# Nazukixv/LiteASR

Measured on AMD Instinct MI355X. Metric: utterances/sec (U2-Conformer+CTC, 80-d fbank T≈1000) at 1/2/4/8 MI355X, higher is better.
Workload: dtype bf16; 1 GPU; U2-Conformer-small hybrid CTC-attention training step (fwd+loss+bwd+allreduce+clip+Noam/Adam); model=U2 enc 12x conformer d256 H4 ff2048, dec 6x, V 4233, global_batch=32, per_gpu_batch=32, seq_len=1000, label_len=40, parallelism=dp1, launch=hipgraph, ranks_seen=1, rank_launcher=env

## Files before the change

### include/liteasr_hip.h

```cpp
#ifndef LITEASR_HIP_H
#define LITEASR_HIP_H

#include <stdint.h>

#ifdef __cplusplus
extern "C" {
#endif

enum { LASR_F32 = 0, LASR_BF16 = 1, LASR_I32 = 2, LASR_I64 = 3, LASR_U8 = 4 };
enum { LASR_OK = 0, LASR_ERR_INVALID = -1, LASR_ERR_LAUNCH = -2 };
enum { LASR_ACT_NONE = 0, LASR_ACT_RELU = 1, LASR_ACT_SWISH = 2,
       LASR_ACT_GATE = 3 ,
       LASR_ACT_TANH = 4  };

const char* lasr_last_error(void);
int lasr_version(void);
int lasr_set_dropout_counter(const uint64_t* dev_counter);
int lasr_counter_add(uint64_t* dev_counter, uint64_t v, void* stream);

typedef struct lasr_gemm_args {
  int M, N, K;
  int batch, batch_div;
  const void* A; int64_t lda_m, lda_k, sa1, sa2;
  const void* B; int64_t ldb_n, ldb_k, sb1, sb2;
  void* C; int64_t ldc, sc1, sc2;
  int in_dtype;
  int c_dtype;
  float alpha; const float* alpha_dev;
  float beta;
  const float* bias;
  int act;
  void* zout;
  const void* aux; int aux_dtype; int64_t ldaux; int aux_act;
  float drop_p; uint64_t drop_seed;
  const void* res; int res_dtype; int64_t ldres; float res_scale;
  int split_k;
  void* workspace; int64_t workspace_bytes;
  float* rowsum;
  int zout_mode;
  int tile_m, tile_n;
  int ksub;
} lasr_gemm_args;
int lasr_gemm(const lasr_gemm_args* args, void* stream);
int lasr_gemm_ln_fwd(const lasr_gemm_args* args, const float* gamma, const float* beta, float eps, void* y,
                     int y_dtype, float* mean, float* rstd, void* stream);
int lasr_gemm_ln_bwd(const lasr_gemm_args* args, const void* x, int x_dtype, const float* gamma, const float* mean,
                     const float* rstd, const void* dres, int dres_dtype, void* dx, int dx_dtype, float* part,
                     int64_t part_floats, void* gb, int gb_dtype, float bscale, float bp, uint64_t bseed,
                     void* stream);
int lasr_gemm_qbias_bwd(const lasr_gemm_args* args, const void* dqu, const void* dqv, int dt, int B, int T, int H,
                        int dk, void* dqkv, int64_t ld, float* ws, int64_t ws_floats, void* stream);
float lasr_dropout_scale(float p);
#define LASR_PLAN_GLDS 1
#define LASR_PLAN_ROWSUM_FUSED 2
#define LASR_PLAN_KSUB2 4
#define LASR_PLAN_WIDE 8
int lasr_gemm_plan(const lasr_gemm_args* args, int* tile_m, int* tile_n, int* split_k, int* flags);

int lasr_gemm_dw_group(const lasr_gemm_args* args, int n, void* stream);
int lasr_gemm_dw_group_order(int longest_first);
int lasr_gemm_narrow_tiles(int on);

typedef struct lasr_reduce_seg {
  const float* part; int64_t N; int P; int accumulate;
  float* out0; float* out1; int64_t split;
} lasr_reduce_seg;
int lasr_reduce_multi(const lasr_reduce_seg* segs, int nseg, void* stream);

int lasr_colsum(const void* X, int dtype, int64_t M, int64_t N, int64_t ldx,
                float* out, int accumulate, float* workspace, int64_t ws_floats, void* stream);

int lasr_layernorm_fwd(const void* x, int x_dtype, int64_t rows, int D, const float* gamma,
                       const float* beta, float eps, void* y, int y_dtype, float* mean,
                       float* rstd, void* y2, int y2_dtype, float p2, uint64_t seed2,
                       void* stream);
int lasr_layernorm2_fwd(const float* x, int64_t rows, int D, const float* g1, const float* b1,
                        const float* g2, const float* b2, float eps, float* y, float* mean1,
                        float* rstd1, void* z, float* mean2, float* rstd2, void* stream);
int lasr_layernorm_bwd(const void* x, int x_dtype, const void* dy, int dy_dtype, int64_t rows,
                       int D, const float* gamma, const float* mean, const float* rstd,
                       const void* dres, int dres_dtype, void* dx, int dx_dtype,
                       float* dgamma, float* dbeta, float* workspace, int64_t ws_floats,
                       void* gb, int gb_dtype, float bscale, float bp, uint64_t bseed,
                       void* stream);
int lasr_layernorm2_bwd(const float* x1, const void* dy1, int dy1_dtype, const float* dres1, int64_t rows, int D,
                        const float* g1, const float* mean1, const float* rstd1, float* part1, const float* x2,
                        const float* g2, const float* mean2, const float* rstd2, float* dx2, float* part2, void* gb2,
                        int gb2_dtype, float bscale, float bp, uint64_t bseed, void* stream);
typedef struct lasr_row_ln_args {
  int M, D, K;
  const void* A; int64_t lda;
  const void* W; int64_t ldw;
  const float* gamma1; const float* beta1; float eps;
  float* mean1; float* rstd1;
  const float* bias; const float* res; float res_scale; float drop_p; uint64_t drop_seed;
  float* out; void* y1; int y1_dtype;
  const float* gamma2; const float* beta2; void* y2; float* mean2; float* rstd2;
  const float* x; const float* dres; float* dx; void* gb; float bscale; float bp; uint64_t bseed;
  float* part; float* dgamma; float* dbeta;
} lasr_row_ln_args;
int lasr_linear_res_ln(const lasr_row_ln_args* args, void* stream);
int lasr_linear_dx_ln_bwd(const lasr_row_ln_args* args, void* stream);

int lasr_branch_grad(const void* dx, int dx_dtype, int64_t n, void* gb, int gb_dtype,
                     float scale, float p, uint64_t seed, void* stream);

int lasr_ctc_fwd(const void* logits, int ldt, int B, int T, int V, int64_t ld, const int32_t* targets,
                 int Lmax, const int32_t* ilen, const int32_t* tlen, float* lse, float* lp,
                 float* alpha, float* beta, float* nll, void* stream);
int lasr_ctc_lattice(int B, int T, int Lmax, const int32_t* targets, const int32_t* ilen, const int32_t* tlen,
                     const float* lp, float* alpha, float* beta, float* nll, void* stream);
int lasr_ctc_bwd(const void* logits, int ldt, int B, int T, int V, int64_t ld, const int32_t* targets,
                 int Lmax, const int32_t* ilen, const int32_t* tlen, const float* lse,
                 const float* lp, const float* alpha, const float* nll, float* beta,
                 int beta_ready, void* grad, int gdt, float gscale, const float* gdev, void* stream);

int lasr_lsm_kl_fwd(const void* logits, int ldt, int R, int V, int64_t ld, const int32_t* target,
                    int ignore, float smoothing, float* lse, float* loss_rows, void* stream);
int lasr_lsm_kl_bwd(const void* logits, int ldt, int R, int V, int64_t ld, const int32_t* target,
                    int ignore, float smoothing, const float* lse, void* grad, int gdt,
                    float gscale, const float* gdev, void* stream);
int lasr_loss_combine(const float* a, int na, float wa, const float* b, int nb, float wb,
                      float* out, void* stream);

int lasr_qbias_fwd(const void* qkv, int dt, int B, int T, int H, int dk, int64_t ld_qkv,
                   const float* bias_u, const float* bias_v, void* qu, void* qv, void* stream);
int lasr_qbias_bwd(const void* dqu, const void* dqv, int dt, int B, int T, int H, int dk,
                   void* dqkv, int64_t ld_dqkv, float* dbias_u, float* dbias_v,
                   float* workspace, int64_t ws_floats, void* stream);
int lasr_attn_softmax_fwd(const float* s_ac, const float* s_bd, int relpos, int B, int H,
                          int Tq, int Tk, int ldS, const uint8_t* mask, int64_t mask_sb,
                          int64_t mask_sq, void* P, int pdt, float drop_p, uint64_t seed,
                          void* Praw, void* stream);
int lasr_attn_softmax_bwd(const void* P, int pdt, const float* dPd, int B, int H, int Tq, int Tk,
                          int ldS, const uint8_t* mask, int64_t mask_sb, int64_t mask_sq,
                          float drop_p, uint64_t seed, void* dS, int dsdt, void* stream);
int lasr_relshift_bwd(const void* dS, int dt, int Z, int T, int ldS, void* dBD, void* stream);
int lasr_relattn_fwd(const void* qu, const void* qv, int64_t ldq, const void* k, const void* v,
                     int64_t ldkv, const void* pos, int64_t ldp, int B, int H, int T, int dk,
                     const uint8_t* mask, int64_t mask_sb, int64_t mask_sq, float scale,
                     float* stats, void* ctx, int64_t ldc, void* stream);
int lasr_relattn_fwd_qb(const void* q, int64_t ldqin, const float* bu, const float* bv, void* qu, void* qv,
                        int64_t ldq, const void* k, const void* v, int64_t ldkv, const void* pos, int64_t ldp,
                        int B, int H, int T, int dk, const uint8_t* mask, int64_t mask_sb, int64_t mask_sq,
                        float scale, float* stats, void* ctx, int64_t ldc, void* stream);
int lasr_relattn_bwd(const void* qu, const void* qv, int64_t ldq, const void* k, const void* v,
                     int64_t ldkv, const void* pos, int64_t ldp, int B, int H, int T, int dk,
                     const uint8_t* mask, int64_t mask_sb, int64_t mask_sq, float scale,
                     const float* stats, const void* ctx, const void* dctx, int64_t ldc,
                     float* Dbuf, void* dqu, void* dbd, int ldS, int dbd_head_major, void* dk_out,
                     void* dv_out, int64_t lddkv, void* stream);
int lasr_attn_fwd(const void* q, int64_t ldq, const void* k, const void* v, int64_t ldkv, int B, int H,
// ... 36 lines not shown
  const void* w2p;
  const float* bias;
  const void* dy2; int64_t dy2_rows;
  void* out;
  float* rowsum;
  void* workspace; int64_t workspace_bytes;
  const float* x; int T, F;
  float* dw1; float* db1;
} lasr_conv2_args;
int lasr_conv2_gemm(const lasr_conv2_args* args, void* stream);
int64_t lasr_conv2_dx_w1_workspace(int B, int T1, int F1, int C);
typedef struct lasr_cif_args {
  int B, T, D, U;
  const float* z; const int* plen; const int* ylen; const float* h;
  float* alpha; float* acc; uint8_t* fired; int* row; float* sum_alpha; float* mae; float* out;
  const float* gout; const float* gsum; float* dz; float* dh;
} lasr_cif_args;
int lasr_cif_fwd(const lasr_cif_args* args, void* stream);
int lasr_cif_bwd(const lasr_cif_args* args, void* stream);
typedef struct lasr_cif_infer_args {
  int B, T, D;
  const float* z; const int* plen; const float* h;
  float* alpha; float* acc; uint8_t* fired; int* row; float* sum_alpha; int* ulen; int* count; float* out;
} lasr_cif_infer_args;
int lasr_cif_infer(const lasr_cif_infer_args* args, void* stream);
int lasr_glancing_mix(int64_t rows, int D, const uint8_t* replace, const float* a, const float* b,
                      float* out, float* out2, int backward, void* stream);
int lasr_permute_last2(const void* src, int sdt, int64_t N, int64_t A, int64_t Bd, void* dst,
                       int ddt, int reverse, int accumulate, void* stream);

int lasr_glu_dwconv_fwd(const void* z1, int dt, int B, int T, int C, int K, const float* w,
                        const float* bias, void* y, int ydt, float* stats_ws, void* stream);
int lasr_dwconv_nparts(int B, int T);
int lasr_bn_finalize(const float* stats_ws, int nparts, int C, float eps, float momentum,
                     const float* gamma, const float* beta, float* running_mean,
                     float* running_var, int64_t* num_batches, float* mean, float* rstd,
                     float* scale, float* shift, int mode, void* stream);
int lasr_bn_act_fwd(const void* y, int ydt, int64_t rows, int C, const float* scale,
                    const float* shift, void* h, int hdt, int act, void* stream);
int lasr_bn_act_bwd(const void* y, int ydt, const void* dh, int hdt, int64_t rows, int C,
                    const float* scale, const float* shift, const float* mean,
                    const float* rstd, const float* gamma, float* dgamma, float* dbeta,
                    void* dy, int dydt, float* ws, int64_t ws_floats, int batch_stats, int act,
                    void* stream);
int lasr_glu_dwconv_bwd(const void* z1, int dt, const void* dy, int dydt, int B, int T, int C,
                        int K, const float* w, void* dz1, float* dw, float* db, float* ws,
                        int64_t ws_floats, void* stream);
int lasr_bn_act_glu_dwconv_bwd(const void* y, int ydt, const void* dh, int hdt, int B, int T, int C,
                               const float* scale, const float* shift, const float* mean, const float* rstd,
                               const float* gamma, float* dgamma, float* dbeta, float* bn_ws,
                               int64_t bn_ws_floats, int batch_stats, int act, const void* z1, int dt, int K,
                               const float* w, void* dz1, float* dw, float* db, float* ws, int64_t ws_floats,
                               void* stream);

int lasr_cast(const void* src, int sdt, void* dst, int ddt, int64_t n, void* stream);
int lasr_scale_add(const void* a, int adt, const void* b, int bdt, float sa, float sb,
                   void* out, int odt, int64_t n, void* stream);
int lasr_embed_pe_fwd(const int32_t* ids, int R, int L, int D, const float* E,
                      const float* pe, float xscale, float p, uint64_t seed, void* y, int ydt,
                      void* stream);
int lasr_embed_bwd(const int32_t* ids, int R, int D, const void* dy, int dydt, float xscale,
                   float p, uint64_t seed, float* dE, void* stream);
int lasr_pe_fwd(const void* x, int xdt, int64_t rows, int T, int D, const float* pe,
                float xscale, float p, uint64_t seed, void* y, int ydt, void* stream);

int lasr_rnnt_fwd(const void* logits, int ldt, int B, int T, int U1, int V, int64_t ld, const int32_t* targets,
                  int Lmax, const int32_t* ilen, const int32_t* tlen, int blank, float* lse, float* lp,
                  float* alpha, float* beta, float* nll, void* stream);
int lasr_rnnt_bwd(const void* logits, int ldt, int B, int T, int U1, int V, int64_t ld, const int32_t* targets,
                  int Lmax, const int32_t* ilen, const int32_t* tlen, int blank, const float* lse, const float* lp,
                  const float* alpha, const float* beta, const float* nll, void* grad, int gdt, float gscale,
                  const float* gdev, void* stream);
int lasr_joint_fwd(const float* e, const float* d, int B, int T, int U1, int J, void* z, int zdt, void* stream);
int lasr_joint_reduce(const void* dz, int dzdt, int B, int T, int U1, int J, void* de, void* dd, int odt,
                      void* stream);
int lasr_lstm_cell_fwd(const float* gates, int64_t ldg, const float* bias, const float* c_prev, int B, int H,
                       float* c_out, void* h_out, int hdt, int64_t ldh, void* stream);
int lasr_lstm_cell_bwd(const float* gates, int64_t ldg, const float* bias, const float* c, const float* c_prev,
                       const void* dh_out, int dhdt, int64_t lddh, const float* dh_rec, const float* dc_next, int B,
                       int H, void* dgates, int gdt, int64_t lddg, float* dc_prev, void* stream);

int lasr_u2_prep(const int64_t* xlens, const int64_t* ys, const int64_t* ylens, int B, int Tx,
                 int L, int Tsub, int sos, int eos, int chunk, int32_t* ys_in, int32_t* tgt,
                 int32_t* tgt_ctc, uint8_t* dec_mask, uint8_t* enc_mask, int32_t* pred_len,
                 int32_t* ylen32, void* stream);
int lasr_u2_prep_ld(const int64_t* xlens, const int64_t* ys, const int64_t* ylens, int B, int Tx,
                    int L, int Tsub, int sos, int eos, int chunk, int32_t* ys_in, int32_t* tgt,
                    int32_t* tgt_ctc, uint8_t* dec_mask, int dec_ld, uint8_t* enc_mask, int enc_ld,
                    int32_t* pred_len, int32_t* ylen32, void* stream);
int lasr_u2_prep_chunk(const int64_t* xlens, const int64_t* ys, const int64_t* ylens, int B, int L,
                       int Tsub, int sos, int eos, int chunk_mode, int chunk, int32_t* chunk_dev,
                       const uint64_t* ctr, uint64_t chunk_seed, int chunk_max, int32_t* ys_in,
                       int32_t* tgt, int32_t* tgt_ctc, uint8_t* dec_mask, int dec_ld, uint8_t* key_mask,
                       uint8_t* chunk_mask, int chunk_ld, int32_t* pred_len, int32_t* ylen32,
                       void* stream);

int64_t lasr_spec_augment_ws_bytes(int B, int Tmax);
int lasr_spec_augment(const float* x, float* out, const int64_t* xlens, const int32_t* plan,
                      int plan_stride, int B, int Tmax, int F, int replace_with_zero, void* ws,
                      int64_t ws_bytes, void* stream);

int lasr_sumsq_nparts(int64_t n);
int lasr_sumsq_partial(const float* g, int64_t n, float* ws, int64_t ws_floats, void* stream);
int lasr_adam_step(float* param, void* param_lp, int lp_dtype, const float* grad, float* m,
                   float* v, int64_t n, const float* ws, int nparts, float* state,
                   float max_norm, int lr_mode, float lr, float factor, float model_dim,
// ... 81 lines not shown
```

### liteasr_amd/_native.py

```python

from __future__ import annotations

import ctypes as C
import os

_HERE = os.path.dirname(os.path.abspath(__file__))
LIB_PATH = os.path.join(_HERE, "lib", "libliteasr_hip.so")

F32, BF16, I32, I64, U8 = 0, 1, 2, 3, 4
ACT_NONE, ACT_RELU, ACT_SWISH, ACT_GATE, ACT_TANH = 0, 1, 2, 3, 4

_p = C.c_void_p
_i = C.c_int
_l = C.c_int64
_f = C.c_float
_u = C.c_uint64


class GemmArgs(C.Structure):

    _fields_ = [
        ("M", _i), ("N", _i), ("K", _i),
        ("batch", _i), ("batch_div", _i),
        ("A", _p), ("lda_m", _l), ("lda_k", _l), ("sa1", _l), ("sa2", _l),
        ("B", _p), ("ldb_n", _l), ("ldb_k", _l), ("sb1", _l), ("sb2", _l),
        ("C", _p), ("ldc", _l), ("sc1", _l), ("sc2", _l),
        ("in_dtype", _i), ("c_dtype", _i),
        ("alpha", _f), ("alpha_dev", _p),
        ("beta", _f),
        ("bias", _p),
        ("act", _i),
        ("zout", _p),
        ("aux", _p), ("aux_dtype", _i), ("ldaux", _l), ("aux_act", _i),
        ("drop_p", _f), ("drop_seed", _u),
        ("res", _p), ("res_dtype", _i), ("ldres", _l), ("res_scale", _f),
        ("split_k", _i), ("workspace", _p), ("workspace_bytes", _l),
        ("rowsum", _p),
        ("zout_mode", _i),
        ("tile_m", _i), ("tile_n", _i), ("ksub", _i),
    ]


class Conv2Args(C.Structure):

    _fields_ = [
        ("mode", _i),
        ("B", _i), ("T1", _i), ("F1", _i), ("C", _i),
        ("y1", _p), ("w2p", _p), ("bias", _p),
        ("dy2", _p), ("dy2_rows", _l),
        ("out", _p), ("rowsum", _p),
        ("workspace", _p), ("workspace_bytes", _l),
        ("x", _p), ("T", _i), ("F", _i),
        ("dw1", _p), ("db1", _p),
    ]


CONV2_FWD, CONV2_DW, CONV2_DX, CONV2_DX_W1 = 0, 1, 2, 3


class CifArgs(C.Structure):

    _fields_ = [
        ("B", _i), ("T", _i), ("D", _i), ("U", _i),
        ("z", _p), ("plen", _p), ("ylen", _p), ("h", _p),
        ("alpha", _p), ("acc", _p), ("fired", _p), ("row", _p), ("sum_alpha", _p), ("mae", _p), ("out", _p),
        ("gout", _p), ("gsum", _p), ("dz", _p), ("dh", _p),
    ]


class CifInferArgs(C.Structure):

    _fields_ = [
        ("B", _i), ("T", _i), ("D", _i),
        ("z", _p), ("plen", _p), ("h", _p),
        ("alpha", _p), ("acc", _p), ("fired", _p), ("row", _p), ("sum_alpha", _p), ("ulen", _p), ("count", _p),
        ("out", _p),
    ]


class RowLnArgs(C.Structure):

    _fields_ = [
        ("M", _i), ("D", _i), ("K", _i),
        ("A", _p), ("lda", _l), ("W", _p), ("ldw", _l),
        ("gamma1", _p), ("beta1", _p), ("eps", _f), ("mean1", _p), ("rstd1", _p),
        ("bias", _p), ("res", _p), ("res_scale", _f), ("drop_p", _f), ("drop_seed", _u),
        ("out", _p), ("y1", _p), ("y1_dtype", _i),
        ("gamma2", _p), ("beta2", _p), ("y2", _p), ("mean2", _p), ("rstd2", _p),
        ("x", _p), ("dres", _p), ("dx", _p), ("gb", _p), ("bscale", _f), ("bp", _f), ("bseed", _u),
        ("part", _p), ("dgamma", _p), ("dbeta", _p),
    ]


class ReduceSeg(C.Structure):

    _fields_ = [("part", _p), ("N", _l), ("P", _i), ("accumulate", _i), ("out0", _p), ("out1", _p),
                ("split", _l)]


RNNT_SEARCH_MAX_LAYERS = 8


class RnntSearchArgs(C.Structure):

    _fields_ = [
        ("Tcap", _i), ("layers", _i), ("dec_dim", _i), ("H", _i), ("J", _i), ("V", _i),
        ("node_cap", _i), ("slot_cap", _i),
        ("w_dtype", _i),
        ("arena", _p), ("arena_bytes", _l),
        ("embed", _p),
        ("Wih", _p * RNNT_SEARCH_MAX_LAYERS), ("Whh", _p * RNNT_SEARCH_MAX_LAYERS),
        ("bih", _p * RNNT_SEARCH_MAX_LAYERS), ("bhh", _p * RNNT_SEARCH_MAX_LAYERS),
        ("Wd", _p), ("Wj", _p), ("bj", _p), ("enc_proj", _p),
    ]


SIGNATURES = {
    "lasr_version": [],
    "lasr_last_error": [],
    "lasr_set_dropout_counter": [_p],
    "lasr_counter_add": [_p, _u, _p],
    "lasr_gemm": [C.POINTER(GemmArgs), _p],
    "lasr_gemm_plan": [C.POINTER(GemmArgs), _p, _p, _p, _p],
    "lasr_gemm_dw_group": [C.POINTER(GemmArgs), _i, _p],
    "lasr_gemm_dw_group_order": [_i],
    "lasr_gemm_narrow_tiles": [_i],
    "lasr_relattn_fwd": [_p, _p, _l, _p, _p, _l, _p, _l, _i, _i, _i, _i, _p, _l, _l, _f, _p, _p, _l, _p],
    "lasr_relattn_fwd_qb": [_p, _l, _p, _p, _p, _p, _l, _p, _p, _l, _p, _l, _i, _i, _i, _i, _p, _l, _l, _f, _p, _p,
                            _l, _p],
    "lasr_attn_fwd": [_p, _l, _p, _p, _l, _i, _i, _i, _i, _i, _p, _l, _l, _f, _p, _p, _l, _p],
    "lasr_attn_bwd": [_p, _l, _p, _p, _l, _i, _i, _i, _i, _i, _p, _l, _l, _f, _p, _p, _p, _l, _p, _p, _p, _p,
                      _l, _p],
    "lasr_attn_fwd_split": [_p, _l, _p, _p, _l, _i, _i, _i, _i, _i, _p, _l, _l, _f, _p, _p, _l, _i, _p, _l, _p],
    "lasr_attn_bwd_split": [_p, _l, _p, _p, _l, _i, _i, _i, _i, _i, _p, _l, _l, _f, _p, _p, _p, _l, _p, _p, _p,
                            _p, _l, _i, _p, _l, _p],
    "lasr_attn_split_work": [_i, _i, _i, _i, _i],
    "lasr_attn_split_count": [_i, _i, _i, _i],
    "lasr_relattn_bwd": [_p, _p, _l, _p, _p, _l, _p, _l, _i, _i, _i, _i, _p, _l, _l, _f, _p, _p, _p, _l,
                         _p, _p, _p, _i, _i, _p, _p, _l, _p],
    "lasr_reduce_multi": [C.POINTER(ReduceSeg), _i, _p],
    "lasr_linear_res_ln": [C.POINTER(RowLnArgs), _p],
    "lasr_linear_dx_ln_bwd": [C.POINTER(RowLnArgs), _p],
    "lasr_dropout_scale": [_f],
    "lasr_colsum": [_p, _i, _l, _l, _l, _p, _i, _p, _l, _p],
    "lasr_layernorm2_fwd": [_p, _l, _i, _p, _p, _p, _p, _f, _p, _p, _p, _p, _p, _p, _p],
    "lasr_layernorm_fwd": [_p, _i, _l, _i, _p, _p, _f, _p, _i, _p, _p, _p, _i, _f, _u, _p],
    "lasr_layernorm_bwd": [_p, _i, _p, _i, _l, _i, _p, _p, _p, _p, _i, _p, _i, _p, _p, _p, _l,
                           _p, _i, _f, _f, _u, _p],
    "lasr_layernorm2_bwd": [_p, _p, _i, _p, _l, _i, _p, _p, _p, _p, _p, _p, _p, _p, _p, _p, _p, _i, _f, _f, _u,
                            _p],
    "lasr_branch_grad": [_p, _i, _l, _p, _i, _f, _f, _u, _p],
    "lasr_ctc_fwd": [_p, _i, _i, _i, _i, _l, _p, _i, _p, _p, _p, _p, _p, _p, _p, _p],
    "lasr_ctc_lattice": [_i, _i, _i, _p, _p, _p, _p, _p, _p, _p, _p],
    "lasr_rnnt_fwd": [_p, _i, _i, _i, _i, _i, _l, _p, _i, _p, _p, _i, _p, _p, _p, _p, _p, _p],
    "lasr_rnnt_bwd": [_p, _i, _i, _i, _i, _i, _l, _p, _i, _p, _p, _i, _p, _p, _p, _p, _p, _p, _i, _f, _p, _p],
    "lasr_joint_fwd": [_p, _p, _i, _i, _i, _i, _p, _i, _p],
    "lasr_joint_reduce": [_p, _i, _i, _i, _i, _i, _p, _p, _i, _p],
    "lasr_lstm_cell_fwd": [_p, _l, _p, _p, _i, _i, _p, _p, _i, _l, _p],
    "lasr_lstm_cell_bwd": [_p, _l, _p, _p, _p, _p, _i, _l, _p, _p, _i, _i, _p, _i, _l, _p, _p],
    "lasr_ctc_bwd": [_p, _i, _i, _i, _i, _l, _p, _i, _p, _p, _p, _p, _p, _p, _p, _i, _p, _i, _f, _p, _p],
    "lasr_lsm_kl_fwd": [_p, _i, _i, _i, _l, _p, _i, _f, _p, _p, _p],
    "lasr_lsm_kl_bwd": [_p, _i, _i, _i, _l, _p, _i, _f, _p, _p, _i, _f, _p, _p],
    "lasr_loss_combine": [_p, _i, _f, _p, _i, _f, _p, _p],
    "lasr_qbias_fwd": [_p, _i, _i, _i, _i, _i, _l, _p, _p, _p, _p, _p],
    "lasr_qbias_bwd": [_p, _p, _i, _i, _i, _i, _i, _p, _l, _p, _p, _p, _l, _p],
    "lasr_attn_softmax_fwd": [_p, _p, _i, _i, _i, _i, _i, _i, _p, _l, _l, _p, _i, _f, _u, _p, _p],
    "lasr_attn_softmax_bwd": [_p, _i, _p, _i, _i, _i, _i, _i, _p, _l, _l, _f, _u, _p, _i, _p],
    "lasr_relshift_bwd": [_p, _i, _i, _i, _i, _p, _p],
    "lasr_reduce_batch": [_p, _i, _i, _i, _i, _p, _i, _p],
    "lasr_conv1_fwd": [_p, _i, _i, _i, _i, _p, _p, _p, _i, _p],
    "lasr_conv1_bwd": [_p, _i, _i, _i, _i, _p, _i, _p, _p, _p, _l, _p],
    "lasr_conv2_gemm": [C.POINTER(Conv2Args), _p],
    "lasr_conv2_dx_w1_workspace": [_i, _i, _i, _i],
    "lasr_cif_fwd": [C.POINTER(CifArgs), _p],
    "lasr_cif_bwd": [C.POINTER(CifArgs), _p],
    "lasr_cif_infer": [C.POINTER(CifInferArgs), _p],
    "lasr_glancing_mix": [_l, _i, _p, _p, _p, _p, _p, _i, _p],
    "lasr_im2col3x3s2": [_p, _i, _i, _i, _i, _i, _p, _p],
    "lasr_col2im3x3s2": [_p, _i, _i, _i, _i, _i, _p, _p, _p],
    "lasr_permute_last2": [_p, _i, _l, _l, _l, _p, _i, _i, _i, _p],
    "lasr_glu_dwconv_fwd": [_p, _i, _i, _i, _i, _i, _p, _p, _p, _i, _p, _p],
    "lasr_dwconv_nparts": [_i, _i],
    "lasr_bn_finalize": [_p, _i, _i, _f, _f, _p, _p, _p, _p, _p, _p, _p, _p, _p, _i, _p],
    "lasr_bn_act_fwd": [_p, _i, _l, _i, _p, _p, _p, _i, _i, _p],
    "lasr_bn_act_bwd": [_p, _i, _p, _i, _l, _i, _p, _p, _p, _p, _p, _p, _p, _p, _i, _p, _l, _i, _i, _p],
    "lasr_glu_dwconv_bwd": [_p, _i, _p, _i, _i, _i, _i, _i, _p, _p, _p, _p, _p, _l, _p],
    "lasr_bn_act_glu_dwconv_bwd": [_p, _i, _p, _i, _i, _i, _i, _p, _p, _p, _p, _p, _p, _p, _p, _l, _i, _i,
                                   _p, _i, _i, _p, _p, _p, _p, _p, _l, _p],
    "lasr_cast": [_p, _i, _p, _i, _l, _p],
    "lasr_scale_add": [_p, _i, _p, _i, _f, _f, _p, _i, _l, _p],
    "lasr_embed_pe_fwd": [_p, _i, _i, _i, _p, _p, _f, _f, _u, _p, _i, _p],
    "lasr_embed_bwd": [_p, _i, _i, _p, _i, _f, _f, _u, _p, _p],
    "lasr_pe_fwd": [_p, _i, _l, _i, _i, _p, _f, _f, _u, _p, _i, _p],
    "lasr_u2_prep": [_p, _p, _p, _i, _i, _i, _i, _i, _i, _i, _p, _p, _p, _p, _p, _p, _p, _p],
    "lasr_u2_prep_ld": [_p, _p, _p, _i, _i, _i, _i, _i, _i, _i, _p, _p, _p, _p, _i, _p, _i, _p, _p, _p],
    "lasr_gemm_qbias_bwd": [C.POINTER(GemmArgs), _p, _p, _i, _i, _i, _i, _i, _p, _l, _p, _l, _p],
    "lasr_gemm_ln_fwd": [C.POINTER(GemmArgs), _p, _p, _f, _p, _i, _p, _p, _p],
    "lasr_gemm_ln_bwd": [C.POINTER(GemmArgs), _p, _i, _p, _p, _p, _p, _i, _p, _i, _p, _l, _p, _i, _f, _f, _u, _p],
    "lasr_u2_prep_chunk": [_p, _p, _p, _i, _i, _i, _i, _i, _i, _i, _p, _p, _u, _i,
                           _p, _p, _p, _p, _i, _p, _p, _i, _p, _p, _p],
    "lasr_sumsq_nparts": [_l],
    "lasr_sumsq_partial": [_p, _l, _p, _l, _p],
    "lasr_adam_step": [_p, _p, _i, _p, _p, _p, _l, _p, _i, _p, _f, _i, _f, _f, _f, _f, _f, _f,
                       _f, _f, _p],
    "lasr_fill": [_p, _i, _l, _f, _p],
    "lasr_spec_augment": [_p, _p, _p, _p, _i, _i, _i, _i, _i, _p, _l, _p],
    "lasr_spec_augment_ws_bytes": [_i, _i],
    "lasr_logsoftmax_topk": [_p, _i, _l, _i, _l, _i, _p, _p, _p, _p, _p],
    "lasr_rnnt_search_workspace": [_i, _i, _i, _i, _i, _i, _i],
    "lasr_rnnt_search_init": [C.POINTER(RnntSearchArgs), _i, _p],
    "lasr_rnnt_search_expand": [C.POINTER(RnntSearchArgs), _i, _p],
    "lasr_rescore_workspace": [_i, _i],
    "lasr_rescore_search": [_p, _l, _i, _i, _i, _i, _i, _p, _p, _p, _p],
    "lasr_rescore_prep": [_p, _l, _i, _i, _i, _i, _p, _p, _i, _p, _p, _p],
    "lasr_rescore_pick": [_p, _l, _i, _i, _p, C.c_double, _p],
    "lasr_w2v_conv0_fwd": [_p, _i, _i, _i, _i, _i, _p, _p, _p, _p],
    "lasr_w2v_conv0_dw_parts": [_i, _i],
    "lasr_w2v_conv0_dw": [_p, _p, _i, _i, _i, _i, _i, _i, _p, _p, _l, _p],
    "lasr_w2v_ln_act_fwd": [_p, _i, _l, _i, _p, _p, _f, _i, _p, _i, _p, _p, _p],
    "lasr_w2v_ln_act_bwd": [_p, _i, _p, _i, _l, _i, _p, _p, _p, _p, _i, _p, _i, _p, _p, _p, _l, _p],
    "lasr_w2v_col2im1d": [_p, _i, _i, _i, _i, _i, _i, _i, _p, _p],
    "lasr_w2v_group_pack": [_p, _i, _i, _i, _i, _i, _i, _p, _i, _p, _p, _i, _p],
    "lasr_w2v_group_unpack": [_p, _i, _p, _i, _p, _i, _i, _i, _i, _p, _p],
    "lasr_w2v_group_colsum": [_p, _i, _i, _l, _i, _p, _p],
    "lasr_w2v_mask_fwd": [_p, _p, _i, _i, _i, _i, _p, _p],
    "lasr_w2v_mask_bwd": [_p, _p, _i, _i, _i, _i, _p, _p],
    "lasr_w2v_gather_rows": [_p, _i, _l, _l, _p, _i, _i, _i, _i, _p, _i, _p],
    "lasr_w2v_scatter_rows": [_p, _i, _p, _i, _i, _i, _i, _p, _l, _l, _i, _p],
    "lasr_w2v_gumbel_fwd": [_p, _i, _p, _u, _f, _i, _l, _i, _i, _p, _i, _p, _i, _p, _p],
    "lasr_w2v_gumbel_bwd": [_p, _i, _p, _u, _f, _i, _l, _i, _i, _p, _i, _p, _i, _p, _p, _i, _p, _p],
    "lasr_w2v_contrast_fwd": [_p, _p, _p, _p, _i, _i, _i, _i, _i, _f, _p, _p, _p, _p, _p],
    "lasr_w2v_contrast_bwd": [_p, _p, _p, _p, _i, _i, _i, _i, _i, _f, _p, _p, _p, _p, _p, _l, _p],
}
_RESTYPES = {"lasr_last_error": C.c_char_p, "lasr_spec_augment_ws_bytes": C.c_int64,
             "lasr_rnnt_search_workspace": C.c_int64, "lasr_rescore_workspace": C.c_int64,
             "lasr_conv2_dx_w1_workspace": C.c_int64, "lasr_attn_split_work": C.c_int64,
             "lasr_dropout_scale": C.c_float}


class NativeError(RuntimeError):
    pass
# ... 39 lines not shown
```

### liteasr_amd/csrc/common.h

```cpp
#pragma once
#include <hip/hip_runtime.h>
#include <stdint.h>

#include "../../include/liteasr_hip.h"

typedef uint16_t bf16_t;

#define LASR_DEV __device__ __forceinline__

LASR_DEV float bf2f(bf16_t h) { return __uint_as_float(((uint32_t)h) << 16); }
LASR_DEV bf16_t f2bf(float f) {
  __bf16 b = (__bf16)f;
  return __builtin_bit_cast(bf16_t, b);
}

typedef float lasr_f2 __attribute__((ext_vector_type(2)));
typedef __bf16 lasr_bf2 __attribute__((ext_vector_type(2)));
LASR_DEV uint32_t pk_bf16(float a, float b) {
  return __builtin_bit_cast(uint32_t, __builtin_convertvector((lasr_f2){a, b}, lasr_bf2));
}

LASR_DEV float to_f(float x) { return x; }
LASR_DEV float to_f(bf16_t x) { return bf2f(x); }
template <typename T> LASR_DEV T from_f(float x);
// ... 180 lines not shown
    if (q + 1 < N) k[q + 1] = (b >> 16) >= d.thr ? 1.f : 0.f;
  }
}
template <int N>
LASR_DEV uint32_t drop_keep_mask(const DropCfg& d, uint32_t key, uint64_t idx0) {
  uint32_t km = 0u;
  if (idx0 & 1) {
#pragma unroll
    for (int q = 0; q < N; ++q) km |= (drop_keep_k(d, key, idx0 + q) != 0.f ? 1u : 0u) << q;
    return km;
  }
#pragma unroll
  for (int q = 0; q < N; q += 2) {
    const uint32_t b = drop_bits(key, (idx0 >> 1) + (q >> 1));
    km |= ((b & 0xFFFFu) >= d.thr ? 1u : 0u) << q;
    if (q + 1 < N) km |= ((b >> 16) >= d.thr ? 1u : 0u) << (q + 1);
  }
  return km;
}
template <int N>
LASR_DEV uint32_t drop_keep_mask_even(const DropCfg& d, uint32_t key, uint64_t idx0) {
  static_assert(N % 2 == 0, "pairs");
  uint32_t km = 0u;
  const uint64_t pair0 = idx0 >> 1;
#pragma unroll
  for (int q = 0; q < N; q += 2) {
    const uint32_t b = drop_bits(key, pair0 + (q >> 1));
    km |= ((b & 0xFFFFu) >= d.thr ? 1u : 0u) << q;
    km |= ((b >> 16) >= d.thr ? 1u : 0u) << (q + 1);
  }
  return km;
}
template <int N>
LASR_DEV void drop_mul_n(const DropCfg& d, uint32_t key, uint64_t idx0, float* m) {
  drop_keep_n<N>(d, key, idx0, m);
#pragma unroll
  for (int q = 0; q < N; ++q) m[q] *= d.scale;
}
LASR_DEV uint32_t drop_key_if(const DropCfg& d) { return d.p > 0.f ? drop_key(d) : 0u; }
LASR_DEV float drop_mul_if(const DropCfg& d, uint32_t key, uint64_t idx) {
  return d.p > 0.f ? drop_mul_k(d, key, idx) : 1.f;
}
LASR_DEV float drop_mul(const DropCfg& d, uint64_t idx) {
  if (d.p <= 0.f) return 1.f;
  return drop_mul_k(d, drop_key(d), idx);
}

LASR_DEV float sigmoidf_(float x) { return __builtin_amdgcn_rcpf(1.f + __expf(-x)); }
LASR_DEV float swishf(float x) { return x * sigmoidf_(x); }
LASR_DEV float swish_grad(float z) {
  const float s = sigmoidf_(z);
  return s * (1.f + z * (1.f - s));
}

void lasr_set_error(const char* fmt, ...);
int lasr_check_launch(const char* what);

#define LASR_CHECK_ARG(cond, ...)          \
  do {                                     \
    if (!(cond)) {                         \
      lasr_set_error(__VA_ARGS__);         \
      return LASR_ERR_INVALID;             \
    }                                      \
  } while (0)

static inline int64_t cdiv(int64_t a, int64_t b) { return (a + b - 1) / b; }

int lasr_reduce_cols(const float* part, int P, int64_t N, float* out0, float* out1, int64_t split,
                     int accumulate, hipStream_t st);
int lasr_scatter_kc(const float* src, int K, int C, int ld, float* dst, float* bias,
                    hipStream_t st);
```

### liteasr_amd/csrc/conv.hip

```cpp
#include "common.h"

template <typename T>
__global__ __launch_bounds__(256) void conv1_fwd_kernel(const float* __restrict__ x, int T_, int F,
                                                        int C, int T1, int F1, const float* w,
                                                        const float* bias, T* y1) {
  extern __shared__ float sh[];
  float* xs = sh;
  float* ws = sh + 3 * F;
  const int bt = blockIdx.x;
  const int b = bt / T1, t1 = bt - b * T1;
  for (int i = threadIdx.x; i < 3 * F; i += blockDim.x) {
    const int kh = i / F, f = i - kh * F;
    xs[i] = x[((int64_t)b * T_ + 2 * t1 + kh) * F + f];
  }
  for (int i = threadIdx.x; i < C * 9; i += blockDim.x) ws[(i / 9) * 10 + (i % 9)] = w[i];
  for (int c = threadIdx.x; c < C; c += blockDim.x) ws[c * 10 + 9] = bias[c];
  __syncthreads();
  T* out = y1 + (int64_t)bt * F1 * C;
  for (int e = threadIdx.x; e < F1 * C; e += blockDim.x) {
    const int f1 = e / C, c = e - f1 * C;
    const float* wc = ws + c * 10;
    float acc = wc[9];
#pragma unroll
    for (int kh = 0; kh < 3; ++kh)
// ... 540 lines not shown
  const int tx = threadIdx.x % BNF_C, ty = threadIdx.x / BNF_C;
  const int c = blockIdx.x * BNF_C + tx;
  if (blockIdx.x == 0 && threadIdx.x == 0 && update == 1 && nbt) nbt[0] += 1;
  if (update == 2) {
    if (ty == 0 && c < C) {
      const float rs = rsqrtf(rvar[c] + eps);
      mean[c] = rmean[c];
      rstd[c] = rs;
      const float sc = __fmul_rn(gamma[c], rs);
      scale[c] = sc;
      shift[c] = fmaf(-rmean[c], sc, beta[c]);
    }
    return;
  }
  double n = 0.0, s = 0.0;
  if (c < C)
    for (int p = ty; p < nparts; p += BNF_G) {
      const float* st = stats + (int64_t)p * 3 * C;
      const double nb = st[c];
      n += nb;
      s += nb * (double)st[C + c];
    }
  sn[ty][tx] = n;
  smu[ty][tx] = s;
  __syncthreads();
  for (int w = BNF_G / 2; w >= 1; w >>= 1) {
    if (ty < w) {
      sn[ty][tx] += sn[ty + w][tx];
      smu[ty][tx] += smu[ty + w][tx];
    }
    __syncthreads();
  }
  n = sn[0][tx];
  s = smu[0][tx];
  const double mu = n > 0.0 ? s / n : 0.0;
  double m2 = 0.0;
  if (c < C)
    for (int p = ty; p < nparts; p += BNF_G) {
      const float* st = stats + (int64_t)p * 3 * C;
      const double nb = st[c], dl = (double)st[C + c] - mu;
      m2 += (double)st[2 * C + c] + nb * dl * dl;
    }
  sm2[ty][tx] = m2;
  __syncthreads();
  for (int w = BNF_G / 2; w >= 1; w >>= 1) {
    if (ty < w) sm2[ty][tx] += sm2[ty + w][tx];
    __syncthreads();
  }
  if (ty != 0 || c >= C) return;
  m2 = sm2[0][tx];
  bn_final_write(c, n, mu, m2, eps, momentum, gamma, beta, rmean, rvar, mean, rstd, scale, shift, update);
}

template <bool RELU>
LASR_DEV float bn_act(float u) {
  if constexpr (RELU) return fmaxf(u, 0.f);
  else return swishf(u);
}
template <bool RELU>
LASR_DEV float bn_act_grad(float u) {
  if constexpr (RELU) return u > 0.f ? 1.f : 0.f;
  else return swish_grad(u);
}

template <bool RELU>
LASR_DEV float bn_dy(float yv, float gv, float sc, float sf, float mu, float rs, float ga, float t1, float t2,
                     float inv_n) {
  const float du = gv * bn_act_grad<RELU>(yv * sc + sf);
  const float xh = (yv - mu) * rs;
  return ga * rs * (du - t1 * inv_n - xh * t2 * inv_n);
}

template <typename TY, typename TH, bool RELU>
struct BnDyWin {
  const TY* y;
  const TH* dh;
  const float *scale, *shift, *mean, *rstd, *gamma, *tot;
  float* dgamma;
  float* dbeta;
  float inv_n;
  int C;
  LASR_DEV float one(float yv, float gv, int c) const {
    return bn_dy<RELU>(yv, gv, scale[c], shift[c], mean[c], rstd[c], gamma[c], tot[c], tot[C + c], inv_n);
  }
  LASR_DEV void load8(const TY* row, int ce, float* v, float* u) const {
    float yv[8], gv[8];
    ldv<8>(row + ce, yv);
    ldv<8>(dh + (row - y) + ce, gv);
#pragma unroll
    for (int k = 0; k < 8; ++k) {
      v[k] = one(yv[k], gv[k], ce + k);
      u[k] = 0.f;
    }
  }
  LASR_DEV void load2(const TY* row, int ce, float* v, float* u) const {
    float yv[2], gv[2];
    ldv<2>(row + ce, yv);
    ldv<2>(dh + (row - y) + ce, gv);
    v[0] = one(yv[0], gv[0], ce);
    v[1] = one(yv[1], gv[1], ce + 1);
    u[0] = u[1] = 0.f;
  }
  LASR_DEV float2 pair(const float* v, const float*) const { return make_float2(v[0], v[1]); }
  LASR_DEV void finish(int) const {
    if (blockIdx.x == 0 && blockIdx.y == 0)
      for (int c = threadIdx.x; c < C; c += blockDim.x) {
        dbeta[c] += tot[c];
        dgamma[c] += tot[C + c];
      }
  }
};

template <typename TY, typename TH, bool RELU>
__global__ void bn_act_fwd_kernel(const TY* y, int64_t rows, int C, const float* scale,
                                  const float* shift, TH* h) {
  const int64_t n8 = rows * C / 8;
// ... 281 lines not shown
  hipStream_t st = (hipStream_t)stream;
  if (act == LASR_ACT_RELU)
    return bn_act_bwd_launch<true>(y, ydt, dh, hdt, rows, C, scale, shift, mean, rstd, gamma, dgamma, dbeta, dy,
                                   dydt, ws, nparts, batch_stats, st);
  return bn_act_bwd_launch<false>(y, ydt, dh, hdt, rows, C, scale, shift, mean, rstd, gamma, dgamma, dbeta, dy,
                                  dydt, ws, nparts, batch_stats, st);
}

extern "C" int lasr_glu_dwconv_bwd(const void* z1, int dt, const void* dy, int dydt, int B, int T,
                                   int C, int K, const float* w, void* dz1, float* dw, float* db,
                                   float* ws, int64_t ws_floats, void* stream) {
  LASR_CHECK_ARG(K == DW_K, "lasr_glu_dwconv_bwd: only kernel size %d is built", DW_K);
  const int nchunk = (int)cdiv(T, DW_TT);
  const int nparts = B * nchunk;
  LASR_CHECK_ARG(ws_floats >= (int64_t)nparts * (DW_K + 1) * C, "lasr_glu_dwconv_bwd: workspace too small");
  LASR_CHECK_ARG(C % 2 == 0, "lasr_glu_dwconv_bwd: C must be even");
  dim3 g((unsigned)nparts, (unsigned)cdiv(C, 2 * DW_CP));
  hipStream_t st = (hipStream_t)stream;
  const int vec = C % 8 == 0 && ((uintptr_t)z1 & 15) == 0 && ((uintptr_t)dy & 15) == 0 && ((uintptr_t)dz1 & 15) == 0;
#define GB(TT, TD) glu_dwconv_bwd_kernel<TT, TD><<<g, DW_NT, 0, st>>>((const TT*)z1, (const TD*)dy, T, C, w, (TT*)dz1, ws, vec)
  if (dt == LASR_F32 && dydt == LASR_F32) GB(float, float);
  else if (dt == LASR_F32) GB(float, bf16_t);
  else if (dydt == LASR_F32) GB(bf16_t, float);
  else GB(bf16_t, bf16_t);
#undef GB
  int rc = lasr_check_launch("glu_dwconv_bwd");
  if (rc || (!dw && !db)) return rc;
  LASR_CHECK_ARG(dw && db, "lasr_glu_dwconv_bwd: dw and db go together");
  return lasr_reduce_cols(ws, nparts, (int64_t)(DW_K + 1) * C, dw, db, (int64_t)DW_K * C, 1, st);
}

template <typename TT, typename TY, typename TH, bool RELU>
static void bn_glu_launch(dim3 g, hipStream_t st, const void* z1, const void* y, const void* dh, int T, int C,
                          const float* w, void* dz1, float* ws, int vec, const BnDyWin<TY, TH, RELU>& f) {
  glu_dwconv_bwd_kernel<TT, TY, BnDyWin<TY, TH, RELU>><<<g, DW_NT, 0, st>>>((const TT*)z1, (const TY*)y, T, C, w,
                                                                          (TT*)dz1, ws, vec, f);
}

template <typename TT, typename TY, typename TH>
static void bn_glu_dispatch(bool relu, dim3 g, hipStream_t st, const void* z1, const void* y, const void* dh, int T,
                            int C, const float* w, void* dz1, float* ws, int vec, const float* scale,
                            const float* shift, const float* mean, const float* rstd, const float* gamma,
                            const float* tot, float* dgamma, float* dbeta, float inv_n) {
  if (relu)
    bn_glu_launch<TT, TY, TH, true>(g, st, z1, y, dh, T, C, w, dz1, ws, vec,
                                    BnDyWin<TY, TH, true>{(const TY*)y, (const TH*)dh, scale, shift, mean, rstd,
                                                          gamma, tot, dgamma, dbeta, inv_n, C});
  else
    bn_glu_launch<TT, TY, TH, false>(g, st, z1, y, dh, T, C, w, dz1, ws, vec,
                                     BnDyWin<TY, TH, false>{(const TY*)y, (const TH*)dh, scale, shift, mean, rstd,
                                                            gamma, tot, dgamma, dbeta, inv_n, C});
}

extern "C" int lasr_bn_act_glu_dwconv_bwd(const void* y, int ydt, const void* dh, int hdt, int B, int T, int C,
                                          const float* scale, const float* shift, const float* mean,
                                          const float* rstd, const float* gamma, float* dgamma, float* dbeta,
                                          float* bn_ws, int64_t bn_ws_floats, int batch_stats, int act,
                                          const void* z1, int dt, int K, const float* w, void* dz1, float* dw,
                                          float* db, float* ws, int64_t ws_floats, void* stream) {
  const int64_t rows = (int64_t)B * T;
  const int64_t nparts_bn = cdiv(rows, BN_ROWS);
  LASR_CHECK_ARG(bn_ws_floats >= (nparts_bn + 1) * 2 * C, "lasr_bn_act_glu_dwconv_bwd: BN workspace too small");
  LASR_CHECK_ARG(nparts_bn <= 65535, "lasr_bn_act_glu_dwconv_bwd: too many rows");
  LASR_CHECK_ARG(act == LASR_ACT_SWISH || act == LASR_ACT_RELU, "lasr_bn_act_glu_dwconv_bwd: act must be SWISH or RELU");
  LASR_CHECK_ARG(K == DW_K, "lasr_bn_act_glu_dwconv_bwd: only kernel size %d is built", DW_K);
  LASR_CHECK_ARG(C % 8 == 0 && rows > 0, "lasr_bn_act_glu_dwconv_bwd: C must be a multiple of 8, rows > 0");
  LASR_CHECK_ARG((ydt == LASR_F32 || ydt == LASR_BF16) && (hdt == LASR_F32 || hdt == LASR_BF16) &&
                     (dt == LASR_F32 || dt == LASR_BF16), "lasr_bn_act_glu_dwconv_bwd: bad dtype");
  const int nchunk = (int)cdiv(T, DW_TT);
  const int nparts = B * nchunk;
  LASR_CHECK_ARG(ws_floats >= (int64_t)nparts * (DW_K + 1) * C, "lasr_bn_act_glu_dwconv_bwd: workspace too small");
  hipStream_t st = (hipStream_t)stream;
  float* tot = bn_ws + nparts_bn * 2 * C;
  {
    dim3 g((unsigned)cdiv(C, 2 * BN_CP), (unsigned)nparts_bn);
#define BR(RL, TY, TH) bn_act_bwd_reduce_kernel<TY, TH, RL><<<g, 256, 0, st>>>((const TY*)y, (const TH*)dh, rows, C, scale, shift, mean, rstd, bn_ws)
    const bool relu = act == LASR_ACT_RELU, yf = ydt == LASR_F32, hf = hdt == LASR_F32;
    if (relu) {
      if (yf && hf) BR(true, float, float); else if (yf) BR(true, float, bf16_t);
      else if (hf) BR(true, bf16_t, float); else BR(true, bf16_t, bf16_t);
    } else {
      if (yf && hf) BR(false, float, float); else if (yf) BR(false, float, bf16_t);
      else if (hf) BR(false, bf16_t, float); else BR(false, bf16_t, bf16_t);
    }
#undef BR
    if (int rc = lasr_check_launch("bn_act_glu_dwconv_bwd/reduce")) return rc;
    if (int rc = lasr_reduce_cols(bn_ws, (int)nparts_bn, 2 * C, tot, nullptr, 2 * C, 0, st)) return rc;
  }
  const float inv_n = batch_stats ? 1.f / (float)rows : 0.f;
  dim3 g((unsigned)nparts, (unsigned)cdiv(C, 2 * DW_CP));
  const int vec = ((uintptr_t)z1 & 15) == 0 && ((uintptr_t)y & 15) == 0 && ((uintptr_t)dh & 15) == 0 &&
                  ((uintptr_t)dz1 & 15) == 0;
  const bool relu = act == LASR_ACT_RELU;
#define BG(TT, TY, TH) bn_glu_dispatch<TT, TY, TH>(relu, g, st, z1, y, dh, T, C, w, dz1, ws, vec, scale, shift, mean, rstd, gamma, tot, dgamma, dbeta, inv_n)
  const bool zf = dt == LASR_F32, yf = ydt == LASR_F32, hf = hdt == LASR_F32;
  if (zf) {
    if (yf && hf) BG(float, float, float); else if (yf) BG(float, float, bf16_t);
    else if (hf) BG(float, bf16_t, float); else BG(float, bf16_t, bf16_t);
  } else {
    if (yf && hf) BG(bf16_t, float, float); else if (yf) BG(bf16_t, float, bf16_t);
    else if (hf) BG(bf16_t, bf16_t, float); else BG(bf16_t, bf16_t, bf16_t);
  }
#undef BG
  int rc = lasr_check_launch("bn_act_glu_dwconv_bwd");
  if (rc || (!dw && !db)) return rc;
  LASR_CHECK_ARG(dw && db, "lasr_bn_act_glu_dwconv_bwd: dw and db go together");
  return lasr_reduce_cols(ws, nparts, (int64_t)(DW_K + 1) * C, dw, db, (int64_t)DW_K * C, 1, st);
}
```

### liteasr_amd/csrc/gemm.hip

```cpp
#include "gemm_kernel.h"
#include <algorithm>


template <bool AKC, bool BKC, typename TC>
void launch_bf16(const GemmP& p, int BM, int BN, int ks, int nw, bool glds, dim3 grid, hipStream_t st);
#define LASR_EXTERN_LAUNCH(ak, bk)                                                                         \
  extern template void launch_bf16<ak, bk, float>(const GemmP&, int, int, int, int, bool, dim3, hipStream_t); \
  extern template void launch_bf16<ak, bk, bf16_t>(const GemmP&, int, int, int, int, bool, dim3, hipStream_t);
LASR_EXTERN_LAUNCH(true, true)
LASR_EXTERN_LAUNCH(true, false)
LASR_EXTERN_LAUNCH(false, true)
LASR_EXTERN_LAUNCH(false, false)
#undef LASR_EXTERN_LAUNCH

template <typename TC>
static void dispatch(const GemmP& p, bool akc, bool bkc, int bf16in, int BM, int BN, int ks, int nw, bool glds,
                     dim3 grid, hipStream_t st) {
  if (bf16in) {
    if (akc && bkc) launch_bf16<true, true, TC>(p, BM, BN, ks, nw, glds, grid, st);
    else if (akc) launch_bf16<true, false, TC>(p, BM, BN, ks, nw, glds, grid, st);
    else if (bkc) launch_bf16<false, true, TC>(p, BM, BN, ks, nw, glds, grid, st);
    else launch_bf16<false, false, TC>(p, BM, BN, ks, nw, glds, grid, st);
  } else {
    if (akc && bkc) gemm_f32_kernel<true, true, TC><<<grid, 256, 0, st>>>(p);
// ... 36 lines not shown
    const int cfg[4][2] = {{128, 128}, {128, 64}, {64, 128}, {64, 64}};
    const int c0 = a->N <= 64 && narrow_n_tiles ? 3 : 0;
    for (int c = c0; c < 4; ++c) {
      const int64_t nb = cdiv(a->M, cfg[c][0]) * cdiv(a->N, cfg[c][1]) * (int64_t)batch;
      BM = cfg[c][0]; BN = cfg[c][1];
      if (nb >= 480) break;
    }
    if (BM == 128 && BN == 128 && a->N >= 256 && a->K >= 1024 && cdiv(a->M, 128) * batch >= 1024) BN = 256;
    if (BM == 128 && BN == 128 && (a->zout || a->aux || (a->act && a->drop_p > 0.f)) && a->N >= 1024) BN = 256;
  }
  if (!bf && autosplit) {
    const int64_t nb = cdiv(a->M, BM) * cdiv(a->N, BN) * (int64_t)batch;
    while (nb * split < 512 && split * 2 <= 32 && kt / (split * 2) >= 4) split *= 2;
  }
  if (bf && a->tile_m) {
    BM = a->tile_m;
    BN = a->tile_n;
    nw = 4;
  }
  if (a->split_k <= -2 && plain && a->workspace) split = -a->split_k;
  const int64_t rs_floats = a->rowsum ? (int64_t)split * a->M : 0;
  if (split > 1 && ((!plain && !autosplit && (a->split_k < 2 || a->zout)) || !a->workspace ||
                    a->workspace_bytes < ((int64_t)split * batch * a->M * a->N + rs_floats) * 4))
    split = 1;
  if (kso) {
    const int64_t kc = split > 1 ? cdiv(a->K, split) : a->K;
    const bool small = BM * BN <= 64 * 128;
    *kso = (bf && BM < 256 && BN < 256 && ((BM == 64 && BN == 64) || kc >= 1024 || (kc >= 512 && small))) ? 2 : 1;
    if (nw == 8) *kso = 2;
    else if (a->ksub) *kso = a->ksub;
  }
  if (nwo) *nwo = nw;
  *BMo = BM;
  *BNo = BN;
  *splito = split;
}

static bool gemm_uses_glds(const lasr_gemm_args* a) {
  if (a->in_dtype != LASR_BF16) return false;
  const bool akc = (a->lda_k == 1), bkc = (a->ldb_k == 1);
  const int64_t s_a = akc ? a->lda_m : a->lda_k;
  const int64_t s_b = bkc ? a->ldb_n : a->ldb_k;
  const bool a_vec = aligned16(a->A) && s_a % 8 == 0 && a->sa1 % 8 == 0 && a->sa2 % 8 == 0;
  const bool b_vec = aligned16(a->B) && s_b % 8 == 0 && a->sb1 % 8 == 0 && a->sb2 % 8 == 0;
  const int64_t M8 = cdiv(a->M, 8) * 8, N8 = cdiv(a->N, 8) * 8;
  return a_vec && b_vec && (akc || a->lda_k >= M8) && (bkc || a->ldb_k >= N8);
}

static bool tile_ok(int tm, int tn) {
  return (tm == 0 && tn == 0) || ((tm == 64 || tm == 128 || tm == 256) && (tn == 64 || tn == 128 || tn == 256) &&
                                  (tm < 256 || tn >= 128) && (tn < 256 || tm >= 128));
}

extern "C" int lasr_gemm_plan(const lasr_gemm_args* a, int* tile_m, int* tile_n, int* split_k, int* flags) {
  LASR_CHECK_ARG(a && tile_m && tile_n && split_k, "lasr_gemm_plan: null argument");
  int ks = 1, nw = 4;
  gemm_plan(a, tile_m, tile_n, split_k, &ks, &nw);
  const bool glds = gemm_uses_glds(a);
  if (!glds) {
    *tile_m = std::min(*tile_m, 128);
    *tile_n = std::min(*tile_n, 128);
    nw = 4;
  }
  if (flags) {
    *flags = (glds ? LASR_PLAN_GLDS : 0) | (a->rowsum && glds && a->lda_k != 1 ? LASR_PLAN_ROWSUM_FUSED : 0) |
             (glds && ks == 2 && (*tile_m < 256 || nw == 8) ? LASR_PLAN_KSUB2 : 0) |
             (glds && nw == 8 ? LASR_PLAN_WIDE : 0);
  }
  return LASR_OK;
}

extern "C" int lasr_gemm(const lasr_gemm_args* a, void* stream) { return gemm_run(a, stream, nullptr); }

int gemm_run(const lasr_gemm_args* a, void* stream, GemmRowPost* post) {
  LASR_CHECK_ARG(a != nullptr, "lasr_gemm: null args");
  LASR_CHECK_ARG(a->M >= 0 && a->N >= 0 && a->K >= 0, "lasr_gemm: negative size");
  LASR_CHECK_ARG(a->in_dtype == LASR_F32 || a->in_dtype == LASR_BF16, "lasr_gemm: bad in_dtype");
  LASR_CHECK_ARG(a->c_dtype == LASR_F32 || a->c_dtype == LASR_BF16, "lasr_gemm: bad c_dtype");
  LASR_CHECK_ARG(a->lda_m == 1 || a->lda_k == 1, "lasr_gemm: A needs a unit stride");
  LASR_CHECK_ARG(a->ldb_n == 1 || a->ldb_k == 1, "lasr_gemm: B needs a unit stride");
  LASR_CHECK_ARG(a->A && a->B && a->C, "lasr_gemm: null operand");
  LASR_CHECK_ARG(a->zout_mode == 0 || a->zout_mode == 1, "lasr_gemm: zout_mode must be 0 or 1");
  LASR_CHECK_ARG(a->act != LASR_ACT_GATE && (!a->aux || a->aux_act != LASR_ACT_NONE),
                 "lasr_gemm: act GATE is only an aux_act; aux needs an aux_act");
  LASR_CHECK_ARG(tile_ok(a->tile_m, a->tile_n) && a->ksub >= 0 && a->ksub <= 2,
                 "lasr_gemm: tile override must be 64/128/256 x 64/128/256 (256 only beside >= 128) or 0 x 0, "
                 "ksub 0, 1 or 2");
  if (a->M == 0 || a->N == 0 || a->batch == 0) return LASR_OK;
  const int batch = a->batch > 0 ? a->batch : 1;
  const int bdiv = a->batch_div > 0 ? a->batch_div : 1;
  LASR_CHECK_ARG(batch == 1 || (!a->aux && !a->res && !a->zout && !a->rowsum),
                 "lasr_gemm: aux/res/zout/rowsum only supported for batch == 1");
  LASR_CHECK_ARG(!a->rowsum || a->lda_m == 1, "lasr_gemm: rowsum needs an M-contiguous A");

  GemmP p;
  p.M = a->M; p.N = a->N; p.K = a->K; p.batch = batch; p.batch_div = bdiv;
  p.A = a->A; p.lda_m = a->lda_m; p.lda_k = a->lda_k; p.sa1 = a->sa1; p.sa2 = a->sa2;
  p.B = a->B; p.ldb_n = a->ldb_n; p.ldb_k = a->ldb_k; p.sb1 = a->sb1; p.sb2 = a->sb2;
  p.C = a->C; p.ldc = a->ldc; p.sc1 = a->sc1; p.sc2 = a->sc2;
  p.alpha = a->alpha; p.alpha_dev = a->alpha_dev; p.beta = a->beta;
  p.bias = a->bias; p.act = a->act; p.zout = a->zout; p.zout_mode = a->zout_mode;
  p.aux = a->aux; p.aux_dtype = a->aux_dtype; p.ldaux = a->ldaux; p.aux_act = a->aux_act;
  p.drop = mkdrop(a->drop_p, a->drop_seed);
  p.res = a->res; p.res_dtype = a->res_dtype; p.ldres = a->ldres; p.res_scale = a->res_scale;

  const bool akc = (a->lda_k == 1);
  const bool bkc = (a->ldb_k == 1);
  const bool bf = a->in_dtype == LASR_BF16;
  {
    const int64_t s_a = akc ? a->lda_m : a->lda_k;
    const int64_t s_b = bkc ? a->ldb_n : a->ldb_k;
    p.a_vec = bf && aligned16(a->A) && s_a % 8 == 0 && a->sa1 % 8 == 0 && a->sa2 % 8 == 0;
    p.b_vec = bf && aligned16(a->B) && s_b % 8 == 0 && a->sb1 % 8 == 0 && a->sb2 % 8 == 0;
  }
  p.c_vec = aligned16(a->C) && a->ldc % 8 == 0 && a->sc1 % 8 == 0 && a->sc2 % 8 == 0 &&
            (!a->zout || aligned16(a->zout));
  p.aux_vec = a->aux && aligned16(a->aux) && a->ldaux % 8 == 0;
  p.res_vec = a->res && aligned16(a->res) && a->ldres % 8 == 0;
  p.ws_vec = a->N % 8 == 0;
  p.bias_vec = a->bias && aligned16(a->bias);
  {
    auto al4 = [](const void* q, int dtp) {
      return ((uintptr_t)q & (dtp == LASR_F32 ? 15 : 7)) == 0;
    };
    const int cdt = a->c_dtype;
    p.v4 = a->N % 4 == 0 && a->ldc % 4 == 0 && a->sc1 % 4 == 0 && a->sc2 % 4 == 0 && al4(a->C, cdt) &&
           (!a->zout || al4(a->zout, cdt)) && (!a->bias || aligned16(a->bias)) &&
           (!a->aux || (a->ldaux % 4 == 0 && al4(a->aux, a->aux_dtype))) &&
           (!a->res || (a->ldres % 4 == 0 && al4(a->res, a->res_dtype))) &&
           (!a->workspace || aligned16(a->workspace));
  }
  {
    const int nsrc = (a->aux ? 1 : 0) + (a->res ? 1 : 0);
    const bool base_ok = p.c_vec && a->beta == 0.f;
    const bool src_ok = nsrc == 1 && a->N % 8 == 0 && (a->aux ? p.aux_vec : p.res_vec);
    p.epi_mode = !base_ok ? 2 : nsrc == 0 ? 0 : src_ok ? 1 : 2;
  }

  int BM, BN, split, ks, nw;
  gemm_plan(a, &BM, &BN, &split, &ks, &nw);
  p.split_k = split;
  const int kstep = bf ? 32 : 16;
  p.kchunk = split > 1 ? (int)(cdiv(cdiv(a->K, split), kstep) * kstep) : a->K;
  p.ws = (float*)a->workspace;
  p.rowsum = nullptr;
  p.rs_ws = nullptr;

  hipStream_t st = (hipStream_t)stream;
  const bool glds = gemm_uses_glds(a);
  if (!glds) {
    BM = std::min(BM, 128);
    BN = std::min(BN, 128);
    nw = 4;
  }
  dim3 grid((unsigned)cdiv(a->N, BN), (unsigned)cdiv(a->M, BM), (unsigned)(batch * split));
  LASR_CHECK_ARG(grid.y <= 65535 && grid.z <= 65535, "lasr_gemm: grid too large");
  const bool rs_fused = a->rowsum && glds && !akc;
  if (rs_fused) {
    p.rowsum = a->rowsum;
    if (split > 1) p.rs_ws = p.ws + (int64_t)split * batch * a->M * a->N;
  }
  if (a->c_dtype == LASR_F32) dispatch<float>(p, akc, bkc, bf, BM, BN, ks, nw, glds, grid, st);
  else dispatch<bf16_t>(p, akc, bkc, bf, BM, BN, ks, nw, glds, grid, st);
  int rc = lasr_check_launch("lasr_gemm");
  if (!rc && split > 1 && a->split_k >= 0 && post) {
    const int r = post->launch(p, post->ctx, st);
    if (r < 0) return r;
    post->done = r;
    if (r) {
      rc = lasr_check_launch("lasr_gemm/splitk_reduce_post");
      if (rc || !a->rowsum || rs_fused) return rc;
    }
  }
  if (!rc && split > 1 && a->split_k >= 0 && !(post && post->done)) {
    const int64_t total = (int64_t)a->M * a->N * batch;
    const int nblk = (int)std::min<int64_t>(cdiv(p.v4 ? total / 4 : total, 256), 4096);
    if (a->c_dtype == LASR_F32) splitk_reduce_kernel<float><<<nblk, 256, 0, st>>>(p);
    else splitk_reduce_kernel<bf16_t><<<nblk, 256, 0, st>>>(p);
    rc = lasr_check_launch("lasr_gemm/splitk_reduce");
  }
  if (rc || !a->rowsum || rs_fused) return rc;
  const int64_t used = split > 1 ? (int64_t)split * batch * a->M * a->N : 0;
  LASR_CHECK_ARG(a->workspace && a->workspace_bytes / 4 > used, "lasr_gemm: no workspace left for the rowsum");
  return lasr_colsum(a->A, a->in_dtype, a->K, a->M, a->lda_k, a->rowsum, 1, (float*)a->workspace + used,
                     a->workspace_bytes / 4 - used, stream);
}


int launch_dw_group(const DwGroupP& g, int BM, int BN, int blocks, bool serial, hipStream_t st);
static int dw_group_lpt = 1;
extern "C" int lasr_gemm_dw_group_order(int longest_first) {
  dw_group_lpt = longest_first != 0;
  return LASR_OK;
}

extern "C" int lasr_gemm_dw_group(const lasr_gemm_args* args, int n, void* stream) {
  LASR_CHECK_ARG(args && n >= 1 && n <= LASR_DW_GROUP_MAX, "lasr_gemm_dw_group: 1..%d problems", LASR_DW_GROUP_MAX);
  DwGroupP g = {};
  g.n = n;
  int ord[LASR_DW_GROUP_MAX];
  int64_t work[LASR_DW_GROUP_MAX];
  auto planned = [](const lasr_gemm_args* a) {
    lasr_gemm_args b = *a;
    if (b.split_k <= -2 && !b.workspace) {
      b.workspace = (void*)(uintptr_t)16;
      b.workspace_bytes = INT64_MAX;
    }
    return b;
  };
// ... 72 lines not shown
```

### liteasr_amd/csrc/gemm_kernel.h

```cpp
#pragma once
#include "common.h"
#include "tile.h"

#include <cstring>
#include <type_traits>

#ifndef LASR_EXP
#define LASR_EXP 0
#endif


struct ConvG {
  int B, T1, F1, T2, F2, C;
  int M2;
  int cls;
  int q32, r32;
  const bf16_t* zero;
  const float* x;
  int T0, F0;
  float* w1part;
  int w1rb;
};
typedef ConvG ConvGeom;
enum { G_LIN = 0, G_FWD = 1, G_DW = 2, G_DX = 3 };

struct GemmP {
  int M, N, K, batch, batch_div;
  const void* A;
  int64_t lda_m, lda_k, sa1, sa2;
  const void* B;
  int64_t ldb_n, ldb_k, sb1, sb2;
  void* C;
  int64_t ldc, sc1, sc2;
  float alpha;
  const float* alpha_dev;
  float beta;
  const float* bias;
  int act;
  void* zout;
  const void* aux;
  int aux_dtype;
  int64_t ldaux;
  int aux_act;
  DropCfg drop;
  const void* res;
  int res_dtype;
  int64_t ldres;
  float res_scale;
  int split_k;
  int kchunk;
  float* ws;
  int a_vec, b_vec;
  int c_vec, aux_vec, res_vec, ws_vec;
  int epi_mode;
  int bias_vec;
  float* rowsum;
  float* rs_ws;
  int v4;
  int zout_mode;
  ConvGeom cv;
};

struct GemmRowPost {
  int (*launch)(const GemmP& p, const void* ctx, hipStream_t st);
  const void* ctx;
  int done;
};
struct lasr_gemm_args;
int gemm_run(const lasr_gemm_args* a, void* stream, GemmRowPost* post);

LASR_DEV float load_any(const void* p, int dt, int64_t i) {
  return dt == LASR_F32 ? ((const float*)p)[i] : bf2f(((const bf16_t*)p)[i]);
}

enum {
  EPI_RT = 0, EPI_SWISH_GATE_DROP = 1, EPI_AUX_GATE = 2, EPI_PLAIN = 3, EPI_RES_DROP = 4, EPI_RELU_GATE_DROP = 5,
  EPI_RELU = 6, EPI_AUX_RELU = 7,
  EPI_AUX_RELU_W1 = 8
};

template <int N, int EPI = EPI_RT, typename ZST>
LASR_DEV void epi_core(const GemmP& p, uint32_t dkey, uint64_t dbase, float (&v)[N], const float (&auxv)[N],
                       bool has_aux, const float (&resv)[N], bool has_res, ZST zst) {
  if constexpr (EPI == EPI_SWISH_GATE_DROP) {
    const uint32_t km = (LASR_EXP & 8) ? 0xffffffffu : drop_keep_mask_even<N>(p.drop, dkey, dbase);
    float g[N];
#pragma unroll
    for (int q = 0; q < N; ++q) {
      if constexpr ((LASR_EXP & 16) != 0) {
        g[q] = v[q];
      } else {
        const float s = sigmoidf_(v[q]);
        g[q] = s * (1.f + v[q] * (1.f - s));
        v[q] *= s;
      }
    }
#pragma unroll
    for (int q = 0; q < N; ++q) g[q] *= (km >> q) & 1u ? 1.f : 0.f;
    zst(g);
#pragma unroll
    for (int q = 0; q < N; ++q) v[q] *= (km >> q) & 1u ? p.drop.scale : 0.f;
    return;
  } else if constexpr (EPI == EPI_AUX_GATE) {
#pragma unroll
    for (int q = 0; q < N; ++q) v[q] *= auxv[q];
    return;
  } else if constexpr (EPI == EPI_RELU_GATE_DROP) {
    const uint32_t km = drop_keep_mask_even<N>(p.drop, dkey, dbase);
    float g[N];
#pragma unroll
    for (int q = 0; q < N; ++q) g[q] = v[q] > 0.f ? 1.f : 0.f;
#pragma unroll
    for (int q = 0; q < N; ++q) g[q] *= (km >> q) & 1u ? 1.f : 0.f;
    zst(g);
#pragma unroll
    for (int q = 0; q < N; ++q) v[q] = fmaxf(v[q], 0.f);
#pragma unroll
    for (int q = 0; q < N; ++q) v[q] *= (km >> q) & 1u ? p.drop.scale : 0.f;
    return;
  } else if constexpr (EPI == EPI_RELU) {
#pragma unroll
    for (int q = 0; q < N; ++q) v[q] = fmaxf(v[q], 0.f);
    return;
  } else if constexpr (EPI == EPI_AUX_RELU || EPI == EPI_AUX_RELU_W1) {
#pragma unroll
    for (int q = 0; q < N; ++q) v[q] *= auxv[q] > 0.f ? 1.f : 0.f;
    return;
  } else if constexpr (EPI == EPI_PLAIN) {
    return;
  } else if constexpr (EPI == EPI_RES_DROP) {
    const uint32_t km = drop_keep_mask_even<N>(p.drop, dkey, dbase);
#pragma unroll
    for (int q = 0; q < N; ++q) v[q] *= (km >> q) & 1u ? p.drop.scale : 0.f;
#pragma unroll
    for (int q = 0; q < N; ++q) v[q] = resv[q] + p.res_scale * v[q];
    return;
  }
  const bool drop = p.drop.p > 0.f;
  const uint32_t km = drop ? drop_keep_mask<N>(p.drop, dkey, dbase) : 0u;
  bool acted = false;
  if (p.zout) {
    if (p.zout_mode == 1) {
      float g[N];
      if (p.act == LASR_ACT_SWISH) {
#pragma unroll
        for (int q = 0; q < N; ++q) {
          const float s = sigmoidf_(v[q]);
          g[q] = s * (1.f + v[q] * (1.f - s));
          v[q] *= s;
        }
        acted = true;
      } else if (p.act == LASR_ACT_RELU) {
#pragma unroll
        for (int q = 0; q < N; ++q) g[q] = v[q] > 0.f ? 1.f : 0.f;
      } else if (p.act == LASR_ACT_TANH) {
#pragma unroll
        for (int q = 0; q < N; ++q) {
          v[q] = tanhf(v[q]);
          g[q] = 1.f - v[q] * v[q];
        }
        acted = true;
      } else {
#pragma unroll
        for (int q = 0; q < N; ++q) g[q] = 1.f;
      }
      if (drop) {
#pragma unroll
        for (int q = 0; q < N; ++q) g[q] *= (km >> q) & 1u ? 1.f : 0.f;
      }
      zst(g);
    } else {
      zst(v);
    }
  }
  if (acted) {
  } else if (p.act == LASR_ACT_SWISH) {
#pragma unroll
    for (int q = 0; q < N; ++q) v[q] = swishf(v[q]);
  } else if (p.act == LASR_ACT_RELU) {
#pragma unroll
    for (int q = 0; q < N; ++q) v[q] = fmaxf(v[q], 0.f);
// ... 62 lines not shown
#pragma unroll
    for (int q = 0; q < 8; ++q)
      if (q < cnt) dst[q] = from_f<T>(v[q]);
  }
}

template <typename TC>
LASR_DEV void epi_store8(const GemmP& p, uint32_t dkey, int z1, int z2, int z, int m, int n, const float* acc,
                         float alpha_eff) {
  const int cnt = min(8, p.N - n);
  float v[8], t[8];
#pragma unroll
  for (int q = 0; q < 8; ++q) v[q] = acc[q] * alpha_eff;
  if (p.bias) {
#pragma unroll
    for (int q = 0; q < 8; ++q) v[q] += q < cnt ? p.bias[n + q] : 0.f;
  }
  const int64_t cidx = (int64_t)z1 * p.sc1 + (int64_t)z2 * p.sc2 + (int64_t)m * p.ldc + n;
  float r[8];
  if (p.aux) ld_any8(p.aux, p.aux_dtype, (int64_t)m * p.ldaux + n, p.aux_vec, cnt, t);
  if (p.res) ld_any8(p.res, p.res_dtype, (int64_t)m * p.ldres + n, p.res_vec, cnt, r);
  epi_core<8>(p, dkey, ((uint64_t)z * p.M + m) * (uint64_t)p.N + n, v, t, p.aux != nullptr, r, p.res != nullptr,
              [&](const float (&zv)[8]) { st_8((TC*)p.zout + cidx, zv, p.c_vec, cnt); });
  TC* C = (TC*)p.C + cidx;
  if (p.beta != 0.f) {
    ld_any8(C, sizeof(TC) == 4 ? LASR_F32 : LASR_BF16, 0, p.c_vec, cnt, t);
#pragma unroll
    for (int q = 0; q < 8; ++q) v[q] += p.beta * t[q];
  }
  st_8(C, v, p.c_vec, cnt);
}

template <typename TC, int EPI = EPI_RT>
LASR_DEV void epi_fast8(const GemmP& p, uint32_t dkey, int64_t cidx, int z, int m, int n, int cnt,
                        const float* acc, float alpha_eff, const float* bv, const float (&sv)[8]) {
  float v[8];
#pragma unroll
  for (int q = 0; q < 8; ++q) v[q] = acc[q] * alpha_eff + bv[q];
  epi_core<8, EPI>(p, dkey, ((uint64_t)z * p.M + m) * (uint64_t)p.N + n, v, sv, p.aux != nullptr, sv, p.res != nullptr,
              [&](const float (&zv)[8]) { st_8((TC*)p.zout + cidx, zv, true, cnt); });
  st_8((TC*)p.C + cidx, v, true, cnt);
}

LASR_DEV float alpha_of(const GemmP& p) {
  return p.alpha_dev ? p.alpha * p.alpha_dev[0] : p.alpha;
}


LASR_DEV int64_t dx_row(const ConvG& g, int m) {
  const int pt = g.cls >> 1, pf = g.cls & 1;
  const int nI = (g.T1 - pt + 1) >> 1, nJ = (g.F1 - pf + 1) >> 1;
  const int j = m % nJ, t = m / nJ, i = t % nI, b = t / nI;
  return ((int64_t)(b * g.T1 + 2 * i + pt) * g.F1 + 2 * j + pf) * g.C;
}

template <int BM, int BN, typename TC, bool TRANS = false, int G = G_LIN, int NW = 4, int EPI = EPI_RT>
LASR_DEV void gemm_epilogue(const GemmP& p, f32x4 (&acc)[BM / 32][BN / (8 * NW)], char* smem_epi, int m0,
                            int n0, int s, int z, int z1, int z2, const int64_t* dxrow = nullptr) {
  auto crow = [&](int m) -> int64_t {
    if constexpr (G == G_DX) return dxrow[m - m0];
    else return (int64_t)z1 * p.sc1 + (int64_t)z2 * p.sc2 + (int64_t)m * p.ldc;
  };
  constexpr int NT = NW * 64, WCOLS = NW / 2;
  constexpr int WM = BM / 2, WN = BN / WCOLS, FM = WM / 16, FN = WN / 16;
  const int tid = threadIdx.x, lane = tid & 63, wid = tid >> 6;
  const int wr = wid / WCOLS, wc = wid % WCOLS;
  constexpr int LDC = BN + 4;
  float* cs = reinterpret_cast<float*>(smem_epi);
  const int rq = (lane >> 4) * 4, cl = lane & 15;
  const float al = alpha_of(p);
  const uint32_t dkey = epi_key(p);
  const bool split = p.split_k > 1;
  float* wsp = split ? p.ws + ((int64_t)s * p.batch + z) * (int64_t)p.M * p.N : nullptr;
  constexpr int CPR = BN / 8, RPI = NT / CPR, ITERS = WM / RPI;
  static_assert(WM % RPI == 0, "epilogue tiling");
  const int ec8 = (tid % CPR) * 8, er0 = tid / CPR;
  const int en = n0 + ec8;
  const bool fast = G != G_LIN || (!split && p.epi_mode < 2);
  float bv[8];
#pragma unroll
  for (int q = 0; q < 8; ++q) bv[q] = 0.f;
  if (fast && p.bias && en < p.N) {
    if (p.bias_vec && en + 8 <= p.N) ld8(p.bias + en, bv);
    else
#pragma unroll
      for (int q = 0; q < 8; ++q) bv[q] = en + q < p.N ? p.bias[en + q] : 0.f;
  }
  const void* src = p.aux ? p.aux : p.res;
  const int src_dt = p.aux ? p.aux_dtype : p.res_dtype;
  const int64_t src_ld = p.aux ? p.ldaux : p.ldres;
#pragma unroll
  for (int h = 0; h < 2; ++h) {
    constexpr int PF = ITERS < 2 ? ITERS : 2;
    float sv[PF][8];
    auto prefetch = [&](int b) {
      if (!(fast && p.epi_mode == 1)) return;
      const int mlast = p.M - 1, nc = min(en, p.N - 8);
      if (src_dt == LASR_F32) {
#pragma unroll
        for (int it = 0; it < PF; ++it) {
          const int m = min(m0 + h * WM + er0 + (b + it) * RPI, mlast);
          const int64_t ro = G == G_DX ? dxrow[m - m0] : (int64_t)m * src_ld;
          ld8((const float*)src + ro + nc, sv[it]);
        }
      } else {
#pragma unroll
        for (int it = 0; it < PF; ++it) {
          const int m = min(m0 + h * WM + er0 + (b + it) * RPI, mlast);
          const int64_t ro = G == G_DX ? dxrow[m - m0] : (int64_t)m * src_ld;
          ld8((const bf16_t*)src + ro + nc, sv[it]);
        }
      }
    };
    prefetch(0);
    if (wr == h) {
      if constexpr (TRANS) {
#pragma unroll
        for (int i = 0; i < FM; ++i)
#pragma unroll
          for (int j = 0; j < FN; ++j)
            *(f32x4*)(cs + (i * 16 + cl) * LDC + wc * WN + j * 16 + rq) = acc[i][j];
      } else {
#pragma unroll
        for (int i = 0; i < FM; ++i)
#pragma unroll
          for (int j = 0; j < FN; ++j)
#pragma unroll
            for (int e = 0; e < 4; ++e) cs[(i * 16 + rq + e) * LDC + wc * WN + j * 16 + cl] = acc[i][j][e];
      }
    }
    __syncthreads();
    if (fast) {
#pragma unroll
      for (int b = 0; b < ITERS; b += PF) {
        if (b > 0) prefetch(b);
#pragma unroll
        for (int it = 0; it < PF; ++it) {
          const int r = er0 + (b + it) * RPI;
          const int m = m0 + h * WM + r;
          if (m < p.M && en < p.N) {
            float a8[8];
#pragma unroll
            for (int q = 0; q < 8; ++q) a8[q] = cs[r * LDC + ec8 + q];
            epi_fast8<TC, EPI>(p, dkey, crow(m) + en, z, m, en, min(8, p.N - en), a8, al, bv, sv[it]);
          }
        }
      }
      __syncthreads();
      continue;
    }
    constexpr int NV = WM * BN / 8;
    for (int v = tid; v < NV; v += NT) {
      const int r = v / (BN / 8), c8 = (v % (BN / 8)) * 8;
      const int m = m0 + h * WM + r, n = n0 + c8;
      if (m < p.M && n < p.N) {
        float a8[8];
#pragma unroll
        for (int q = 0; q < 8; ++q) a8[q] = cs[r * LDC + c8 + q];
        if (split) {
          float* dst = wsp + (int64_t)m * p.N + n;
          if (p.ws_vec && n + 8 <= p.N) st8(dst, a8);
          else
            for (int q = 0; q < 8 && n + q < p.N; ++q) dst[q] = a8[q];
        } else {
          epi_store8<TC>(p, dkey, z1, z2, z, m, n, a8, al);
        }
      }
    }
    __syncthreads();
  }
}

template <int BM, int BN, bool AKC, bool BKC, typename TC>
__global__ __launch_bounds__(256) void gemm_bf16_kernel(GemmP p) {
  constexpr int BK = 32;
  constexpr int WM = BM / 2, WN = BN / 2, FM = WM / 16, FN = WN / 16;
  constexpr int MAIN_BYTES = 2 * (BM + BN) * BK * 2;
  constexpr int EPI_BYTES = WM * (BN + 4) * 4;
  __shared__ __attribute__((aligned(16))) char smem_epi[MAIN_BYTES > EPI_BYTES ? MAIN_BYTES : EPI_BYTES];
  bf16_t* smem = reinterpret_cast<bf16_t*>(smem_epi);
  const int tid = threadIdx.x, lane = tid & 63, wid = tid >> 6;
  const int wr = wid >> 1, wc = wid & 1;

  const int zz = blockIdx.z;
  const int s = zz % p.split_k, z = zz / p.split_k;
  const int z1 = z / p.batch_div, z2 = z % p.batch_div;
  const bf16_t* A = (const bf16_t*)p.A + z1 * p.sa1 + z2 * p.sa2;
  const bf16_t* B = (const bf16_t*)p.B + z1 * p.sb1 + z2 * p.sb2;
  const int m0 = blockIdx.y * BM, n0 = blockIdx.x * BN;
  const int kbeg = s * p.kchunk;
  const int kend = min(p.K, kbeg + p.kchunk);
  const int nk = kend > kbeg ? (kend - kbeg + BK - 1) / BK : 0;

  f32x4 acc[FM][FN];
#pragma unroll
  for (int i = 0; i < FM; ++i)
#pragma unroll
    for (int j = 0; j < FN; ++j) acc[i][j] = (f32x4){0.f, 0.f, 0.f, 0.f};

  TileLoader<BM, AKC> la;
  TileLoader<BN, BKC> lb;
  const int64_t a_ldr = AKC ? p.lda_m : 0, a_ldk = AKC ? 0 : p.lda_k;
  const int64_t b_ldr = BKC ? p.ldb_n : 0, b_ldk = BKC ? 0 : p.ldb_k;

  if (nk > 0) {
    la.load(A, a_ldr, a_ldk, m0, p.M, kbeg, kend, p.a_vec, tid);
    lb.load(B, b_ldr, b_ldk, n0, p.N, kbeg, kend, p.b_vec, tid);
    la.store(smem, tid);
    lb.store(smem + BM * BK, tid);
  }
  __syncthreads();

  for (int kt = 0; kt < nk; ++kt) {
    bf16_t* cur = smem + (kt & 1) * (BM + BN) * BK;
    bf16_t* nxt = smem + ((kt + 1) & 1) * (BM + BN) * BK;
    const bool more = kt + 1 < nk;
    if (more) {
      const int k0 = kbeg + (kt + 1) * BK;
      la.load(A, a_ldr, a_ldk, m0, p.M, k0, kend, p.a_vec, tid);
      lb.load(B, b_ldr, b_ldk, n0, p.N, k0, kend, p.b_vec, tid);
    }
    bf16x8 af[FM], bfr[FN];
// ... 288 lines not shown
    const int tap = n0 / g.C, kh = tap / 3, kw = tap - 3 * kh;
    const int tbase = (kh * g.F1 + kw) * g.C - tap * g.C;
#pragma unroll
    for (int i = 0; i < PER; ++i) {
      const int P = i * NT + tid, k = P / CPR, ps = P % CPR;
      const int ls = ((((ps >> 1) ^ htr<R_TILE>(k))) << 1) | (ps & 1);
      const int gc = min(n0 + ls * 8, ((N + 7) & ~7) - 8);
      noff[i] = tbase + gc;
      const int m = kbeg + k;
      f2[i] = m % g.F2;
      const int t = m / g.F2;
      t2[i] = t % g.T2;
      b[i] = t / g.T2;
    }
  }
  LASR_DEV void issue(const ConvG& g, const bf16_t* base, bf16_t* dst, int tid) {
    const int wid = tid >> 6;
    const int last = ((g.B * g.T1 - g.T1 + 2 * (g.T2 - 1)) * g.F1 + 2 * (g.F2 - 1)) * g.C;
#pragma unroll
    for (int i = 0; i < PER; ++i) {
      const int rb = b[i] < g.B ? ((b[i] * g.T1 + 2 * t2[i]) * g.F1 + 2 * f2[i]) * g.C : last;
      __builtin_amdgcn_global_load_lds((gptr_t)(base + rb + noff[i]), (lptr_t)(dst + (i * NT + wid * 64) * 8),
                                       16, 0, 0);
      f2[i] += g.r32;
      t2[i] += g.q32;
      if (f2[i] >= g.F2) { f2[i] -= g.F2; t2[i] += 1; }
      while (t2[i] >= g.T2) { t2[i] -= g.T2; b[i] += 1; }
    }
  }
};

LASR_DEV int xcd_remap(int orig, int nwg) {
  const int xcd = orig & 7, q8 = nwg >> 3, r8 = nwg & 7;
  return (xcd < r8 ? xcd * (q8 + 1) : r8 * (q8 + 1) + (xcd - r8) * q8) + (orig >> 3);
}

template <int BM, int BN, bool AKC, bool BKC, typename TC, int S, int G, int KS, int NW = 4, int EPI = EPI_RT,
          bool SERIAL = false>
LASR_DEV void gemm_glds_tile(const GemmP& p, const int tx, const int ty, const int zz) {
  static_assert(G == G_LIN || (G == G_DW ? (!AKC && !BKC) : (AKC && (G == G_FWD) == BKC)),
                "gather instance operand orientation");
  static_assert(!SERIAL || (G == G_LIN && !AKC && !BKC && std::is_same<TC, float>::value && EPI == EPI_RT),
                "serial slices: fp32 weight gradients only");
  static_assert(KS == 1 || KS == 2, "k sub-tiles per ring stage");
  static_assert(NW == 4 || NW == 8, "4 waves (2 x 2) or 8 waves (2 x 4)");
  constexpr int BK = 32;
  constexpr int NT = NW * 64, WCOLS = NW / 2;
  constexpr int WM = BM / 2, WN = BN / WCOLS, FM = WM / 16, FN = WN / 16;
  constexpr int TILE = (BM + BN) * BK;
  constexpr int STAGE = KS * TILE;
  constexpr int MAIN_BYTES = S * STAGE * 2;
  constexpr int EPI_BYTES = WM * (BN + 4) * 4;
  constexpr int GL = (BM + BN) * 4 / NT;
  __shared__ __attribute__((aligned(16))) char smem_epi[MAIN_BYTES > EPI_BYTES ? MAIN_BYTES : EPI_BYTES];
  bf16_t* smem = reinterpret_cast<bf16_t*>(smem_epi);
  const int tid = threadIdx.x, lane = tid & 63, wid = tid >> 6;
  const int wr = wid / WCOLS, wc = wid % WCOLS;

  int s = SERIAL ? 0 : zz % p.split_k;
  const int z = SERIAL ? 0 : zz / p.split_k;
  const int z1 = z / p.batch_div, z2 = z % p.batch_div;
  const bf16_t* A = (const bf16_t*)p.A + z1 * p.sa1 + z2 * p.sa2;
  const bf16_t* B = (const bf16_t*)p.B + z1 * p.sb1 + z2 * p.sb2;
  const int m0 = ty * BM, n0 = tx * BN;
  int kbeg = s * p.kchunk;
  int kend = min(p.K, kbeg + p.kchunk);
  int nk = kend > kbeg ? (kend - kbeg + BK - 1) / BK : 0;
  const int64_t lda = AKC ? p.lda_m : p.lda_k, ldb = BKC ? p.ldb_n : p.ldb_k;

  f32x4 acc[FM][FN];
#pragma unroll
  for (int i = 0; i < FM; ++i)
#pragma unroll
    for (int j = 0; j < FN; ++j) acc[i][j] = (f32x4){0.f, 0.f, 0.f, 0.f};

  int nfull = (kend - kbeg) > 0 ? (kend - kbeg) / BK : 0;
  [[maybe_unused]] ConvRowsKC<BM, NT> ga;
  [[maybe_unused]] ConvRowsDW<BN, NT> gb;
  if constexpr (G == G_FWD) ga.init_fwd(p.cv, m0, p.M, tid);
  if constexpr (G == G_DX) ga.init_dx(p.cv, m0, p.M, tid);
  [[maybe_unused]] __shared__ int64_t dxrow[G == G_DX ? BM : 1];
  if constexpr (G == G_DX)
    for (int r = tid; r < BM; r += NT) dxrow[r] = dx_row(p.cv, min(m0 + r, p.M - 1));
  constexpr bool W1 = G == G_DX && EPI == EPI_AUX_RELU_W1;
  constexpr int XN = W1 ? (9 * BM + NT - 1) / NT : 1;
  [[maybe_unused]] float xr[XN];
  if constexpr (W1) {
    const ConvG& g = p.cv;
    const int pt = g.cls >> 1, pf = g.cls & 1;
    const int nI = (g.T1 - pt + 1) >> 1, nJ = (g.F1 - pf + 1) >> 1;
#pragma unroll
    for (int i = 0; i < XN; ++i) {
      const int e = i * NT + tid, r = e / 9, k = e - 9 * r;
      xr[i] = 0.f;
      if (e < 9 * BM) {
        const int m = min(m0 + r, p.M - 1);
        const int j = m % nJ, t = m / nJ, ii = t % nI, b = t / nI;
        const int kh = k / 3, kw = k - 3 * kh;
        xr[i] = g.x[((int64_t)b * g.T0 + 2 * (2 * ii + pt) + kh) * g.F0 + 2 * (2 * j + pf) + kw];
      }
    }
  }
  if constexpr (G == G_DW) gb.init(p.cv, n0, p.N, kbeg, tid);
  auto issue_sub = [&](const int k0, bf16_t* dst) {
    if (LASR_EXP & 4) return;
    if constexpr (G == G_LIN) {
// ... 337 lines not shown
  const int64_t total = MN * p.batch;
  const float al = alpha_of(p);
  const uint32_t dkey = epi_key(p);
  if (p.v4) {
    const int64_t sstride = (int64_t)p.batch * MN;
    for (int64_t i4 = (int64_t)bx * 256 + threadIdx.x; i4 < total / 4; i4 += (int64_t)nbx * 256) {
      const int64_t i = i4 * 4;
      const int z = (int)(i / MN);
      const int64_t r = i - (int64_t)z * MN;
      const float* src = p.ws + (int64_t)z * MN + r;
      float acc[4] = {0.f, 0.f, 0.f, 0.f};
      int sl = 0;
      for (; sl + 4 <= p.split_k; sl += 4) {
        f32x4 v[4];
#pragma unroll
        for (int u = 0; u < 4; ++u) v[u] = *(const f32x4*)(src + (int64_t)(sl + u) * sstride);
#pragma unroll
        for (int u = 0; u < 4; ++u)
#pragma unroll
          for (int e = 0; e < 4; ++e) acc[e] += v[u][e];
      }
      for (; sl < p.split_k; ++sl) {
        const f32x4 v = *(const f32x4*)(src + (int64_t)sl * sstride);
#pragma unroll
        for (int e = 0; e < 4; ++e) acc[e] += v[e];
      }
      const int m = (int)(r / p.N), n = (int)(r - (int64_t)m * p.N);
      epi_store4<TC, true>(p, dkey, z / p.batch_div, z % p.batch_div, z, m, n, 4, acc, al);
    }
  } else {
    for (int64_t i = (int64_t)bx * 256 + threadIdx.x; i < total; i += (int64_t)nbx * 256) {
      const int z = (int)(i / MN);
      const int64_t r = i - (int64_t)z * MN;
      float acc = 0.f;
      for (int s = 0; s < p.split_k; ++s) acc += p.ws[((int64_t)s * p.batch + z) * MN + r];
      const int m = (int)(r / p.N), n = (int)(r - (int64_t)m * p.N);
      epi_store<TC>(p, dkey, z / p.batch_div, z % p.batch_div, z, m, n, acc, al);
    }
  }
  if (p.rs_ws) {
    for (int64_t m = (int64_t)bx * 256 + threadIdx.x; m < p.M; m += (int64_t)nbx * 256) {
      float acc = 0.f;
      for (int s = 0; s < p.split_k; ++s) acc += p.rs_ws[(int64_t)s * p.M + m];
      p.rowsum[m] += acc;
    }
  }
}
template <typename TC>
__global__ __launch_bounds__(256) void splitk_reduce_kernel(GemmP p) {
  splitk_reduce_body<TC>(p, blockIdx.x, gridDim.x);
}


static inline int epi_code(const GemmP& p) {
  static const int on = [] { const char* e = getenv("LASR_EPI_SPEC"); return e && e[0] ? atoi(e) : 1; }();
  if (!on || p.split_k > 1 || p.beta != 0.f || p.alpha_dev || p.N % 8 != 0) return EPI_RT;
  if (p.res) {
    return !p.zout && p.act == LASR_ACT_NONE && !p.aux && p.drop.p > 0.f && p.epi_mode == 1 ? EPI_RES_DROP : EPI_RT;
  }
  if (!p.zout && p.act == LASR_ACT_NONE && !p.aux && p.drop.p <= 0.f && p.epi_mode == 0) return EPI_PLAIN;
  if (!p.zout && p.act == LASR_ACT_RELU && !p.aux && p.drop.p <= 0.f && p.epi_mode == 0) return EPI_RELU;
  if (!p.zout && p.act == LASR_ACT_NONE && p.aux && p.aux_act == LASR_ACT_RELU && p.drop.p <= 0.f && p.epi_mode == 1)
    return EPI_AUX_RELU;
  if (p.zout && p.zout_mode == 1 && p.act == LASR_ACT_SWISH && p.drop.p > 0.f && !p.aux && p.epi_mode == 0)
    return EPI_SWISH_GATE_DROP;
  if (p.zout && p.zout_mode == 1 && p.act == LASR_ACT_RELU && p.drop.p > 0.f && !p.aux && p.epi_mode == 0)
    return EPI_RELU_GATE_DROP;
  if (!p.zout && p.act == LASR_ACT_NONE && p.aux && p.aux_act == LASR_ACT_GATE && p.drop.p <= 0.f && p.epi_mode == 1)
    return EPI_AUX_GATE;
  return EPI_RT;
}

static inline bool aligned16(const void* ptr) { return ((uintptr_t)ptr & 15) == 0; }
```

### liteasr_amd/csrc/gemm_launch.h

```cpp
#pragma once
#include "gemm_kernel.h"

template <bool AKC, bool BKC, typename TC>
void launch_bf16(const GemmP& p, int BM, int BN, int ks, int nw, bool glds, dim3 grid, hipStream_t st) {
  (void)nw;
  if (glds && ks == 2 && BM < 256) {
    if (BN == 256) gemm_bf16_glds_kernel<128, 256, AKC, BKC, TC, 2, 1, G_LIN, 2><<<grid, 256, 0, st>>>(p);
    else if (BM == 128 && BN == 128) gemm_bf16_glds_kernel<128, 128, AKC, BKC, TC, 2, 2, G_LIN, 2><<<grid, 256, 0, st>>>(p);
    else if (BM == 128) gemm_bf16_glds_kernel<128, 64, AKC, BKC, TC, 3, 2, G_LIN, 2><<<grid, 256, 0, st>>>(p);
    else if (BN == 128) gemm_bf16_glds_kernel<64, 128, AKC, BKC, TC, 3, 2, G_LIN, 2><<<grid, 256, 0, st>>>(p);
    else {
      const int e = epi_code(p);
#define L64(E) gemm_bf16_glds_kernel<64, 64, AKC, BKC, TC, 3, 3, G_LIN, 2, 4, E><<<grid, 256, 0, st>>>(p)
      if constexpr (AKC && std::is_same<TC, bf16_t>::value) {
        if (e == EPI_PLAIN) { L64(EPI_PLAIN); return; }
      }
      if constexpr (AKC && !BKC && std::is_same<TC, bf16_t>::value) {
        if (e == EPI_AUX_GATE) { L64(EPI_AUX_GATE); return; }
      }
      if constexpr (AKC && BKC && std::is_same<TC, bf16_t>::value) {
        if (e == EPI_RELU_GATE_DROP) { L64(EPI_RELU_GATE_DROP); return; }
      }
#undef L64
      if constexpr (AKC && BKC && std::is_same<TC, float>::value) {
        if (e == EPI_RES_DROP) {
          gemm_bf16_glds_kernel<64, 64, AKC, BKC, TC, 3, 3, G_LIN, 2, 4, EPI_RES_DROP><<<grid, 256, 0, st>>>(p);
          return;
        }
      }
      gemm_bf16_glds_kernel<64, 64, AKC, BKC, TC, 3, 3, G_LIN, 2><<<grid, 256, 0, st>>>(p);
    }
    return;
  }
  if (glds) {
    if (BM == 256 && BN == 256) gemm_bf16_glds_kernel<256, 256, AKC, BKC, TC, 3, 1><<<grid, 256, 0, st>>>(p);
    else if (BM == 256) gemm_bf16_glds_kernel<256, 128, AKC, BKC, TC, 3, 2><<<grid, 256, 0, st>>>(p);
    else if (BN == 256) {
      const int e = epi_code(p);
      if constexpr (AKC && BKC && std::is_same<TC, bf16_t>::value) {
        if (e == EPI_SWISH_GATE_DROP) {
          gemm_bf16_glds_kernel<128, 256, AKC, BKC, TC, 3, 2, G_LIN, 1, 4, EPI_SWISH_GATE_DROP><<<grid, 256, 0, st>>>(p);
          return;
        }
      }
      if constexpr (AKC && !BKC && std::is_same<TC, bf16_t>::value) {
        if (e == EPI_AUX_GATE) {
          gemm_bf16_glds_kernel<128, 256, AKC, BKC, TC, 3, 2, G_LIN, 1, 4, EPI_AUX_GATE><<<grid, 256, 0, st>>>(p);
          return;
        }
        if (e == EPI_AUX_RELU) {
          gemm_bf16_glds_kernel<128, 256, AKC, BKC, TC, 3, 2, G_LIN, 1, 4, EPI_AUX_RELU><<<grid, 256, 0, st>>>(p);
          return;
        }
      }
      gemm_bf16_glds_kernel<128, 256, AKC, BKC, TC, 3, 2><<<grid, 256, 0, st>>>(p);
    }
    else if (BM == 128 && BN == 128) {
      if constexpr (AKC && BKC && std::is_same<TC, bf16_t>::value) {
        if (epi_code(p) == EPI_PLAIN) {
          gemm_bf16_glds_kernel<128, 128, AKC, BKC, TC, 3, 3, G_LIN, 1, 4, EPI_PLAIN><<<grid, 256, 0, st>>>(p);
          return;
        }
      }
      gemm_bf16_glds_kernel<128, 128, AKC, BKC, TC, 3><<<grid, 256, 0, st>>>(p);
    }
    else if (BM == 128) {
      if constexpr (AKC && BKC && std::is_same<TC, bf16_t>::value) {
        if (epi_code(p) == EPI_PLAIN) {
          gemm_bf16_glds_kernel<128, 64, AKC, BKC, TC, 4, 3, G_LIN, 1, 4, EPI_PLAIN><<<grid, 256, 0, st>>>(p);
          return;
        }
// ... 22 lines not shown
```

### liteasr_amd/csrc/gemm_row.hip

```cpp
#include "gemm_kernel.h"
#include "ln_math.h"

namespace {

constexpr int RB = 32;
constexpr int BK = 32;
constexpr int KS = 2;

template <int D>
struct RowCfg {
  static constexpr int NT = 512;
  static constexpr int WN = D / 4;
  static constexpr int FN = WN / 16;
  static constexpr int NPL = D / 64;
  static constexpr int RW = RB / 8;
  static constexpr int TILE = (RB + D) * BK;
  static constexpr int STAGE = KS * TILE;
  static constexpr int S = D == 256 ? 4 : 2;
  static constexpr int GLB = KS * D * 4 / NT;
  static constexpr int GLA = GLB + 1;
  static constexpr int LDC = D + 4;
  static constexpr int RPW = NPL <= 8 ? 1 : 2;
  static constexpr int SMEM = S * STAGE * 2;
  static_assert(SMEM >= (RB * LDC + RB * D) * 4, "epilogue staging must fit the ring");
};

struct RowP {
  int M, K;
  const bf16_t* A;
  int64_t lda;
  const bf16_t* W;
  int64_t ldw;
  const float* g1;
  const float* b1;
  float eps;
  float* mean1;
  float* rstd1;
  const float* bias;
  const float* res;
  float res_scale;
  DropCfg drop;
  float* out;
  void* y1;
  const float* g2;
  const float* b2;
  bf16_t* y2;
  float* mean2;
  float* rstd2;
  const float* x;
  const float* dres;
  float* dx;
  bf16_t* gb;
  float bscale;
  DropCfg bd;
  float* part;
};

template <int D>
LASR_DEV void issue_a(const RowP& p, int m0, int k0, bf16_t* stage, int tid) {
  const int u = tid >> 7, P = tid & 127, r = P >> 2, c = (P & 3) ^ swz(r);
  const int gr = min(m0 + r, p.M - 1);
  const bf16_t* src = p.A + (int64_t)gr * p.lda + k0 + u * BK + c * 8;
  __builtin_amdgcn_global_load_lds((gptr_t)src, (lptr_t)(stage + u * RowCfg<D>::TILE + (P & ~63) * 8), 16, 0,
                                   0);
}

template <int R_TILE, bool KC>
LASR_DEV void glds_tile512(const bf16_t* base, int64_t ld, int R, int k0, bf16_t* dst, int tid) {
  constexpr int PER = R_TILE * 4 / 512;
  const int wid = tid >> 6;
#pragma unroll
  for (int i = 0; i < PER; ++i) {
    const int P = i * 512 + tid;
    const bf16_t* src;
    if (KC) {
      const int r = P >> 2, c = (P & 3) ^ swz(r);
      src = base + (int64_t)min(r, R - 1) * ld + k0 + c * 8;
    } else {
      constexpr int CPR = R_TILE / 8;
      const int k = P / CPR, ps = P % CPR;
      const int ls = ((((ps >> 1) ^ htr<R_TILE>(k))) << 1) | (ps & 1);
      src = base + (int64_t)(k0 + k) * ld + min(ls * 8, ((R + 7) & ~7) - 8);
    }
    __builtin_amdgcn_global_load_lds((gptr_t)src, (lptr_t)(dst + (i * 512 + wid * 64) * 8), 16, 0, 0);
  }
}

template <int D, bool BKC>
LASR_DEV void row_mainloop(const RowP& p, int m0, bf16_t* smem) {
  using Cf = RowCfg<D>;
  constexpr int FN = Cf::FN, S = Cf::S;
  const int tid = threadIdx.x, lane = tid & 63, wid = tid >> 6;
  const int wr = wid >> 2, wc = wid & 3;
  f32x4 acc[FN];
#pragma unroll
  for (int j = 0; j < FN; ++j) acc[j] = (f32x4){0.f, 0.f, 0.f, 0.f};

  auto issue = [&](int t) {
    bf16_t* dst = smem + (t % S) * Cf::STAGE;
    const int k0 = t * (KS * BK);
    if (wid < 4) issue_a<D>(p, m0, k0, dst, tid);
#pragma unroll
    for (int u = 0; u < KS; ++u) glds_tile512<D, BKC>(p.W, p.ldw, D, k0 + u * BK, dst + u * Cf::TILE + RB * BK, tid);
  };
  auto compute = [&](const bf16_t* cur) {
    bf16x8 bfr[FN];
    v2i rb[2 * FN];
    const bf16x8 af = frag<RB, true>(cur, wr * 16, lane);
#pragma unroll
    for (int j = 0; j < FN; ++j) {
      if constexpr (BKC) bfr[j] = frag<D, true>(cur + RB * BK, wc * Cf::WN + j * 16, lane);
      else frag_tr_raw<D>(cur + RB * BK, wc * Cf::WN + j * 16, lane, rb + 2 * j);
    }
    if constexpr (!BKC) {
      tie_lgkm<2 * FN>(rb);
#pragma unroll
      for (int j = 0; j < FN; ++j) bfr[j] = frag_from_raw(rb + 2 * j);
    }
#pragma unroll
    for (int j = 0; j < FN; ++j) acc[j] = __builtin_amdgcn_mfma_f32_16x16x32_bf16(bfr[j], af, acc[j], 0, 0, 0);
  };

  const int nst = p.K / (KS * BK);
#pragma unroll
  for (int t = 0; t < S - 1; ++t)
    if (t < nst) issue(t);
  for (int kt = 0; kt < nst; ++kt) {
    const int after = min(S - 2, nst - 1 - kt);
    if (wid < 4) wait_ring<S, Cf::GLA>(after);
    else wait_ring<S, Cf::GLB>(after);
    lds_barrier();
    if (kt + S - 1 < nst) issue(kt + S - 1);
#pragma unroll
    for (int u = 0; u < KS; ++u) compute(smem + (kt % S) * Cf::STAGE + u * Cf::TILE);
  }
  __syncthreads();
  float* cs = reinterpret_cast<float*>(smem);
  const int cl = lane & 15, rq = (lane >> 4) * 4;
#pragma unroll
  for (int j = 0; j < FN; ++j) *(f32x4*)(cs + (wr * 16 + cl) * Cf::LDC + wc * Cf::WN + j * 16 + rq) = acc[j];
  __syncthreads();
}

template <int D, typename TY1>
__global__ __launch_bounds__(512, 1) void row_res_ln_kernel(RowP p) {
  using Cf = RowCfg<D>;
  constexpr int NPL = Cf::NPL, RW = Cf::RW;
  __shared__ __attribute__((aligned(16))) char smem_raw[Cf::SMEM];
  bf16_t* smem = reinterpret_cast<bf16_t*>(smem_raw);
  const int m0 = blockIdx.x * RB;
  const int lane = threadIdx.x & 63, wid = threadIdx.x >> 6, c0 = lane * NPL;
  float rv[RW][NPL];
#pragma unroll
  for (int it = 0; it < RW; ++it) ldv<NPL>(p.res + (int64_t)min(m0 + it * 8 + wid, p.M - 1) * D + c0, rv[it]);
  float bv[NPL], g1[NPL], b1[NPL], g2[NPL], b2[NPL];
  if (p.bias) ldv<NPL>(p.bias + c0, bv);
  else
#pragma unroll
    for (int q = 0; q < NPL; ++q) bv[q] = 0.f;
  ldv<NPL>(p.g1 + c0, g1);
  ldv<NPL>(p.b1 + c0, b1);
  if (p.g2) {
    ldv<NPL>(p.g2 + c0, g2);
    ldv<NPL>(p.b2 + c0, b2);
  }
  row_mainloop<D, true>(p, m0, smem);

  const float* cs = reinterpret_cast<const float*>(smem_raw);
  const bool drop = p.drop.p > 0.f;
  const uint32_t key = drop ? drop_key(p.drop) : 0u;
#pragma unroll
  for (int it = 0; it < RW; ++it) {
    const int r = it * 8 + wid, m = m0 + r;
    if (m < p.M) {
      float v[NPL];
#pragma unroll
      for (int q = 0; q < NPL; ++q) v[q] = cs[r * Cf::LDC + c0 + q] * 1.f + bv[q];
      if (drop) {
        const uint32_t km = drop_keep_mask<NPL>(p.drop, key, (uint64_t)m * D + c0);
#pragma unroll
        for (int q = 0; q < NPL; ++q) v[q] *= (km >> q) & 1u ? p.drop.scale : 0.f;
      }
#pragma unroll
      for (int q = 0; q < NPL; ++q) v[q] = rv[it][q] + p.res_scale * v[q];
      stv<NPL>(p.out + (int64_t)m * D + c0, v);
      float o[NPL], mu, rs;
      ln_fwd_row<D, NPL>(v, g1, b1, p.eps, o, mu, rs);
      if (lane == 0) { p.mean1[m] = mu; p.rstd1[m] = rs; }
      stv<NPL>((TY1*)p.y1 + (int64_t)m * D + c0, o);
      if (p.g2) {
        float z[NPL];
        ln_fwd_row<D, NPL>(o, g2, b2, p.eps, z, mu, rs);
        if (lane == 0) { p.mean2[m] = mu; p.rstd2[m] = rs; }
        stv<NPL>(p.y2 + (int64_t)m * D + c0, z);
      }
    }
  }
}

template <int D>
__global__ __launch_bounds__(512, 1) void row_dx_ln_bwd_kernel(RowP p) {
  using Cf = RowCfg<D>;
  constexpr int NPL = Cf::NPL, RPW = Cf::RPW, LDC = Cf::LDC, NG = Cf::RW;
  static_assert(RPW == 1, "row groups of more than one row: D > 512 is not instantiated");
  __shared__ __attribute__((aligned(16))) char smem_raw[Cf::SMEM];
  bf16_t* smem = reinterpret_cast<bf16_t*>(smem_raw);
  const int m0 = blockIdx.x * RB;
  const int lane = threadIdx.x & 63, wid = threadIdx.x >> 6, c0 = lane * NPL;
  float xv[NG][NPL], rv[NG][NPL], mu[NG], rs[NG];
#pragma unroll
  for (int it = 0; it < NG; ++it) {
    const int m = min(m0 + it * 8 + wid, p.M - 1);
    ldv<NPL>(p.x + (int64_t)m * D + c0, xv[it]);
    if (p.dres) ldv<NPL>(p.dres + (int64_t)m * D + c0, rv[it]);
    mu[it] = p.mean1[m];
    rs[it] = p.rstd1[m];
  }
  float gm[NPL];
  ldv<NPL>(p.g1 + c0, gm);
// ... 31 lines not shown
    }
  }
  __syncthreads();
#pragma unroll
  for (int hh = 0; hh < RB / 16 * D / Cf::NT; ++hh) {
    const int h = D == 256 ? (int)(threadIdx.x >> 8) : hh, c = threadIdx.x % D;
    if (m0 + h * 16 >= p.M) continue;
    float* dst = p.part + (int64_t)(m0 / 16 + h) * 2 * D;
    {
      float a = 0.f, b = 0.f;
#pragma unroll
      for (int k = 0; k < 16; ++k) {
        a += cs[(h * 16 + k) * LDC + c];
        b += pb[(h * 16 + k) * D + c];
      }
      dst[c] = a;
      dst[D + c] = b;
    }
  }
}

bool al16(const void* q) { return ((uintptr_t)q & 15) == 0; }

}

static int row_common(const lasr_row_ln_args* a, RowP& p, const char* who) {
  LASR_CHECK_ARG(a != nullptr, "%s: null args", who);
  LASR_CHECK_ARG(a->D == 256 || a->D == 512, "%s: D=%d (256 or 512)", who, a->D);
  LASR_CHECK_ARG(a->M >= 0 && a->K > 0 && a->K % 64 == 0, "%s: K=%d must be a positive multiple of 64", who, a->K);
  LASR_CHECK_ARG(a->A && a->W && al16(a->A) && al16(a->W) && a->lda % 8 == 0 && a->ldw % 8 == 0 &&
                     a->lda >= a->K,
                 "%s: A / W must be 16-B aligned with row strides a multiple of 8", who);
  LASR_CHECK_ARG(a->gamma1 && a->mean1 && a->rstd1 && al16(a->gamma1), "%s: gamma1 / mean1 / rstd1 required", who);
  p = RowP{};
  p.M = a->M; p.K = a->K;
  p.A = (const bf16_t*)a->A; p.lda = a->lda;
  p.W = (const bf16_t*)a->W; p.ldw = a->ldw;
  p.g1 = a->gamma1; p.b1 = a->beta1; p.eps = a->eps; p.mean1 = a->mean1; p.rstd1 = a->rstd1;
  return LASR_OK;
}

extern "C" int lasr_linear_res_ln(const lasr_row_ln_args* a, void* stream) {
  RowP p;
  int rc = row_common(a, p, "lasr_linear_res_ln");
  if (rc) return rc;
  LASR_CHECK_ARG(a->ldw >= a->K, "lasr_linear_res_ln: W is [D, K] (ldw >= K)");
  LASR_CHECK_ARG(a->res && a->out && a->y1 && a->beta1 && al16(a->res) && al16(a->out) && al16(a->y1) &&
                     al16(a->beta1) && (!a->bias || al16(a->bias)),
                 "lasr_linear_res_ln: res / out / y1 / beta1 required, 16-B aligned");
  LASR_CHECK_ARG(a->y1_dtype == LASR_BF16 || a->y1_dtype == LASR_F32, "lasr_linear_res_ln: y1 bf16 or fp32");
  LASR_CHECK_ARG(!a->gamma2 || (a->y1_dtype == LASR_F32 && a->beta2 && a->y2 && a->mean2 && a->rstd2 &&
                                al16(a->gamma2) && al16(a->beta2) && al16(a->y2)),
                 "lasr_linear_res_ln: the chained norm needs an fp32 y1 and gamma2 / beta2 / y2 / mean2 / rstd2");
  if (a->M == 0) return LASR_OK;
  p.bias = a->bias; p.res = a->res; p.res_scale = a->res_scale;
  p.drop = mkdrop(a->drop_p, a->drop_seed);
  p.out = a->out; p.y1 = a->y1;
  p.g2 = a->gamma2; p.b2 = a->beta2; p.y2 = (bf16_t*)a->y2; p.mean2 = a->mean2; p.rstd2 = a->rstd2;
  const dim3 grid((unsigned)cdiv(a->M, RB));
  hipStream_t st = (hipStream_t)stream;
  if (a->D == 256) {
    if (a->y1_dtype == LASR_F32) row_res_ln_kernel<256, float><<<grid, 512, 0, st>>>(p);
    else row_res_ln_kernel<256, bf16_t><<<grid, 512, 0, st>>>(p);
  } else {
    if (a->y1_dtype == LASR_F32) row_res_ln_kernel<512, float><<<grid, 512, 0, st>>>(p);
    else row_res_ln_kernel<512, bf16_t><<<grid, 512, 0, st>>>(p);
  }
  return lasr_check_launch("lasr_linear_res_ln");
}

extern "C" int lasr_linear_dx_ln_bwd(const lasr_row_ln_args* a, void* stream) {
  RowP p;
  int rc = row_common(a, p, "lasr_linear_dx_ln_bwd");
  if (rc) return rc;
  LASR_CHECK_ARG(a->ldw >= a->D, "lasr_linear_dx_ln_bwd: W is [K, D] (ldw >= D)");
  LASR_CHECK_ARG(!a->dgamma == !a->dbeta, "lasr_linear_dx_ln_bwd: dgamma and dbeta together (or neither)");
  LASR_CHECK_ARG(a->x && a->dx && a->part && al16(a->x) && al16(a->dx) && al16(a->part) &&
                     (!a->dres || al16(a->dres)) && (!a->gb || al16(a->gb)),
                 "lasr_linear_dx_ln_bwd: x / dx / part required, 16-B aligned");
  if (a->M == 0) return LASR_OK;
  p.x = a->x; p.dres = a->dres; p.dx = a->dx; p.gb = (bf16_t*)a->gb; p.bscale = a->bscale;
  p.bd = mkdrop(a->bp, a->bseed);
  p.part = a->part;
  const dim3 grid((unsigned)cdiv(a->M, RB));
  hipStream_t st = (hipStream_t)stream;
  if (a->D == 256) row_dx_ln_bwd_kernel<256><<<grid, 512, 0, st>>>(p);
  else row_dx_ln_bwd_kernel<512><<<grid, 512, 0, st>>>(p);
  rc = lasr_check_launch("lasr_linear_dx_ln_bwd");
  if (rc || !a->dgamma) return rc;
  return lasr_reduce_cols(a->part, (int)cdiv(a->M, 16), 2 * a->D, a->dgamma, a->dbeta, a->D, 1, st);
}
```

### liteasr_amd/kernels.py

```python

from __future__ import annotations

import contextlib
import os
import ctypes as C
import math
from types import SimpleNamespace
from typing import Optional

import torch

from . import _native as N

_DT = {torch.float32: N.F32, torch.bfloat16: N.BF16}


def dt(t: torch.Tensor) -> int:
    try:
        return _DT[t.dtype]
    except KeyError:
        raise TypeError(f"unsupported dtype {t.dtype}") from None


def ptr(t: Optional[torch.Tensor]):
# ... 186 lines not shown
    segs = _DEFER.held + _DEFER.segs
    _DEFER.held, _DEFER.segs = [], []
    done, _DEFER.done = _DEFER.done, []
    if segs or _DEFER.gemms:
        _flush_node_end(segs)
    for fn in done:
        fn()



GEMM_NARROW_TILES = True
_narrow_set = [None]


def _split(t: torch.Tensor):
    nb = t.dim() - 2
    assert 0 <= nb <= 2, "gemm operands take at most 2 batch dims"
    st = t.stride()
    sh = t.shape
    if nb == 0:
        return (0, 0), (1, 1), st[0], st[1]
    if nb == 1:
        return (st[0], 0), (sh[0], 1), st[1], st[2]
    return (st[0], st[1]), (sh[0], sh[1]), st[2], st[3]


def gemm(
    a: torch.Tensor,
    b: torch.Tensor,
    c: torch.Tensor,
    *,
    alpha: float = 1.0,
    alpha_dev: Optional[torch.Tensor] = None,
    beta: float = 0.0,
    bias: Optional[torch.Tensor] = None,
    act: int = N.ACT_NONE,
    zout: Optional[torch.Tensor] = None,
    aux: Optional[torch.Tensor] = None,
    aux_act: int = N.ACT_NONE,
    drop_p: float = 0.0,
    drop_seed: int = 0,
    res: Optional[torch.Tensor] = None,
    res_scale: float = 1.0,
    split_k: int = 1,
    rowsum: Optional[torch.Tensor] = None,
    plan_only: bool = False,
    zout_mode: int = 0,
    group: bool = False,
    tile: Optional[tuple] = None,
    ksub: int = 0,
    ln_fwd: Optional[tuple] = None,
    ln_bwd: Optional[object] = None,
    qbias: Optional[tuple] = None,
):
    if _narrow_set[0] != GEMM_NARROW_TILES:
        N.call("lasr_gemm_narrow_tiles", int(GEMM_NARROW_TILES))
        _narrow_set[0] = GEMM_NARROW_TILES
    M, K = a.shape[-2], a.shape[-1]
    K2, Nn = b.shape[-2], b.shape[-1]
    assert K == K2 and c.shape[-2] == M and c.shape[-1] == Nn, (a.shape, b.shape, c.shape)
    assert a.dtype == b.dtype
    (sa1, sa2), (za1, za2), a_m, a_k = _split(a)
    (sb1, sb2), (zb1, zb2), b_k, b_n = _split(b)
    (sc1, sc2), (zc1, zc2), c_m, c_n = _split(c)
    assert c_n == 1, "C must be row-contiguous"
    z1, z2 = zc1, zc2
    assert (za1, za2) == (z1, z2) and (zb1, zb2) == (z1, z2), "batch shapes differ"
    if a_k != 1 and a_m != 1:
        raise ValueError("A needs a unit stride")
    if b_k != 1 and b_n != 1:
        raise ValueError("B needs a unit stride")
    args = N.GemmArgs()
    args.M, args.N, args.K = M, Nn, K
    args.batch, args.batch_div = z1 * z2, z2
    args.A, args.lda_m, args.lda_k, args.sa1, args.sa2 = ptr(a), a_m, a_k, sa1, sa2
    args.B, args.ldb_n, args.ldb_k, args.sb1, args.sb2 = ptr(b), b_n, b_k, sb1, sb2
    args.C, args.ldc, args.sc1, args.sc2 = ptr(c), c_m, sc1, sc2
    if a_k == 1 and a_m == 1:
        args.lda_k = 1
    if b_k == 1 and b_n == 1:
        args.ldb_k = 1
    args.in_dtype, args.c_dtype = dt(a), dt(c)
    args.alpha, args.alpha_dev, args.beta = alpha, ptr(alpha_dev), beta
    args.bias = ptr(bias)
    args.act = act
    args.zout = ptr(zout)
    args.zout_mode = zout_mode
    if aux is not None:
        args.aux, args.aux_dtype, args.ldaux, args.aux_act = ptr(aux), dt(aux), aux.stride(0), aux_act
    args.drop_p, args.drop_seed = drop_p, drop_seed
    if tile is not None:
        args.tile_m, args.tile_n = int(tile[0]), int(tile[1])
    args.ksub = int(ksub)
    if res is not None:
        args.res, args.res_dtype, args.ldres, args.res_scale = ptr(res), dt(res), res.stride(0), res_scale
    auto_split = (split_k == 1 and SMALL_GRID_SPLIT and rowsum is None and zout is None and not group
                  and a.dtype == torch.bfloat16 and z1 * z2 == 1 and K >= 1024
                  and ((M + 63) // 64) * ((Nn + 63) // 64) < SMALL_GRID_TILES)
    if auto_split:
        split_k = 0
    args.split_k = split_k
    if rowsum is not None:
        assert rowsum.dtype == torch.float32 and rowsum.is_contiguous() and rowsum.numel() == M
        assert z1 * z2 == 1 and a_m == 1, "rowsum needs batch 1 and an M-contiguous A"
        args.rowsum = ptr(rowsum)
    if split_k != 1 or rowsum is not None:
# ... 36 lines not shown
            return c
        if sp > 1:
            nrs = (sp + 128) * M if rowsum is not None else 0
            part = torch.empty(sp * M * Nn + nrs, dtype=torch.float32, device=c.device)
            args.split_k = -sp
            args.workspace, args.workspace_bytes = ptr(part), part.numel() * 4
            if grouped:
                key = _GROUP_TILES[(tm.value, tn.value)]
                _DEFER.gemms.append((key, N.GemmArgs.from_buffer_copy(args), (a, b)))
            else:
                N.call("lasr_gemm", C.byref(args), stream())
            _defer(part, sp, M * Nn, c, accumulate=beta == 1.0)
            if rowsum is not None and fl.value & 2:
                _defer(part[sp * M * Nn:], sp, M, rowsum)
            return c
    if ln_fwd is not None:
        g_, b_, eps, y, mean, rstd = ln_fwd
        assert c.dtype == torch.float32 and c.is_contiguous() and z1 * z2 == 1 and rowsum is None
        N.call("lasr_gemm_ln_fwd", C.byref(args), ptr(g_), ptr(b_), float(eps), ptr(y), dt(y), ptr(mean), ptr(rstd),
               stream())
        return c
    if qbias is not None:
        dqu, dqv, B_, T_, H_, dk_, dqkv, du, dv = qbias
        assert c.dtype == dqu.dtype == dqv.dtype == dqkv.dtype
        D_ = H_ * dk_
        nchunk = (B_ * T_ + 63) // 64
        part = torch.empty(nchunk * 2 * D_, dtype=torch.float32, device=c.device)
        N.call("lasr_gemm_qbias_bwd", C.byref(args), ptr(dqu), ptr(dqv), dt(dqu), B_, T_, H_, dk_, ptr(dqkv),
               dqkv.stride(0), ptr(part), part.numel(), stream())
        if _DEFER.depth:
            _defer(part, nchunk, 2 * D_, du, dv, split=D_)
        else:
            arr = (N.ReduceSeg * 1)()
            arr[0] = N.ReduceSeg(ptr(part), 2 * D_, nchunk, 1, ptr(du), ptr(dv), D_)
            N.call("lasr_reduce_multi", arr, 1, stream())
        return c
    if ln_bwd is not None:
        q = ln_bwd
        assert c.is_contiguous() and z1 * z2 == 1 and rowsum is None
        nblk = (M + 15) // 16
        defer = _DEFER.depth and q.dgamma is not None and q.dbeta is not None
        part = torch.empty(nblk * 2 * Nn, dtype=torch.float32, device=c.device)
        N.call("lasr_gemm_ln_bwd", C.byref(args), ptr(q.x), dt(q.x), ptr(q.g), ptr(q.mean), ptr(q.rstd),
               ptr(q.dres), dt(q.dres) if q.dres is not None else 0, ptr(q.dx), dt(q.dx), ptr(part), part.numel(),
               ptr(q.gb), dt(q.gb) if q.gb is not None else 0, float(q.bscale), float(q.bp), int(q.bseed), stream())
        if defer:
            _defer(part, nblk, 2 * Nn, q.dgamma, q.dbeta, split=Nn)
        elif q.dgamma is not None or q.dbeta is not None:
            assert q.dgamma is not None and q.dbeta is not None
            arr = (N.ReduceSeg * 1)()
            arr[0] = N.ReduceSeg(ptr(part), 2 * Nn, nblk, 1, ptr(q.dgamma), ptr(q.dbeta), Nn)
            N.call("lasr_reduce_multi", arr, 1, stream())
        return c
    N.call("lasr_gemm", C.byref(args), stream())
    return c


def gemm_plan(a, b, c, flags=False, **kw):
    return gemm(a, b, c, plan_only="flags" if flags else True, **kw)


def linear(x, w, out, bias=None, **kw):
    return gemm(x, w.t(), out, bias=bias, **kw)


def dropout_scale(p: float) -> float:
    return float(N.load().lasr_dropout_scale(float(p))) if p > 0 else 1.0


def colsum(x2d: torch.Tensor, out: torch.Tensor, accumulate=True):
    M, Nn = x2d.shape
    nchunk = max(1, min((M + 63) // 64, 128))
    ws = WS.get(nchunk * Nn, x2d.device)
    N.call("lasr_colsum", ptr(x2d), dt(x2d), M, Nn, x2d.stride(0), ptr(out), int(accumulate),
           ptr(ws), ws.numel(), stream())


def layernorm_fwd(x, gamma, beta, eps, y, mean, rstd, y2=None, p2=0.0, seed2=0):
    rows, D = x.shape
    N.call("lasr_layernorm_fwd", ptr(x), dt(x), rows, D, ptr(gamma), ptr(beta), eps, ptr(y),
           dt(y), ptr(mean), ptr(rstd), ptr(y2), dt(y2) if y2 is not None else 0, p2, seed2,
           stream())


def layernorm2_fwd(x, g1, b1, g2, b2, eps, y, mean1, rstd1, z, mean2, rstd2):
    rows, D = x.shape
    N.call("lasr_layernorm2_fwd", ptr(x), rows, D, ptr(g1), ptr(b1), ptr(g2), ptr(b2), eps, ptr(y), ptr(mean1),
           ptr(rstd1), ptr(z), ptr(mean2), ptr(rstd2), stream())


def layernorm_bwd(x, dy, gamma, mean, rstd, dx, dgamma, dbeta, dres=None, gb=None,
                  bscale=1.0, bp=0.0, bseed=0):
    rows, D = x.shape
    nblk = (rows + 15) // 16
    defer = _DEFER.depth and dgamma is not None and dbeta is not None
    if defer:
        ws = torch.empty(nblk * 2 * D, dtype=torch.float32, device=x.device)
        og, ob = None, None
    else:
        ws = WS.get(nblk * 2 * D, x.device)
        og, ob = dgamma, dbeta
    N.call("lasr_layernorm_bwd", ptr(x), dt(x), ptr(dy), dt(dy), rows, D, ptr(gamma), ptr(mean),
           ptr(rstd), ptr(dres), dt(dres) if dres is not None else 0, ptr(dx), dt(dx),
           ptr(og), ptr(ob), ptr(ws), ws.numel(), ptr(gb),
           dt(gb) if gb is not None else 0, bscale, bp, bseed, stream())
    if defer:
        _defer(ws, nblk, 2 * D, dgamma, dbeta, split=D)


def layernorm2_bwd(x1, dy1, dres1, g1, mean1, rstd1, dgamma1, dbeta1, x2, g2, mean2, rstd2, dx2, dgamma2, dbeta2,
                   gb2=None, bscale=1.0, bp=0.0, bseed=0):
    rows, D = x1.shape
    assert x1.dtype == x2.dtype == dres1.dtype == dx2.dtype == torch.float32
    assert dy1.shape == x1.shape == x2.shape == dres1.shape == dx2.shape
    nblk = (rows + 15) // 16
    part1 = torch.empty(nblk * 2 * D, dtype=torch.float32, device=x1.device)
    part2 = torch.empty(nblk * 2 * D, dtype=torch.float32, device=x1.device)
    N.call("lasr_layernorm2_bwd", ptr(x1), ptr(dy1), dt(dy1), ptr(dres1), rows, D, ptr(g1), ptr(mean1), ptr(rstd1),
           ptr(part1), ptr(x2), ptr(g2), ptr(mean2), ptr(rstd2), ptr(dx2), ptr(part2), ptr(gb2),
           dt(gb2) if gb2 is not None else 0, bscale, bp, bseed, stream())
    if _DEFER.depth:
        _defer(part1, nblk, 2 * D, dgamma1, dbeta1, split=D)
        _defer(part2, nblk, 2 * D, dgamma2, dbeta2, split=D)
        return
    arr = (N.ReduceSeg * 2)()
    arr[0] = N.ReduceSeg(ptr(part1), 2 * D, nblk, 1, ptr(dgamma1), ptr(dbeta1), D)
    arr[1] = N.ReduceSeg(ptr(part2), 2 * D, nblk, 1, ptr(dgamma2), ptr(dbeta2), D)
    N.call("lasr_reduce_multi", arr, 2, stream())


def _al16(t):
    return t is None or t.data_ptr() % 16 == 0


ROW_LN_MAX_K = 1024
ROW_LN_MAX_D = 256


def row_ln_ok(a, w, D, max_k=None, max_d=None):
    Kd = a.shape[-1]
    return (a.dtype == torch.bfloat16 and w.dtype == torch.bfloat16 and D in (256, 512)
            and D <= (ROW_LN_MAX_D if max_d is None else max_d) and a.dim() == 2
            and Kd % 64 == 0 and Kd <= (ROW_LN_MAX_K if max_k is None else max_k) and a.stride(1) == 1
            and a.stride(0) % 8 == 0 and w.is_contiguous() and _al16(a) and _al16(w))


def linear_res_ln(x, w, out, y1, mean1, rstd1, g1, b1, eps, *, bias=None, res, res_scale=1.0, drop_p=0.0,
                  drop_seed=0, g2=None, b2=None, y2=None, mean2=None, rstd2=None):
    M, Kd = x.shape
    D = w.shape[0]
    a = N.RowLnArgs()
    a.M, a.D, a.K = M, D, Kd
    a.A, a.lda, a.W, a.ldw = ptr(x), x.stride(0), ptr(w), w.stride(0)
    a.gamma1, a.beta1, a.eps, a.mean1, a.rstd1 = ptr(g1), ptr(b1), eps, ptr(mean1), ptr(rstd1)
    a.bias, a.res, a.res_scale, a.drop_p, a.drop_seed = ptr(bias), ptr(res), res_scale, drop_p, drop_seed
    a.out, a.y1, a.y1_dtype = ptr(out), ptr(y1), dt(y1)
    if g2 is not None:
        a.gamma2, a.beta2, a.y2, a.mean2, a.rstd2 = ptr(g2), ptr(b2), ptr(y2), ptr(mean2), ptr(rstd2)
    N.call("lasr_linear_res_ln", C.byref(a), stream())


def linear_dx_ln_bwd(dy, w, x, gamma, mean, rstd, dx, dgamma, dbeta, dres=None, gb=None, bscale=1.0, bp=0.0,
                     bseed=0):
    M, Kd = dy.shape
    D = w.shape[1]
    nblk = (M + 15) // 16
    defer = _DEFER.depth and dgamma is not None and dbeta is not None
    part = torch.empty(nblk * 2 * D, dtype=torch.float32, device=dy.device) if defer else \
        WS.get(nblk * 2 * D, dy.device)
    a = N.RowLnArgs()
    a.M, a.D, a.K = M, D, Kd
    a.A, a.lda, a.W, a.ldw = ptr(dy), dy.stride(0), ptr(w), w.stride(0)
    a.gamma1, a.mean1, a.rstd1 = ptr(gamma), ptr(mean), ptr(rstd)
    a.x, a.dres, a.dx, a.gb, a.bscale, a.bp, a.bseed = ptr(x), ptr(dres), ptr(dx), ptr(gb), bscale, bp, bseed
    a.part = ptr(part)
    if not defer:
        a.dgamma, a.dbeta = ptr(dgamma), ptr(dbeta)
    N.call("lasr_linear_dx_ln_bwd", C.byref(a), stream())
    if defer:
        _defer(part, nblk, 2 * D, dgamma, dbeta, split=D)


def branch_grad(dx, gb, scale, p=0.0, seed=0):
    N.call("lasr_branch_grad", ptr(dx), dt(dx), dx.numel(), ptr(gb), dt(gb), scale, p, seed,
           stream())


def _rows_ld(x, lead):
    ld = x.stride(-2)
    assert x.stride(-1) == 1 and ld >= x.shape[-1], "logits rows must be unit-stride"
    for d in range(lead):
        assert x.stride(d) == ld * math.prod(x.shape[d + 1:-1]), "logits rows must be evenly spaced"
    return ld


def ctc_fwd(logits, targets, ilen, tlen, lse, lp, alpha, nll, beta=None):
    B, T, V = logits.shape
    Lmax = targets.shape[1]
    N.call("lasr_ctc_fwd", ptr(logits), dt(logits), B, T, V, _rows_ld(logits, 1), ptr(targets), Lmax,
           ptr(ilen), ptr(tlen), ptr(lse), ptr(lp), ptr(alpha), ptr(beta), ptr(nll), stream())


def ctc_bwd(logits, targets, ilen, tlen, lse, lp, alpha, nll, beta, grad, gscale, gdev=None,
            beta_ready=False):
    B, T, V = logits.shape
    Lmax = targets.shape[1]
    ld = _rows_ld(logits, 1)
    assert grad.shape == logits.shape and _rows_ld(grad, 1) == ld
    N.call("lasr_ctc_bwd", ptr(logits), dt(logits), B, T, V, ld, ptr(targets), Lmax, ptr(ilen),
           ptr(tlen), ptr(lse), ptr(lp), ptr(alpha), ptr(nll), ptr(beta), int(beta_ready), ptr(grad),
           dt(grad), gscale, ptr(gdev), stream())
# ... 225 lines not shown

def conv2_dx_w1(dy2, w2p, y1, x, dw1, db1):
    _conv2(N.CONV2_DX_W1, y1, None, w2p=w2p, dy2=dy2, x=x, dw1=dw1, db1=db1)


def permute_last2(src, Nn, A, Bd, dst, reverse=False, accumulate=False):
    N.call("lasr_permute_last2", ptr(src), dt(src), Nn, A, Bd, ptr(dst), dt(dst), int(reverse),
           int(accumulate), stream())


def dwconv_nparts(B, T):
    return N.load().lasr_dwconv_nparts(B, T)


def glu_dwconv_fwd(z1, B, T, Cc, K, w, bias, y, stats):
    N.call("lasr_glu_dwconv_fwd", ptr(z1), dt(z1), B, T, Cc, K, ptr(w), ptr(bias), ptr(y), dt(y),
           ptr(stats), stream())


def bn_finalize(stats, nparts, Cc, eps, momentum, gamma, beta, rmean, rvar, nbt, mean, rstd,
                scale, shift, update):
    N.call("lasr_bn_finalize", ptr(stats), nparts, Cc, eps, momentum, ptr(gamma), ptr(beta),
           ptr(rmean), ptr(rvar), ptr(nbt), ptr(mean), ptr(rstd), ptr(scale), ptr(shift),
           int(update), stream())


def bn_act_fwd(y, scale, shift, h, act=N.ACT_SWISH):
    rows, Cc = y.shape
    N.call("lasr_bn_act_fwd", ptr(y), dt(y), rows, Cc, ptr(scale), ptr(shift), ptr(h), dt(h), act, stream())


def bn_act_bwd(y, dh, scale, shift, mean, rstd, gamma, dgamma, dbeta, dy, batch_stats=True, act=N.ACT_SWISH):
    rows, Cc = y.shape
    ws = WS.get(((rows + 63) // 64 + 1) * 2 * Cc, y.device)
    N.call("lasr_bn_act_bwd", ptr(y), dt(y), ptr(dh), dt(dh), rows, Cc, ptr(scale), ptr(shift),
           ptr(mean), ptr(rstd), ptr(gamma), ptr(dgamma), ptr(dbeta), ptr(dy), dt(dy), ptr(ws),
           ws.numel(), int(bool(batch_stats)), act, stream())


def glu_dwconv_bwd(z1, dy, B, T, Cc, K, w, dz1, dw, db):
    nparts = dwconv_nparts(B, T)
    if _DEFER.depth:
        ws = torch.empty(nparts * (K + 1) * Cc, dtype=torch.float32, device=z1.device)
        N.call("lasr_glu_dwconv_bwd", ptr(z1), dt(z1), ptr(dy), dt(dy), B, T, Cc, K, ptr(w), ptr(dz1),
               None, None, ptr(ws), ws.numel(), stream())
        _defer(ws, nparts, (K + 1) * Cc, dw, db, split=K * Cc)
        return
    ws = WS.get((nparts + 1) * (K + 1) * Cc, z1.device)
    N.call("lasr_glu_dwconv_bwd", ptr(z1), dt(z1), ptr(dy), dt(dy), B, T, Cc, K, ptr(w), ptr(dz1),
           ptr(dw), ptr(db), ptr(ws), ws.numel(), stream())


def bn_act_glu_dwconv_bwd(y, dh, scale, shift, mean, rstd, gamma, dgamma, dbeta, z1, B, T, Cc, K, w, dz1, dw, db,
                          batch_stats=True, act=N.ACT_SWISH):
    rows = y.shape[0]
    assert rows == B * T and y.shape[1] == Cc and dh.shape == y.shape and z1.shape == (rows, 2 * Cc)
    bn_ws = torch.empty(((rows + 63) // 64 + 1) * 2 * Cc, dtype=torch.float32, device=y.device)
    nparts = dwconv_nparts(B, T)
    head = (ptr(y), dt(y), ptr(dh), dt(dh), B, T, Cc, ptr(scale), ptr(shift), ptr(mean), ptr(rstd), ptr(gamma),
            ptr(dgamma), ptr(dbeta), ptr(bn_ws), bn_ws.numel(), int(bool(batch_stats)), act, ptr(z1), dt(z1), K,
            ptr(w), ptr(dz1))
    if _DEFER.depth:
        ws = torch.empty(nparts * (K + 1) * Cc, dtype=torch.float32, device=z1.device)
        N.call("lasr_bn_act_glu_dwconv_bwd", *head, None, None, ptr(ws), ws.numel(), stream())
        _defer(ws, nparts, (K + 1) * Cc, dw, db, split=K * Cc)
        return
    ws = WS.get((nparts + 1) * (K + 1) * Cc, z1.device)
    N.call("lasr_bn_act_glu_dwconv_bwd", *head, ptr(dw), ptr(db), ptr(ws), ws.numel(), stream())


def cast(src, dst):
    N.call("lasr_cast", ptr(src), dt(src), ptr(dst), dt(dst), src.numel(), stream())


def scale_add(a, b, sa, sb, out):
    N.call("lasr_scale_add", ptr(a), dt(a), ptr(b), dt(b) if b is not None else 0, sa, sb,
           ptr(out), dt(out), out.numel(), stream())


def pe_fwd(x, rows, T, D, pe, xscale, y, p=0.0, seed=0):
    N.call("lasr_pe_fwd", ptr(x), dt(x) if x is not None else 0, rows, T, D, ptr(pe), xscale, p,
           seed, ptr(y), dt(y), stream())


def embed_pe_fwd(ids, L, E, pe, xscale, y, p=0.0, seed=0):
    R = ids.numel()
    D = E.shape[1]
    N.call("lasr_embed_pe_fwd", ptr(ids), R, L, D, ptr(E), ptr(pe), xscale, p, seed, ptr(y),
           dt(y), stream())


def embed_bwd(ids, dy, xscale, dE, p=0.0, seed=0):
    R = ids.numel()
    D = dE.shape[1]
    N.call("lasr_embed_bwd", ptr(ids), R, D, ptr(dy), dt(dy), xscale, p, seed, ptr(dE), stream())


def fill(t, value):
    N.call("lasr_fill", ptr(t), dt(t), t.numel(), float(value), stream())


CHUNK_NONE, CHUNK_FIXED, CHUNK_DEVICE, CHUNK_SAMPLE = 0, 1, 2, 3


def u2_prep(xlens, ys, ylens, Tx, Tsub, sos, eos, chunk, out, chunk_mode=None, chunk_dev=None, ctr=None,
            chunk_seed=0, chunk_max=25):
    B, L = ys.shape
    if chunk_mode is None:
        chunk_mode = CHUNK_FIXED if chunk > 0 else CHUNK_NONE
    dm, em = out["dec_mask"], out["enc_mask"]
    assert dm.is_contiguous() and dm.dim() == 3 and tuple(dm.shape[:2]) == (B, L + 1) and dm.shape[-1] >= L + 1
    assert em.is_contiguous() and em.dtype == torch.uint8 and em.numel() == B * Tsub
    cm, cld = None, 0
    if chunk_mode != CHUNK_NONE:
        cm = out["chunk_mask"]
        assert cm.is_contiguous() and cm.dim() == 3 and tuple(cm.shape[:2]) == (B, Tsub) and cm.shape[-1] >= Tsub
        cld = cm.shape[-1]
    if chunk_mode in (CHUNK_DEVICE, CHUNK_SAMPLE):
        assert chunk_dev is not None and chunk_dev.dtype == torch.int32 and chunk_dev.is_cuda
    if chunk_mode == CHUNK_SAMPLE:
        assert ctr is not None and ctr.dtype == torch.int64 and ctr.is_cuda
# ... 344 lines not shown
```

### liteasr_amd/nets/functional.py

```python

from __future__ import annotations

import math
from types import SimpleNamespace

import torch

from .. import kernels as K
from .._native import ACT_GATE, ACT_NONE, ACT_RELU, ACT_SWISH, ACT_TANH
from ..utils.markers import ranged
from .links import LayerLink

F32 = torch.float32
LN_EPS = 1e-12


def _e(shape, dtype, dev):
    return torch.empty(shape, dtype=dtype, device=dev)


def ld_scores(T):
    return (T + 7) // 8 * 8


def _seed(base, k):
    return (base * 0x100000001B3 + k * 0x9E3779B1 + 1) & 0xFFFFFFFFFFFFFFFF


def ln_forward(x, g, b, adt, y2=False, p2=0.0, seed2=0):
    rows, D = x.shape
    dev = x.device
    y = _e((rows, D), adt, dev)
    mean = _e(rows, F32, dev)
    rstd = _e(rows, F32, dev)
    yd = _e((rows, D), adt, dev) if y2 else None
    K.layernorm_fwd(x, g, b, LN_EPS, y, mean, rstd, yd, p2, seed2)
    return y, yd, mean, rstd


ROW_LN = True
DEC_ROW_LN = True
SPLITK_LN = True
QBIAS_IN_REDUCE = True
LN2_BWD_CHAIN = True
BN_GLU_FUSED = True
LAYER_RED_HOLD = True


def _link(env, layer):
    return env.links[layer] if env.links is not None else None


def _hold(link):
    return LAYER_RED_HOLD and link is not None and not link.floor


class PostLN:

    __slots__ = ("g", "b", "f32", "nxt", "y1", "m1", "r1", "y2", "m2", "r2")

    def __init__(self, ln, f32=False, nxt=None):
        self.g, self.b, self.f32, self.nxt = ln.g, ln.b, f32, nxt
        self.y1 = self.m1 = self.r1 = self.y2 = self.m2 = self.r2 = None


def norm_of(x, ln, adt, post=None):
    if post is not None and post.y1 is not None:
        return post.y1, post.m1, post.r1
    y, _, m, r = ln_forward(x, ln.g, ln.b, adt)
    return y, m, r


def res_proj(x, W, bias, res, res_scale, p_res, s_res, post=None):
    M, D = x.shape[0], W.shape[0]
    dev = x.device
    out = _e((M, D), F32, dev)
    if post is not None:
        post.y1 = None
    if post is None or not ROW_LN or not K.row_ln_ok(x, W, D):
        if post is not None and SPLITK_LN and post.nxt is None and x.dtype == torch.bfloat16 and W.shape[1] >= 1024:
            post.y1 = _e((M, D), F32 if post.f32 else x.dtype, dev)
            post.m1, post.r1 = _e(M, F32, dev), _e(M, F32, dev)
            K.linear(x, W, out, bias=bias, res=res, res_scale=res_scale, drop_p=p_res, drop_seed=s_res,
                     ln_fwd=(post.g, post.b, LN_EPS, post.y1, post.m1, post.r1))
            return out
        K.linear(x, W, out, bias=bias, res=res, res_scale=res_scale, drop_p=p_res, drop_seed=s_res)
        return out
    post.y1 = _e((M, D), F32 if post.f32 else x.dtype, dev)
    post.m1, post.r1 = _e(M, F32, dev), _e(M, F32, dev)
    kw = {}
    if post.nxt is not None:
        post.y2 = _e((M, D), x.dtype, dev)
        post.m2, post.r2 = _e(M, F32, dev), _e(M, F32, dev)
        kw = dict(g2=post.nxt[0], b2=post.nxt[1], y2=post.y2, mean2=post.m2, rstd2=post.r2)
    K.linear_res_ln(x, W, out, post.y1, post.m1, post.r1, post.g, post.b, LN_EPS, bias=bias, res=res,
                    res_scale=res_scale, drop_p=p_res, drop_seed=s_res, **kw)
    return out


class LnBwd:

    __slots__ = ("x", "g", "mean", "rstd", "dx", "dgamma", "dbeta", "dres", "gb", "bscale", "bp", "bseed", "chain")

    def __init__(self, x, g, mean, rstd, dx, dgamma, dbeta, dres=None, gb=None, bscale=1.0, bp=0.0, bseed=0,
                 chain=None):
        self.x, self.g, self.mean, self.rstd, self.dx, self.dgamma, self.dbeta = x, g, mean, rstd, dx, dgamma, dbeta
        self.dres, self.gb, self.bscale, self.bp, self.bseed, self.chain = dres, gb, bscale, bp, bseed, chain


def dx_ln(dy, W, lnb):
    M, D = dy.shape[0], W.shape[1]
    ch = lnb.chain if lnb is not None else None
    if lnb is not None and ROW_LN and K.row_ln_ok(dy, W, D) and lnb.x.dtype == F32 and lnb.dx.dtype == F32:
        K.linear_dx_ln_bwd(dy, W, lnb.x, lnb.g, lnb.mean, lnb.rstd, lnb.dx, lnb.dgamma, lnb.dbeta,
                           dres=lnb.dres, gb=lnb.gb, bscale=lnb.bscale, bp=lnb.bp, bseed=lnb.bseed)
        if ch is not None:
            ln_bwd_of(lnb.dx, ch)
        return None
    dln = _e((M, D), dy.dtype, dy.device)
    if ch is not None:
        assert lnb.gb is None and lnb.dres is not None and ch.dres is None and lnb.x.dtype == F32
        K.gemm(dy, W, dln)
        K.layernorm2_bwd(lnb.x, dln, lnb.dres, lnb.g, lnb.mean, lnb.rstd, lnb.dgamma, lnb.dbeta, ch.x, ch.g,
                         ch.mean, ch.rstd, ch.dx, ch.dgamma, ch.dbeta, gb2=ch.gb, bscale=ch.bscale, bp=ch.bp,
                         bseed=ch.bseed)
        return None
    if lnb is not None and SPLITK_LN and dy.dtype == torch.bfloat16 and W.shape[0] >= 1024:
        K.gemm(dy, W, dln, ln_bwd=lnb)
        return None
    K.gemm(dy, W, dln)
    if lnb is None:
        return dln
    ln_bwd_of(dln, lnb)
    return None


def ln_bwd_of(dln, lnb):
    K.layernorm_bwd(lnb.x, dln, lnb.g, lnb.mean, lnb.rstd, lnb.dx, lnb.dgamma, lnb.dbeta, dres=lnb.dres,
                    gb=lnb.gb, bscale=lnb.bscale, bp=lnb.bp, bseed=lnb.bseed)


def ffn_forward(ln, W1, b1, W2, b2, act, p_ff, s_ff, res, res_scale, p_res, s_res, post=None):
    M = ln.shape[0]
    dev, adt = ln.device, ln.dtype
    h = _e((M, W1.shape[0]), adt, dev)
    g = _e((M, W1.shape[0]), adt, dev)
    K.linear(ln, W1, h, bias=b1, act=act, zout=g, zout_mode=1, drop_p=p_ff, drop_seed=s_ff)
    out = res_proj(h, W2, b2, res, res_scale, p_res, s_res, post)
    return out, g, h
# ... 238 lines not shown
        if own_kv:
            K.gemm(dkv.t(), mem, g.Wkv, beta=1.0, split_k=0, rowsum=g.bkv, group=True)
            K.gemm(dkv, w.Wkv, dmem, beta=1.0)
        return dx_ln(dq, w.Wq, lnb)
    dctx4 = _heads(dctx, B, Tq, H, dk)
    if mem is None:
        q4 = _slot(sv.qkv, B, Tq, 3, 0, H, dk)
        k4 = _slot(sv.qkv, B, Tk, 3, 1, H, dk)
        v4 = _slot(sv.qkv, B, Tk, 3, 2, H, dk)
        dqkv = _e((R, 3 * d), adt, dev)
        dq4, dk4, dv4 = (_slot(dqkv, B, Tq, 3, i, H, dk) for i in range(3))
    else:
        q4 = _heads(sv.q, B, Tq, H, dk)
        k4 = _slot(sv.kv, B, Tk, 2, 0, H, dk)
        v4 = _slot(sv.kv, B, Tk, 2, 1, H, dk)
        dq = _e((R, d), adt, dev)
        if own_kv:
            dkv = _e((B * Tk, 2 * d), adt, dev)
        dq4 = _heads(dq, B, Tq, H, dk)
        dk4 = _slot(dkv, B, Tk, 2, 0, H, dk)
        dv4 = _slot(dkv, B, Tk, 2, 1, H, dk)
    dPd = _e((B, H, Tq, ldS), F32, dev)
    K.gemm(dctx4, v4.transpose(-1, -2), dPd[..., :Tk])
    K.gemm(sv.P[..., :Tk].transpose(-1, -2), dctx4, dv4)
    dS = _e((B, H, Tq, ldS), adt, dev)
    K.attn_softmax_bwd(sv.Praw if sv.Praw is not None else sv.P, dPd, B, H, Tq, Tk, ldS, mask, msb,
                       msq, dS, p_att, s_att)
    K.gemm(dS[..., :Tk], k4, dq4, alpha=scale)
    K.gemm(dS[..., :Tk].transpose(-1, -2), q4, dk4, alpha=scale)
    if mem is None:
        K.gemm(dqkv.t(), ln, g.Wqkv, beta=1.0, split_k=0, rowsum=g.bqkv, group=True)
        return dx_ln(dqkv, w.Wqkv, lnb)
    K.gemm(dq.t(), ln, g.Wq, beta=1.0, split_k=0, rowsum=g.bq, group=True)
    if own_kv:
        K.gemm(dkv.t(), mem, g.Wkv, beta=1.0, split_k=0, rowsum=g.bkv, group=True)
        K.gemm(dkv, w.Wkv, dmem, beta=1.0)
    return dx_ln(dq, w.Wq, lnb)


def conv_forward(ln, w, env, x_in, p_res, s_res, training, post=None):
    B, T = env.B, env.T
    M, d = ln.shape
    dev, adt = ln.device, ln.dtype
    z1 = _e((M, 2 * d), adt, dev)
    K.linear(ln, w.Wpw1, z1, bias=w.bpw1)
    y = _e((M, d), adt, dev)
    nparts = K.dwconv_nparts(B, T)
    stats = _e(nparts * 3 * d, F32, dev)
    K.glu_dwconv_fwd(z1, B, T, d, w.kernel, w.wdw, w.bdw, y, stats)
    mean, rstd, scale, shift = (_e(d, F32, dev) for _ in range(4))
    K.bn_finalize(stats, nparts, d, 1e-5, 0.1, w.gamma, w.beta, w.rmean, w.rvar, w.nbt, mean, rstd,
                  scale, shift, 1 if training else 2)
    h3 = _e((M, d), adt, dev)
    K.bn_act_fwd(y, scale, shift, h3, act=getattr(w, "act", ACT_SWISH))
    out = res_proj(h3, w.Wpw2, w.bpw2, x_in, 1.0, p_res, s_res, post)
    return out, SimpleNamespace(z1=z1, y=y, mean=mean, rstd=rstd, scale=scale, shift=shift, h3=h3,
                                training=training)


def conv_backward(gb, ln, sv, w, g, env, lnb=None):
    B, T = env.B, env.T
    M, d = ln.shape
    dev, adt = ln.device, ln.dtype
    K.gemm(gb.t(), sv.h3, g.Wpw2, beta=1.0, split_k=0, rowsum=g.bpw2, group=True)
    dh3 = _e((M, d), adt, dev)
    K.gemm(gb, w.Wpw2, dh3)
    dz1 = _e((M, 2 * d), adt, dev)
    if BN_GLU_FUSED and d % 8 == 0:
        K.bn_act_glu_dwconv_bwd(sv.y, dh3, sv.scale, sv.shift, sv.mean, sv.rstd, w.gamma, g.gamma, g.beta, sv.z1,
                                B, T, d, w.kernel, w.wdw, dz1, g.wdw, g.bdw, batch_stats=sv.training,
                                act=getattr(w, "act", ACT_SWISH))
    else:
        dy = _e((M, d), F32, dev)
        K.bn_act_bwd(sv.y, dh3, sv.scale, sv.shift, sv.mean, sv.rstd, w.gamma, g.gamma, g.beta, dy,
                     batch_stats=sv.training, act=getattr(w, "act", ACT_SWISH))
        K.glu_dwconv_bwd(sv.z1, dy, B, T, d, w.kernel, w.wdw, dz1, g.wdw, g.bdw)
    K.gemm(dz1.t(), ln, g.Wpw1, beta=1.0, split_k=0, rowsum=g.bpw1, group=True)
    return dx_ln(dz1, w.Wpw1, lnb)


def _conv2_implicit(adt, C):
    return adt == torch.bfloat16 and C % 128 == 0


@ranged
class EmbedConvFn(torch.autograd.Function):

    @staticmethod
    def forward(ctx, xs, anchor, mod, env):
        B, Tx, Fd = xs.shape
        w = mod.weights()
        C = w.C
        adt, dev = env.adt, xs.device
        T1, F1 = (Tx - 3) // 2 + 1, (Fd - 3) // 2 + 1
        T2, F2 = (T1 - 3) // 2 + 1, (F1 - 3) // 2 + 1
        M2 = B * T2 * F2
        xs = xs.contiguous()
        y1 = _e((B, T1, F1, C), adt, dev)
        K.conv1_fwd(xs, w.W1, w.b1, y1)
        y2_full = _e((K.conv2_dy2_rows(M2), C), adt, dev)
        y2_full[M2:].zero_()
        y2 = y2_full[:M2]
        implicit = _conv2_implicit(adt, C)
        if implicit:
            col = None
            K.conv2_fwd(y1, w.W2p, w.b2, y2)
        else:
            col = _e((M2, 9 * C), adt, dev)
            K.im2col(y1, col)
            K.linear(col, w.W2p, y2, bias=w.b2, act=ACT_RELU)
        ctx.sv = SimpleNamespace(xs=xs, y1=y1, col=col, dims=(B, T1, F1, T2, F2, C), implicit=implicit)
        ctx.mod, ctx.env = mod, env
        return y2_full

    @staticmethod
    def backward(ctx, dy2_full):
        sv, mod = ctx.sv, ctx.mod
        B, T1, F1, T2, F2, C = sv.dims
        w, g = mod.weights(), mod.grads()
        M2 = B * T2 * F2
        dev = dy2_full.device
        dW2 = _e((C, 9 * C), F32, dev)
        if sv.implicit and K.conv2_dx_w1_ok(C):
            K.conv2_dw(dy2_full, sv.y1, dW2, rowsum=g.b2)
# ... 925 lines not shown
```

Measured before the change: 3495 utterances/sec.

## Fuse BatchNorm-activation into pw2 row kernel and BN-grad sums into dx GEMM epilogue

```diff
diff --git a/include/liteasr_hip.h b/include/liteasr_hip.h
--- a/include/liteasr_hip.h
+++ b/include/liteasr_hip.h
@@ -40,6 +40,10 @@
   int zout_mode;
   int tile_m, tile_n;
   int ksub;
+  const void* bn_y;
+  const float* bn_scale; const float* bn_shift; const float* bn_mean; const float* bn_rstd;
+  float* bn_part;
+  int bn_act;
 } lasr_gemm_args;
 int lasr_gemm(const lasr_gemm_args* args, void* stream);
 int lasr_gemm_ln_fwd(const lasr_gemm_args* args, const float* gamma, const float* beta, float eps, void* y,
@@ -55,6 +59,7 @@
 #define LASR_PLAN_ROWSUM_FUSED 2
 #define LASR_PLAN_KSUB2 4
 #define LASR_PLAN_WIDE 8
+#define LASR_PLAN_BN_SUMS 16
 int lasr_gemm_plan(const lasr_gemm_args* args, int* tile_m, int* tile_n, int* split_k, int* flags);
 
 int lasr_gemm_dw_group(const lasr_gemm_args* args, int n, void* stream);
@@ -98,6 +103,7 @@
   const float* gamma2; const float* beta2; void* y2; float* mean2; float* rstd2;
   const float* x; const float* dres; float* dx; void* gb; float bscale; float bp; uint64_t bseed;
   float* part; float* dgamma; float* dbeta;
+  const float* a_scale; const float* a_shift; int a_act; void* a_out;
 } lasr_row_ln_args;
 int lasr_linear_res_ln(const lasr_row_ln_args* args, void* stream);
 int lasr_linear_dx_ln_bwd(const lasr_row_ln_args* args, void* stream);
@@ -240,6 +246,12 @@
                                int64_t bn_ws_floats, int batch_stats, int act, const void* z1, int dt, int K,
                                const float* w, void* dz1, float* dw, float* db, float* ws, int64_t ws_floats,
                                void* stream);
+int lasr_bn_sums_glu_dwconv_bwd(const void* y, int ydt, const void* dh, int hdt, int B, int T, int C,
+                                const float* scale, const float* shift, const float* mean, const float* rstd,
+                                const float* gamma, float* dgamma, float* dbeta, float* bn_ws,
+                                int64_t bn_ws_floats, int batch_stats, int act, const void* z1, int dt, int K,
+                                const float* w, void* dz1, float* dw, float* db, float* ws, int64_t ws_floats,
+                                void* stream);
 
 int lasr_cast(const void* src, int sdt, void* dst, int ddt, int64_t n, void* stream);
 int lasr_scale_add(const void* a, int adt, const void* b, int bdt, float sa, float sb,
diff --git a/liteasr_amd/_native.py b/liteasr_amd/_native.py
--- a/liteasr_amd/_native.py
+++ b/liteasr_amd/_native.py
@@ -9,6 +9,7 @@
 
 F32, BF16, I32, I64, U8 = 0, 1, 2, 3, 4
 ACT_NONE, ACT_RELU, ACT_SWISH, ACT_GATE, ACT_TANH = 0, 1, 2, 3, 4
+PLAN_BN_SUMS = 16
 
 _p = C.c_void_p
 _i = C.c_int
@@ -38,6 +39,8 @@
         ("rowsum", _p),
         ("zout_mode", _i),
         ("tile_m", _i), ("tile_n", _i), ("ksub", _i),
+        ("bn_y", _p), ("bn_scale", _p), ("bn_shift", _p), ("bn_mean", _p), ("bn_rstd", _p), ("bn_part", _p),
+        ("bn_act", _i),
     ]
 
 
@@ -89,6 +92,7 @@
         ("gamma2", _p), ("beta2", _p), ("y2", _p), ("mean2", _p), ("rstd2", _p),
         ("x", _p), ("dres", _p), ("dx", _p), ("gb", _p), ("bscale", _f), ("bp", _f), ("bseed", _u),
         ("part", _p), ("dgamma", _p), ("dbeta", _p),
+        ("a_scale", _p), ("a_shift", _p), ("a_act", _i), ("a_out", _p),
     ]
 
 
@@ -187,6 +191,8 @@
     "lasr_glu_dwconv_bwd": [_p, _i, _p, _i, _i, _i, _i, _i, _p, _p, _p, _p, _p, _l, _p],
     "lasr_bn_act_glu_dwconv_bwd": [_p, _i, _p, _i, _i, _i, _i, _p, _p, _p, _p, _p, _p, _p, _p, _l, _i, _i,
                                    _p, _i, _i, _p, _p, _p, _p, _p, _l, _p],
+    "lasr_bn_sums_glu_dwconv_bwd": [_p, _i, _p, _i, _i, _i, _i, _p, _p, _p, _p, _p, _p, _p, _p, _l, _i, _i,
+                                    _p, _i, _i, _p, _p, _p, _p, _p, _l, _p],
     "lasr_cast": [_p, _i, _p, _i, _l, _p],
     "lasr_scale_add": [_p, _i, _p, _i, _f, _f, _p, _i, _l, _p],
     "lasr_embed_pe_fwd": [_p, _i, _i, _i, _p, _p, _f, _f, _u, _p, _i, _p],
diff --git a/liteasr_amd/csrc/common.h b/liteasr_amd/csrc/common.h
--- a/liteasr_amd/csrc/common.h
+++ b/liteasr_amd/csrc/common.h
@@ -256,6 +256,16 @@
   const float s = sigmoidf_(z);
   return s * (1.f + z * (1.f - s));
 }
+template <bool RELU>
+LASR_DEV float bn_act(float u) {
+  if constexpr (RELU) return fmaxf(u, 0.f);
+  else return swishf(u);
+}
+template <bool RELU>
+LASR_DEV float bn_act_grad(float u) {
+  if constexpr (RELU) return u > 0.f ? 1.f : 0.f;
+  else return swish_grad(u);
+}
 
 void lasr_set_error(const char* fmt, ...);
 int lasr_check_launch(const char* what);
diff --git a/liteasr_amd/csrc/conv.hip b/liteasr_amd/csrc/conv.hip
--- a/liteasr_amd/csrc/conv.hip
+++ b/liteasr_amd/csrc/conv.hip
@@ -616,16 +616,6 @@
   bn_final_write(c, n, mu, m2, eps, momentum, gamma, beta, rmean, rvar, mean, rstd, scale, shift, update);
 }
 
-template <bool RELU>
-LASR_DEV float bn_act(float u) {
-  if constexpr (RELU) return fmaxf(u, 0.f);
-  else return swishf(u);
-}
-template <bool RELU>
-LASR_DEV float bn_act_grad(float u) {
-  if constexpr (RELU) return u > 0.f ? 1.f : 0.f;
-  else return swish_grad(u);
-}
 
 template <bool RELU>
 LASR_DEV float bn_dy(float yv, float gv, float sc, float sf, float mu, float rs, float ga, float t1, float t2,
@@ -1013,12 +1003,12 @@
                                                             gamma, tot, dgamma, dbeta, inv_n, C});
 }
 
-extern "C" int lasr_bn_act_glu_dwconv_bwd(const void* y, int ydt, const void* dh, int hdt, int B, int T, int C,
-                                          const float* scale, const float* shift, const float* mean,
-                                          const float* rstd, const float* gamma, float* dgamma, float* dbeta,
-                                          float* bn_ws, int64_t bn_ws_floats, int batch_stats, int act,
-                                          const void* z1, int dt, int K, const float* w, void* dz1, float* dw,
-                                          float* db, float* ws, int64_t ws_floats, void* stream) {
+static int bn_act_glu_dwconv_bwd_run(bool parts_ready, const void* y, int ydt, const void* dh, int hdt, int B, int T,
+                                     int C, const float* scale, const float* shift, const float* mean,
+                                     const float* rstd, const float* gamma, float* dgamma, float* dbeta,
+                                     float* bn_ws, int64_t bn_ws_floats, int batch_stats, int act,
+                                     const void* z1, int dt, int K, const float* w, void* dz1, float* dw,
+                                     float* db, float* ws, int64_t ws_floats, void* stream) {
   const int64_t rows = (int64_t)B * T;
   const int64_t nparts_bn = cdiv(rows, BN_ROWS);
   LASR_CHECK_ARG(bn_ws_floats >= (nparts_bn + 1) * 2 * C, "lasr_bn_act_glu_dwconv_bwd: BN workspace too small");
@@ -1033,7 +1023,7 @@
   LASR_CHECK_ARG(ws_floats >= (int64_t)nparts * (DW_K + 1) * C, "lasr_bn_act_glu_dwconv_bwd: workspace too small");
   hipStream_t st = (hipStream_t)stream;
   float* tot = bn_ws + nparts_bn * 2 * C;
-  {
+  if (!parts_ready) {
     dim3 g((unsigned)cdiv(C, 2 * BN_CP), (unsigned)nparts_bn);
 #define BR(RL, TY, TH) bn_act_bwd_reduce_kernel<TY, TH, RL><<<g, 256, 0, st>>>((const TY*)y, (const TH*)dh, rows, C, scale, shift, mean, rstd, bn_ws)
     const bool relu = act == LASR_ACT_RELU, yf = ydt == LASR_F32, hf = hdt == LASR_F32;
@@ -1046,8 +1036,8 @@
     }
 #undef BR
     if (int rc = lasr_check_launch("bn_act_glu_dwconv_bwd/reduce")) return rc;
-    if (int rc = lasr_reduce_cols(bn_ws, (int)nparts_bn, 2 * C, tot, nullptr, 2 * C, 0, st)) return rc;
-  }
+  }
+  if (int rc = lasr_reduce_cols(bn_ws, (int)nparts_bn, 2 * C, tot, nullptr, 2 * C, 0, st)) return rc;
   const float inv_n = batch_stats ? 1.f / (float)rows : 0.f;
   dim3 g((unsigned)nparts, (unsigned)cdiv(C, 2 * DW_CP));
   const int vec = ((uintptr_t)z1 & 15) == 0 && ((uintptr_t)y & 15) == 0 && ((uintptr_t)dh & 15) == 0 &&
@@ -1068,3 +1058,25 @@
   LASR_CHECK_ARG(dw && db, "lasr_bn_act_glu_dwconv_bwd: dw and db go together");
   return lasr_reduce_cols(ws, nparts, (int64_t)(DW_K + 1) * C, dw, db, (int64_t)DW_K * C, 1, st);
 }
+
+extern "C" int lasr_bn_act_glu_dwconv_bwd(const void* y, int ydt, const void* dh, int hdt, int B, int T, int C,
+                                          const float* scale, const float* shift, const float* mean,
+                                          const float* rstd, const float* gamma, float* dgamma, float* dbeta,
+                                          float* bn_ws, int64_t bn_ws_floats, int batch_stats, int act,
+                                          const void* z1, int dt, int K, const float* w, void* dz1, float* dw,
+                                          float* db, float* ws, int64_t ws_floats, void* stream) {
+  return bn_act_glu_dwconv_bwd_run(false, y, ydt, dh, hdt, B, T, C, scale, shift, mean, rstd, gamma, dgamma, dbeta,
+                                   bn_ws, bn_ws_floats, batch_stats, act, z1, dt, K, w, dz1, dw, db, ws, ws_floats,
+                                   stream);
+}
+
+extern "C" int lasr_bn_sums_glu_dwconv_bwd(const void* y, int ydt, const void* dh, int hdt, int B, int T, int C,
+                                           const float* scale, const float* shift, const float* mean,
+                                           const float* rstd, const float* gamma, float* dgamma, float* dbeta,
+                                           float* bn_ws, int64_t bn_ws_floats, int batch_stats, int act,
+                                           const void* z1, int dt, int K, const float* w, void* dz1, float* dw,
+                                           float* db, float* ws, int64_t ws_floats, void* stream) {
+  return bn_act_glu_dwconv_bwd_run(true, y, ydt, dh, hdt, B, T, C, scale, shift, mean, rstd, gamma, dgamma, dbeta,
+                                   bn_ws, bn_ws_floats, batch_stats, act, z1, dt, K, w, dz1, dw, db, ws, ws_floats,
+                                   stream);
+}
diff --git a/liteasr_amd/csrc/gemm.hip b/liteasr_amd/csrc/gemm.hip
--- a/liteasr_amd/csrc/gemm.hip
+++ b/liteasr_amd/csrc/gemm.hip
@@ -112,6 +112,14 @@
                                   (tm < 256 || tn >= 128) && (tn < 256 || tm >= 128));
 }
 
+static bool bn_sums_ok(const lasr_gemm_args* a, int BM, int BN, int split, int ks, bool glds) {
+  const int batch = a->batch > 0 ? a->batch : 1;
+  return glds && BM == 64 && BN == 64 && split == 1 && ks == 2 && batch == 1 && a->N % 64 == 0 && a->lda_k == 1 &&
+         a->ldb_k != 1 && a->c_dtype == LASR_BF16 && !a->zout && a->act == LASR_ACT_NONE && !a->aux && !a->res &&
+         a->drop_p <= 0.f && a->beta == 0.f && !a->alpha_dev && !a->rowsum && aligned16(a->C) && a->ldc % 8 == 0 &&
+         epi_spec_on();
+}
+
 extern "C" int lasr_gemm_plan(const lasr_gemm_args* a, int* tile_m, int* tile_n, int* split_k, int* flags) {
   LASR_CHECK_ARG(a && tile_m && tile_n && split_k, "lasr_gemm_plan: null argument");
   int ks = 1, nw = 4;
@@ -125,7 +133,8 @@
   if (flags) {
     *flags = (glds ? LASR_PLAN_GLDS : 0) | (a->rowsum && glds && a->lda_k != 1 ? LASR_PLAN_ROWSUM_FUSED : 0) |
              (glds && ks == 2 && (*tile_m < 256 || nw == 8) ? LASR_PLAN_KSUB2 : 0) |
-             (glds && nw == 8 ? LASR_PLAN_WIDE : 0);
+             (glds && nw == 8 ? LASR_PLAN_WIDE : 0) |
+             (bn_sums_ok(a, *tile_m, *tile_n, *split_k, ks, glds) ? LASR_PLAN_BN_SUMS : 0);
   }
   return LASR_OK;
 }
@@ -146,6 +155,18 @@
   LASR_CHECK_ARG(tile_ok(a->tile_m, a->tile_n) && a->ksub >= 0 && a->ksub <= 2,
                  "lasr_gemm: tile override must be 64/128/256 x 64/128/256 (256 only beside >= 128) or 0 x 0, "
                  "ksub 0, 1 or 2");
+  const bool bn_sums = a->bn_y || a->bn_scale || a->bn_shift || a->bn_mean || a->bn_rstd || a->bn_part || a->bn_act;
+  if (bn_sums) {
+    LASR_CHECK_ARG(a->bn_y && a->bn_scale && a->bn_shift && a->bn_mean && a->bn_rstd && a->bn_part,
+                   "lasr_gemm: bn_y, bn_scale, bn_shift, bn_mean, bn_rstd and bn_part go together");
+    LASR_CHECK_ARG(a->bn_act == LASR_ACT_SWISH || a->bn_act == LASR_ACT_RELU,
+                   "lasr_gemm: bn_act must be SWISH or RELU");
+    LASR_CHECK_ARG(a->c_dtype == LASR_BF16 && a->in_dtype == LASR_BF16,
+                   "lasr_gemm: the bn_* column sums need bf16 operands and a bf16 C");
+    LASR_CHECK_ARG(aligned16(a->bn_y) && aligned16(a->bn_scale) && aligned16(a->bn_shift) && aligned16(a->bn_mean) &&
+                       aligned16(a->bn_rstd) && aligned16(a->bn_part),
+                   "lasr_gemm: bn_y / bn_scale / bn_shift / bn_mean / bn_rstd / bn_part must be 16-B aligned");
+  }
   if (a->M == 0 || a->N == 0 || a->batch == 0) return LASR_OK;
   const int batch = a->batch > 0 ? a->batch : 1;
   const int bdiv = a->batch_div > 0 ? a->batch_div : 1;
@@ -215,6 +236,16 @@
   }
   dim3 grid((unsigned)cdiv(a->N, BN), (unsigned)cdiv(a->M, BM), (unsigned)(batch * split));
   LASR_CHECK_ARG(grid.y <= 65535 && grid.z <= 65535, "lasr_gemm: grid too large");
+  if (bn_sums) {
+    LASR_CHECK_ARG(bn_sums_ok(a, BM, BN, split, ks, glds),
+                   "lasr_gemm: the bn_* column sums ride only the plain bf16-out 64 x 64 LDS-DMA plan without a "
+                   "K split, N %% 64 == 0 (lasr_gemm_plan: LASR_PLAN_BN_SUMS); planned %d x %d, split %d",
+                   BM, BN, split);
+    p.aux = a->bn_y; p.aux_dtype = LASR_BF16; p.ldaux = a->N; p.aux_act = LASR_ACT_NONE; p.aux_vec = 1;
+    p.epi_mode = 1;
+    p.bn_scale = a->bn_scale; p.bn_shift = a->bn_shift; p.bn_mean = a->bn_mean; p.bn_rstd = a->bn_rstd;
+    p.bn_part = a->bn_part; p.bn_relu = a->bn_act == LASR_ACT_RELU;
+  }
   const bool rs_fused = a->rowsum && glds && !akc;
   if (rs_fused) {
     p.rowsum = a->rowsum;
diff --git a/liteasr_amd/csrc/gemm_kernel.h b/liteasr_amd/csrc/gemm_kernel.h
--- a/liteasr_amd/csrc/gemm_kernel.h
+++ b/liteasr_amd/csrc/gemm_kernel.h
@@ -59,6 +59,12 @@
   int v4;
   int zout_mode;
   ConvGeom cv;
+  const float* bn_scale = nullptr;
+  const float* bn_shift = nullptr;
+  const float* bn_mean = nullptr;
+  const float* bn_rstd = nullptr;
+  float* bn_part = nullptr;
+  int bn_relu = 0;
 };
 
 struct GemmRowPost {
@@ -76,7 +82,8 @@
 enum {
   EPI_RT = 0, EPI_SWISH_GATE_DROP = 1, EPI_AUX_GATE = 2, EPI_PLAIN = 3, EPI_RES_DROP = 4, EPI_RELU_GATE_DROP = 5,
   EPI_RELU = 6, EPI_AUX_RELU = 7,
-  EPI_AUX_RELU_W1 = 8
+  EPI_AUX_RELU_W1 = 8,
+  EPI_BN_SUMS = 9
 };
 
 template <int N, int EPI = EPI_RT, typename ZST>
@@ -126,7 +133,7 @@
 #pragma unroll
     for (int q = 0; q < N; ++q) v[q] *= auxv[q] > 0.f ? 1.f : 0.f;
     return;
-  } else if constexpr (EPI == EPI_PLAIN) {
+  } else if constexpr (EPI == EPI_PLAIN || EPI == EPI_BN_SUMS) {
     return;
   } else if constexpr (EPI == EPI_RES_DROP) {
     const uint32_t km = drop_keep_mask_even<N>(p.drop, dkey, dbase);
@@ -295,6 +302,50 @@
   const int nI = (g.T1 - pt + 1) >> 1, nJ = (g.F1 - pf + 1) >> 1;
   const int j = m % nJ, t = m / nJ, i = t % nI, b = t / nI;
   return ((int64_t)(b * g.T1 + 2 * i + pt) * g.F1 + 2 * j + pf) * g.C;
+}
+
+struct BnSumsLds {
+  static constexpr int T = 64;
+  static constexpr int G = 8;
+  static constexpr int DH = (T / 2) * (T + 4) * 4;
+  static constexpr int Y = DH + T * T * 2;
+  static constexpr int SP = Y + T * T * 2;
+  static constexpr int END = SP + G * 2 * T * 4;
+};
+
+template <bool RELU>
+LASR_DEV void bn_sums_tile(const GemmP& p, char* smem_epi, int m0, int n0, const float* sc, const float* sf,
+                           const float* mu, const float* rs) {
+  using L = BnSumsLds;
+  const bf16_t* dhs = reinterpret_cast<const bf16_t*>(smem_epi + L::DH);
+  const bf16_t* ys = reinterpret_cast<const bf16_t*>(smem_epi + L::Y);
+  float (*sp)[2][L::T] = reinterpret_cast<float (*)[2][L::T]>(smem_epi + L::SP);
+  const int cp = threadIdx.x % 32, grp = threadIdx.x / 32;
+  float s1[2] = {0.f, 0.f}, s2[2] = {0.f, 0.f};
+  const int r1 = min(L::T, p.M - m0);
+  for (int r = grp; r < r1; r += L::G) {
+    float yv[2], gv[2];
+    ldv<2>(ys + r * L::T + 2 * cp, yv);
+    ldv<2>(dhs + r * L::T + 2 * cp, gv);
+#pragma unroll
+    for (int q = 0; q < 2; ++q) {
+      const float du = gv[q] * bn_act_grad<RELU>(yv[q] * sc[q] + sf[q]);
+      s1[q] += du;
+      s2[q] += du * (yv[q] - mu[q]) * rs[q];
+    }
+  }
+#pragma unroll
+  for (int q = 0; q < 2; ++q) {
+    sp[grp][0][2 * cp + q] = s1[q];
+    sp[grp][1][2 * cp + q] = s2[q];
+  }
+  __syncthreads();
+  if (threadIdx.x >= 2 * L::T) return;
+  const int which = threadIdx.x / L::T, cl = threadIdx.x % L::T;
+  float v = sp[0][which][cl];
+#pragma unroll
+  for (int q = 1; q < L::G; ++q) v += sp[q][which][cl];
+  p.bn_part[(int64_t)(m0 / L::T) * 2 * p.N + (int64_t)which * p.N + n0 + cl] = v;
 }
 
 template <int BM, int BN, typename TC, bool TRANS = false, int G = G_LIN, int NW = 4, int EPI = EPI_RT>
@@ -332,6 +383,17 @@
   const void* src = p.aux ? p.aux : p.res;
   const int src_dt = p.aux ? p.aux_dtype : p.res_dtype;
   const int64_t src_ld = p.aux ? p.ldaux : p.ldres;
+  [[maybe_unused]] float bsc[2], bsf[2], bmu[2], brs[2];
+  if constexpr (EPI == EPI_BN_SUMS) {
+    static_assert(BM == BnSumsLds::T && BN == BnSumsLds::T && NW == 4 && G == G_LIN &&
+                      std::is_same<TC, bf16_t>::value,
+                  "EPI_BN_SUMS: the 64 x 64 bf16-out tile on 4 waves");
+    const int c = n0 + 2 * (tid % 32);
+    ldv<2>(p.bn_scale + c, bsc);
+    ldv<2>(p.bn_shift + c, bsf);
+    ldv<2>(p.bn_mean + c, bmu);
+    ldv<2>(p.bn_rstd + c, brs);
+  }
 #pragma unroll
   for (int h = 0; h < 2; ++h) {
     constexpr int PF = ITERS < 2 ? ITERS : 2;
@@ -386,6 +448,13 @@
 #pragma unroll
             for (int q = 0; q < 8; ++q) a8[q] = cs[r * LDC + ec8 + q];
             epi_fast8<TC, EPI>(p, dkey, crow(m) + en, z, m, en, min(8, p.N - en), a8, al, bv, sv[it]);
+            if constexpr (EPI == EPI_BN_SUMS) {
+              float v8[8];
+#pragma unroll
+              for (int q = 0; q < 8; ++q) v8[q] = a8[q] * al + bv[q];
+              st8(reinterpret_cast<bf16_t*>(smem_epi + BnSumsLds::DH) + (h * WM + r) * BN + ec8, v8);
+              st8(reinterpret_cast<bf16_t*>(smem_epi + BnSumsLds::Y) + (h * WM + r) * BN + ec8, sv[it]);
+            }
           }
         }
       }
@@ -411,6 +480,10 @@
       }
     }
     __syncthreads();
+  }
+  if constexpr (EPI == EPI_BN_SUMS) {
+    if (p.bn_relu) bn_sums_tile<true>(p, smem_epi, m0, n0, bsc, bsf, bmu, brs);
+    else bn_sums_tile<false>(p, smem_epi, m0, n0, bsc, bsf, bmu, brs);
   }
 }
 
@@ -805,6 +878,7 @@
   constexpr int MAIN_BYTES = S * STAGE * 2;
   constexpr int EPI_BYTES = WM * (BN + 4) * 4;
   constexpr int GL = (BM + BN) * 4 / NT;
+  static_assert(EPI != EPI_BN_SUMS || MAIN_BYTES >= BnSumsLds::END, "EPI_BN_SUMS: its LDS rows reuse the ring");
   __shared__ __attribute__((aligned(16))) char smem_epi[MAIN_BYTES > EPI_BYTES ? MAIN_BYTES : EPI_BYTES];
   bf16_t* smem = reinterpret_cast<bf16_t*>(smem_epi);
   const int tid = threadIdx.x, lane = tid & 63, wid = tid >> 6;
@@ -1248,9 +1322,13 @@
 }
 
 
+static inline bool epi_spec_on() {
+  static const int on = [] { const char* e = getenv("LASR_EPI_SPEC"); return e && e[0] ? atoi(e) : 1; }();
+  return on != 0;
+}
 static inline int epi_code(const GemmP& p) {
-  static const int on = [] { const char* e = getenv("LASR_EPI_SPEC"); return e && e[0] ? atoi(e) : 1; }();
-  if (!on || p.split_k > 1 || p.beta != 0.f || p.alpha_dev || p.N % 8 != 0) return EPI_RT;
+  if (!epi_spec_on() || p.split_k > 1 || p.beta != 0.f || p.alpha_dev || p.N % 8 != 0) return EPI_RT;
+  if (p.bn_part) return EPI_BN_SUMS;
   if (p.res) {
     return !p.zout && p.act == LASR_ACT_NONE && !p.aux && p.drop.p > 0.f && p.epi_mode == 1 ? EPI_RES_DROP : EPI_RT;
   }
diff --git a/liteasr_amd/csrc/gemm_launch.h b/liteasr_amd/csrc/gemm_launch.h
--- a/liteasr_amd/csrc/gemm_launch.h
+++ b/liteasr_amd/csrc/gemm_launch.h
@@ -17,6 +17,7 @@
       }
       if constexpr (AKC && !BKC && std::is_same<TC, bf16_t>::value) {
         if (e == EPI_AUX_GATE) { L64(EPI_AUX_GATE); return; }
+        if (e == EPI_BN_SUMS) { L64(EPI_BN_SUMS); return; }
       }
       if constexpr (AKC && BKC && std::is_same<TC, bf16_t>::value) {
         if (e == EPI_RELU_GATE_DROP) { L64(EPI_RELU_GATE_DROP); return; }
diff --git a/liteasr_amd/csrc/gemm_row.hip b/liteasr_amd/csrc/gemm_row.hip
--- a/liteasr_amd/csrc/gemm_row.hip
+++ b/liteasr_amd/csrc/gemm_row.hip
@@ -6,6 +6,7 @@
 constexpr int RB = 32;
 constexpr int BK = 32;
 constexpr int KS = 2;
+constexpr int ABN_MAX_K = 1024;
 
 template <int D>
 struct RowCfg {
@@ -23,6 +24,8 @@
   static constexpr int RPW = NPL <= 8 ? 1 : 2;
   static constexpr int SMEM = S * STAGE * 2;
   static_assert(SMEM >= (RB * LDC + RB * D) * 4, "epilogue staging must fit the ring");
+  static constexpr int ABN_SMEM = 2 * ABN_MAX_K * 4;
+  static_assert(SMEM + ABN_SMEM <= 160 * 1024, "ring + BN vectors must fit the LDS");
 };
 
 struct RowP {
@@ -47,6 +50,10 @@
   bf16_t* y2;
   float* mean2;
   float* rstd2;
+  const float* a_scale;
+  const float* a_shift;
+  bf16_t* a_out;
+  int a_relu;
   const float* x;
   const float* dres;
   float* dx;
@@ -63,6 +70,37 @@
   const bf16_t* src = p.A + (int64_t)gr * p.lda + k0 + u * BK + c * 8;
   __builtin_amdgcn_global_load_lds((gptr_t)src, (lptr_t)(stage + u * RowCfg<D>::TILE + (P & ~63) * 8), 16, 0,
                                    0);
+}
+
+LASR_DEV void ds_w128_asm(bf16_t* p, v4i v) {
+  const uint32_t a = (uint32_t)(uintptr_t)(lptr_t)p;
+  asm volatile("ds_write_b128 %0, %1" ::"v"(a), "v"(v) : "memory");
+}
+
+template <int D, bool RELU>
+LASR_DEV void abn_unit(const RowP& p, int m0, int k0, bf16_t* stage, const float* ssf, int tid) {
+  const int u = tid >> 7, P = tid & 127, r = P >> 2, c = (P & 3) ^ swz(r);
+  const int kc = k0 + u * BK + c * 8;
+  bf16_t* unit = stage + u * RowCfg<D>::TILE + P * 8;
+  v4i raw = ds_b128_asm(unit);
+  v4i s0 = ds_b128_asm((const bf16_t*)(ssf + kc)), s1 = ds_b128_asm((const bf16_t*)(ssf + kc + 4));
+  v4i f0 = ds_b128_asm((const bf16_t*)(ssf + p.K + kc)), f1 = ds_b128_asm((const bf16_t*)(ssf + p.K + kc + 4));
+  asm volatile("s_waitcnt lgkmcnt(0)" : "+v"(raw), "+v"(s0), "+v"(s1), "+v"(f0), "+v"(f1));
+  float v[8], sc[8], sf[8];
+#pragma unroll
+  for (int i = 0; i < 4; ++i) {
+    v[2 * i] = __uint_as_float((uint32_t)raw[i] << 16);
+    v[2 * i + 1] = __uint_as_float((uint32_t)raw[i] & 0xFFFF0000u);
+    sc[i] = __int_as_float(s0[i]); sc[4 + i] = __int_as_float(s1[i]);
+    sf[i] = __int_as_float(f0[i]); sf[4 + i] = __int_as_float(f1[i]);
+  }
+#pragma unroll
+  for (int q = 0; q < 8; ++q) v[q] = bn_act<RELU>(v[q] * sc[q] + sf[q]);
+  v4i h;
+#pragma unroll
+  for (int i = 0; i < 4; ++i) h[i] = (int)pk_bf16(v[2 * i], v[2 * i + 1]);
+  ds_w128_asm(unit, h);
+  if (m0 + r < p.M) *(v4i*)(p.a_out + (int64_t)(m0 + r) * p.K + kc) = h;
 }
 
 template <int R_TILE, bool KC>
@@ -86,7 +124,7 @@
   }
 }
 
-template <int D, bool BKC>
+template <int D, bool BKC, bool ABN = false>
 LASR_DEV void row_mainloop(const RowP& p, int m0, bf16_t* smem) {
   using Cf = RowCfg<D>;
   constexpr int FN = Cf::FN, S = Cf::S;
@@ -129,6 +167,14 @@
     const int after = min(S - 2, nst - 1 - kt);
     if (wid < 4) wait_ring<S, Cf::GLA>(after);
     else wait_ring<S, Cf::GLB>(after);
+    if constexpr (ABN) {
+      if (wid < 4) {
+        bf16_t* cur = smem + (kt % S) * Cf::STAGE;
+        const float* ssf = reinterpret_cast<const float*>(smem + S * Cf::STAGE);
+        if (p.a_relu) abn_unit<D, true>(p, m0, kt * (KS * BK), cur, ssf, tid);
+        else abn_unit<D, false>(p, m0, kt * (KS * BK), cur, ssf, tid);
+      }
+    }
     lds_barrier();
     if (kt + S - 1 < nst) issue(kt + S - 1);
 #pragma unroll
@@ -142,14 +188,22 @@
   __syncthreads();
 }
 
-template <int D, typename TY1>
+template <int D, typename TY1, bool ABN>
 __global__ __launch_bounds__(512, 1) void row_res_ln_kernel(RowP p) {
   using Cf = RowCfg<D>;
   constexpr int NPL = Cf::NPL, RW = Cf::RW;
-  __shared__ __attribute__((aligned(16))) char smem_raw[Cf::SMEM];
+  __shared__ __attribute__((aligned(16))) char smem_raw[Cf::SMEM + (ABN ? Cf::ABN_SMEM : 0)];
   bf16_t* smem = reinterpret_cast<bf16_t*>(smem_raw);
   const int m0 = blockIdx.x * RB;
   const int lane = threadIdx.x & 63, wid = threadIdx.x >> 6, c0 = lane * NPL;
+  if constexpr (ABN) {
+    float* ssf = reinterpret_cast<float*>(smem_raw + Cf::SMEM);
+    for (int i = threadIdx.x; i < p.K; i += Cf::NT) {
+      ssf[i] = p.a_scale[i];
+      ssf[p.K + i] = p.a_shift[i];
+    }
+    __syncthreads();
+  }
   float rv[RW][NPL];
 #pragma unroll
   for (int it = 0; it < RW; ++it) ldv<NPL>(p.res + (int64_t)min(m0 + it * 8 + wid, p.M - 1) * D + c0, rv[it]);
@@ -164,7 +218,7 @@
     ldv<NPL>(p.g2 + c0, g2);
     ldv<NPL>(p.b2 + c0, b2);
   }
-  row_mainloop<D, true>(p, m0, smem);
+  row_mainloop<D, true, ABN>(p, m0, smem);
 
   const float* cs = reinterpret_cast<const float*>(smem_raw);
   const bool drop = p.drop.p > 0.f;
@@ -302,20 +356,35 @@
   LASR_CHECK_ARG(!a->gamma2 || (a->y1_dtype == LASR_F32 && a->beta2 && a->y2 && a->mean2 && a->rstd2 &&
                                 al16(a->gamma2) && al16(a->beta2) && al16(a->y2)),
                  "lasr_linear_res_ln: the chained norm needs an fp32 y1 and gamma2 / beta2 / y2 / mean2 / rstd2");
+  const bool abn = a->a_scale || a->a_shift || a->a_out || a->a_act;
+  if (abn) {
+    LASR_CHECK_ARG(a->a_scale && a->a_shift && a->a_out,
+                   "lasr_linear_res_ln: a_scale, a_shift and a_out go together");
+    LASR_CHECK_ARG(a->a_act == LASR_ACT_SWISH || a->a_act == LASR_ACT_RELU,
+                   "lasr_linear_res_ln: a_act must be SWISH or RELU");
+    LASR_CHECK_ARG(al16(a->a_out) && al16(a->a_scale) && al16(a->a_shift),
+                   "lasr_linear_res_ln: a_out / a_scale / a_shift must be 16-B aligned");
+    LASR_CHECK_ARG(a->K <= ABN_MAX_K, "lasr_linear_res_ln: K=%d above %d with the A transform", a->K, ABN_MAX_K);
+    LASR_CHECK_ARG(a->a_out != a->A, "lasr_linear_res_ln: a_out must not be A (clamped rows re-read it)");
+  }
   if (a->M == 0) return LASR_OK;
   p.bias = a->bias; p.res = a->res; p.res_scale = a->res_scale;
   p.drop = mkdrop(a->drop_p, a->drop_seed);
   p.out = a->out; p.y1 = a->y1;
   p.g2 = a->gamma2; p.b2 = a->beta2; p.y2 = (bf16_t*)a->y2; p.mean2 = a->mean2; p.rstd2 = a->rstd2;
+  p.a_scale = a->a_scale; p.a_shift = a->a_shift; p.a_out = (bf16_t*)a->a_out; p.a_relu = a->a_act == LASR_ACT_RELU;
   const dim3 grid((unsigned)cdiv(a->M, RB));
   hipStream_t st = (hipStream_t)stream;
+#define ROW_RES(DD, TY) (abn ? row_res_ln_kernel<DD, TY, true><<<grid, 512, 0, st>>>(p) \
+                             : row_res_ln_kernel<DD, TY, false><<<grid, 512, 0, st>>>(p))
   if (a->D == 256) {
-    if (a->y1_dtype == LASR_F32) row_res_ln_kernel<256, float><<<grid, 512, 0, st>>>(p);
-    else row_res_ln_kernel<256, bf16_t><<<grid, 512, 0, st>>>(p);
+    if (a->y1_dtype == LASR_F32) ROW_RES(256, float);
+    else ROW_RES(256, bf16_t);
   } else {
-    if (a->y1_dtype == LASR_F32) row_res_ln_kernel<512, float><<<grid, 512, 0, st>>>(p);
-    else row_res_ln_kernel<512, bf16_t><<<grid, 512, 0, st>>>(p);
-  }
+    if (a->y1_dtype == LASR_F32) ROW_RES(512, float);
+    else ROW_RES(512, bf16_t);
+  }
+#undef ROW_RES
   return lasr_check_launch("lasr_linear_res_ln");
 }
 
diff --git a/liteasr_amd/kernels.py b/liteasr_amd/kernels.py
--- a/liteasr_amd/kernels.py
+++ b/liteasr_amd/kernels.py
@@ -262,6 +262,7 @@
     ln_fwd: Optional[tuple] = None,
     ln_bwd: Optional[object] = None,
     qbias: Optional[tuple] = None,
+    bn_sums: Optional[tuple] = None,
 ):
     if _narrow_set[0] != GEMM_NARROW_TILES:
         N.call("lasr_gemm_narrow_tiles", int(GEMM_NARROW_TILES))
@@ -404,8 +405,24 @@
             arr[0] = N.ReduceSeg(ptr(part), 2 * Nn, nblk, 1, ptr(q.dgamma), ptr(q.dbeta), Nn)
             N.call("lasr_reduce_multi", arr, 1, stream())
         return c
+    if bn_sums is not None:
+        y_, sc_, sf_, mu_, rs_, act_, part_ = bn_sums
+        assert y_.dtype == torch.bfloat16 and y_.is_contiguous() and tuple(y_.shape) == (M, Nn)
+        assert part_.dtype == torch.float32 and part_.numel() >= ((M + 63) // 64) * 2 * Nn
+        args.bn_y, args.bn_scale, args.bn_shift, args.bn_mean, args.bn_rstd = (ptr(t) for t in (y_, sc_, sf_, mu_, rs_))
+        args.bn_part, args.bn_act = ptr(part_), act_
     N.call("lasr_gemm", C.byref(args), stream())
     return c
+
+
+def bn_sums_workspace(rows, Cc, device):
+    return torch.empty(((rows + 63) // 64 + 1) * 2 * Cc, dtype=torch.float32, device=device)
+
+
+def gemm_bn_sums(a, b, c, y, scale, shift, mean, rstd, act, bn_ws):
+    fused = bool(gemm(a, b, c, plan_only="flags")[3] & N.PLAN_BN_SUMS)
+    gemm(a, b, c, bn_sums=(y, scale, shift, mean, rstd, act, bn_ws) if fused else None)
+    return fused
 
 
 def gemm_plan(a, b, c, flags=False, **kw):
@@ -487,6 +504,7 @@
 
 ROW_LN_MAX_K = 1024
 ROW_LN_MAX_D = 256
+ROW_LN_ABN_MAX_K = 1024
 
 
 def row_ln_ok(a, w, D, max_k=None, max_d=None):
@@ -498,7 +516,7 @@
 
 
 def linear_res_ln(x, w, out, y1, mean1, rstd1, g1, b1, eps, *, bias=None, res, res_scale=1.0, drop_p=0.0,
-                  drop_seed=0, g2=None, b2=None, y2=None, mean2=None, rstd2=None):
+                  drop_seed=0, g2=None, b2=None, y2=None, mean2=None, rstd2=None, a_bn=None):
     M, Kd = x.shape
     D = w.shape[0]
     a = N.RowLnArgs()
@@ -509,6 +527,11 @@
     a.out, a.y1, a.y1_dtype = ptr(out), ptr(y1), dt(y1)
     if g2 is not None:
         a.gamma2, a.beta2, a.y2, a.mean2, a.rstd2 = ptr(g2), ptr(b2), ptr(y2), ptr(mean2), ptr(rstd2)
+    if a_bn is not None:
+        scale, shift, act, h = a_bn
+        assert h.dtype == torch.bfloat16 and h.is_contiguous() and tuple(h.shape) == (M, Kd)
+        assert scale.dtype == shift.dtype == torch.float32 and scale.numel() == shift.numel() == Kd
+        a.a_scale, a.a_shift, a.a_act, a.a_out = ptr(scale), ptr(shift), act, ptr(h)
     N.call("lasr_linear_res_ln", C.byref(a), stream())
 
 
@@ -840,21 +863,24 @@
 
 
 def bn_act_glu_dwconv_bwd(y, dh, scale, shift, mean, rstd, gamma, dgamma, dbeta, z1, B, T, Cc, K, w, dz1, dw, db,
-                          batch_stats=True, act=N.ACT_SWISH):
+                          batch_stats=True, act=N.ACT_SWISH, bn_ws=None, bn_parts_ready=False):
     rows = y.shape[0]
     assert rows == B * T and y.shape[1] == Cc and dh.shape == y.shape and z1.shape == (rows, 2 * Cc)
-    bn_ws = torch.empty(((rows + 63) // 64 + 1) * 2 * Cc, dtype=torch.float32, device=y.device)
+    assert bn_ws is not None or not bn_parts_ready
+    entry = "lasr_bn_sums_glu_dwconv_bwd" if bn_parts_ready else "lasr_bn_act_glu_dwconv_bwd"
+    if bn_ws is None:
+        bn_ws = bn_sums_workspace(rows, Cc, y.device)
     nparts = dwconv_nparts(B, T)
     head = (ptr(y), dt(y), ptr(dh), dt(dh), B, T, Cc, ptr(scale), ptr(shift), ptr(mean), ptr(rstd), ptr(gamma),
             ptr(dgamma), ptr(dbeta), ptr(bn_ws), bn_ws.numel(), int(bool(batch_stats)), act, ptr(z1), dt(z1), K,
             ptr(w), ptr(dz1))
     if _DEFER.depth:
         ws = torch.empty(nparts * (K + 1) * Cc, dtype=torch.float32, device=z1.device)
-        N.call("lasr_bn_act_glu_dwconv_bwd", *head, None, None, ptr(ws), ws.numel(), stream())
+        N.call(entry, *head, None, None, ptr(ws), ws.numel(), stream())
         _defer(ws, nparts, (K + 1) * Cc, dw, db, split=K * Cc)
         return
     ws = WS.get((nparts + 1) * (K + 1) * Cc, z1.device)
-    N.call("lasr_bn_act_glu_dwconv_bwd", *head, ptr(dw), ptr(db), ptr(ws), ws.numel(), stream())
+    N.call(entry, *head, ptr(dw), ptr(db), ptr(ws), ws.numel(), stream())
 
 
 def cast(src, dst):
diff --git a/liteasr_amd/nets/functional.py b/liteasr_amd/nets/functional.py
--- a/liteasr_amd/nets/functional.py
+++ b/liteasr_amd/nets/functional.py
@@ -44,6 +44,8 @@
 QBIAS_IN_REDUCE = True
 LN2_BWD_CHAIN = True
 BN_GLU_FUSED = True
+BN_ACT_IN_PW2 = True
+BN_SUMS_IN_PW2_DX = True
 LAYER_RED_HOLD = True
 
 
@@ -71,13 +73,18 @@
     return y, m, r
 
 
-def res_proj(x, W, bias, res, res_scale, p_res, s_res, post=None):
+def res_proj_on_row(x, W, post):
+    return post is not None and ROW_LN and K.row_ln_ok(x, W, W.shape[0])
+
+
+def res_proj(x, W, bias, res, res_scale, p_res, s_res, post=None, a_bn=None):
     M, D = x.shape[0], W.shape[0]
     dev = x.device
     out = _e((M, D), F32, dev)
     if post is not None:
         post.y1 = None
-    if post is None or not ROW_LN or not K.row_ln_ok(x, W, D):
+    if not res_proj_on_row(x, W, post):
+        assert a_bn is None, "the A-operand BatchNorm runs on the row kernel only"
         if post is not None and SPLITK_LN and post.nxt is None and x.dtype == torch.bfloat16 and W.shape[1] >= 1024:
             post.y1 = _e((M, D), F32 if post.f32 else x.dtype, dev)
             post.m1, post.r1 = _e(M, F32, dev), _e(M, F32, dev)
@@ -94,7 +101,7 @@
         post.m2, post.r2 = _e(M, F32, dev), _e(M, F32, dev)
         kw = dict(g2=post.nxt[0], b2=post.nxt[1], y2=post.y2, mean2=post.m2, rstd2=post.r2)
     K.linear_res_ln(x, W, out, post.y1, post.m1, post.r1, post.g, post.b, LN_EPS, bias=bias, res=res,
-                    res_scale=res_scale, drop_p=p_res, drop_seed=s_res, **kw)
+                    res_scale=res_scale, drop_p=p_res, drop_seed=s_res, a_bn=a_bn, **kw)
     return out
 
 
@@ -439,8 +446,12 @@
     K.bn_finalize(stats, nparts, d, 1e-5, 0.1, w.gamma, w.beta, w.rmean, w.rvar, w.nbt, mean, rstd,
                   scale, shift, 1 if training else 2)
     h3 = _e((M, d), adt, dev)
-    K.bn_act_fwd(y, scale, shift, h3, act=getattr(w, "act", ACT_SWISH))
-    out = res_proj(h3, w.Wpw2, w.bpw2, x_in, 1.0, p_res, s_res, post)
+    act = getattr(w, "act", ACT_SWISH)
+    if BN_ACT_IN_PW2 and d <= K.ROW_LN_ABN_MAX_K and res_proj_on_row(y, w.Wpw2, post):
+        out = res_proj(y, w.Wpw2, w.bpw2, x_in, 1.0, p_res, s_res, post, a_bn=(scale, shift, act, h3))
+    else:
+        K.bn_act_fwd(y, scale, shift, h3, act=act)
+        out = res_proj(h3, w.Wpw2, w.bpw2, x_in, 1.0, p_res, s_res, post)
     return out, SimpleNamespace(z1=z1, y=y, mean=mean, rstd=rstd, scale=scale, shift=shift, h3=h3,
                                 training=training)
 
@@ -451,12 +462,19 @@
     dev, adt = ln.device, ln.dtype
     K.gemm(gb.t(), sv.h3, g.Wpw2, beta=1.0, split_k=0, rowsum=g.bpw2, group=True)
     dh3 = _e((M, d), adt, dev)
-    K.gemm(gb, w.Wpw2, dh3)
+    act = getattr(w, "act", ACT_SWISH)
+    fused_bn = BN_GLU_FUSED and d % 8 == 0
+    bn_ws, ready = None, False
+    if fused_bn and BN_SUMS_IN_PW2_DX and adt == torch.bfloat16:
+        bn_ws = K.bn_sums_workspace(M, d, dev)
+        ready = K.gemm_bn_sums(gb, w.Wpw2, dh3, sv.y, sv.scale, sv.shift, sv.mean, sv.rstd, act, bn_ws)
+    else:
+        K.gemm(gb, w.Wpw2, dh3)
     dz1 = _e((M, 2 * d), adt, dev)
-    if BN_GLU_FUSED and d % 8 == 0:
+    if fused_bn:
         K.bn_act_glu_dwconv_bwd(sv.y, dh3, sv.scale, sv.shift, sv.mean, sv.rstd, w.gamma, g.gamma, g.beta, sv.z1,
                                 B, T, d, w.kernel, w.wdw, dz1, g.wdw, g.bdw, batch_stats=sv.training,
-                                act=getattr(w, "act", ACT_SWISH))
+                                act=act, bn_ws=bn_ws, bn_parts_ready=ready)
     else:
         dy = _e((M, d), F32, dev)
         K.bn_act_bwd(sv.y, dh3, sv.scale, sv.shift, sv.mean, sv.rstd, w.gamma, g.gamma, g.beta, dy,
```

New measurement: 3526 utterances/sec, median of 6. Within noise of the previous version (+0.9%).
